# ifpen/wfcrl-env

Hardware: AMD Instinct MI355X
Metric: farm_steps_per_sec (higher is better)
Workload: dtype f32

## Files before the change

### include/wfstep.h

```cpp
#ifndef WFSTEP_H
#define WFSTEP_H

#ifdef __cplusplus
extern "C" {
#endif

#define WF_ABI_VERSION 7

#define WF_OK 0
#define WF_E_INVALID -1
#define WF_E_UNSUPPORTED -2
#define WF_E_NODEVICE -3
#define WF_E_HIP -4
#define WF_E_NOMEM -5

#define WF_MAX_TURBINES 256
#define WF_MAX_TABLE 64
#define WF_MAX_TURBINE_TYPES 4

typedef struct wf_handle wf_handle;

typedef struct wf_model_params {
  double air_density, ambient_ti, shear, veer;
  double rotor_diameter, hub_height, tsr, pP, pT, gen_eff, ref_density;
// ... 42 lines not shown
int wf_set_wind(wf_handle* h, const double* ws, const double* wd, int count, int on_device);

int wf_set_wind_counts(wf_handle* h, const double* ws, int n_ws, const double* wd, int n_wd, int on_device);

int wf_step(wf_handle* h, const float* yaw, float* power, float* wind_speed, float* wind_dir, float* load,
            int on_device);

int wf_sync(wf_handle* h);

#define WF_RISK_OVERLAP 1
#define WF_RISK_POWER_KNEE 2
#define WF_RISK_THRUST_RAMP 4
#define WF_RISK_THRUST_UNITY 8
#define WF_RISK_NEGATIVE_SPEED 16
int wf_set_risk_guard(wf_handle* h, double rel_band);
int wf_get_risk_flags(wf_handle* h, int* flags, int on_device);

int wf_set_risk_resolve(wf_handle* h, int mode);
int wf_get_risk_resolve(wf_handle* h, int* mode);
int wf_get_resolve_stats(wf_handle* h, int* n_resolved, int* raw_flags, int on_device);

typedef struct wf_env_params {
  float yaw_lo, yaw_hi, yaw_step;
  float actuator_rate;
  float dt;
  float budget;
  float load_coef;
  int discrete;
} wf_env_params;

int wf_env_config(wf_handle* h, const wf_env_params* p);

int wf_env_set_power_unit(wf_handle* h, int megawatts);

int wf_env_reset(wf_handle* h);

int wf_env_step(wf_handle* h, const float* action, float* reward, float* yaw, float* power, float* wind_speed,
                float* wind_dir, float* load, int on_device);

int wf_env_set_prev_wind(wf_handle* h, const double* wind_speed , int on_device);

int wf_env_state(wf_handle* h, float* yaw, float* acc, int* moves, int set, int on_device);

typedef struct wf_wind_dist {
  double ws_scale, ws_shape, ws_lo, ws_hi, wd_mean, wd_std, wd_lo, wd_hi;
} wf_wind_dist;
int wf_wind_sample(wf_handle* h, unsigned long long seed, const wf_wind_dist* dist);

int wf_wind_sample_binned(wf_handle* h, unsigned long long seed, const wf_wind_dist* dist, double step_deg);

int wf_wind_series(wf_handle* h, int T, const double* ws, const double* wd, const int* start, unsigned long long seed);
int wf_wind_series_step(wf_handle* h);

int wf_get_wind(wf_handle* h, double* ws, double* wd, int on_device);

int wf_timing_begin(wf_handle* h);
int wf_timing_end(wf_handle* h, float* elapsed_ms);

typedef struct wf_kernel_info {
  int lanes_per_env, slots_per_lane, envs_per_block, threads_per_block, grid_blocks;
  int vgprs, lds_bytes, scratch_bytes;
  int pair_table;
  int direction_groups;
  int mixed_main_farms;
  int one_block_kernel;
} wf_kernel_info;
int wf_get_kernel_info(wf_handle* h, wf_kernel_info* info);

typedef struct wf_kernel_choice {
  int slot_G, slot_S;
  int one_block;
  int ll_G, ll_S;
  int pair_table;
  int fly_one_block;
  int far_skip;
  int calibrate;
  int mixed;
} wf_kernel_choice;
int wf_set_kernel_choice(wf_handle* h, const wf_kernel_choice* c);
int wf_get_calibration(wf_handle* h, int* code, float* family_ms);
int wf_get_fly_calibration(wf_handle* h, int* choice, float* ms);
int wf_get_mixed_launch(wf_handle* h, int* main_farms, float* mixed_ms);
int wf_get_kernel_choice(wf_handle* h, wf_kernel_choice* c);
int wf_calibrate(wf_handle* h);
int wf_set_calibration(wf_handle* h, int code, int fly_choice);

const char* wf_last_error(wf_handle* h);

#ifdef __cplusplus
}
#endif
#endif
```

### wfcrl-env_amd/_lib.py

```python
from __future__ import annotations

import ctypes as C
import os
import subprocess
from pathlib import Path

PKG_DIR = Path(__file__).resolve().parent
LIB_PATH = PKG_DIR / "libwfstep.so"

WF_OK = 0
WF_RISK_OVERLAP = 1
WF_RISK_POWER_KNEE = 2
WF_RISK_THRUST_RAMP = 4
WF_RISK_THRUST_UNITY = 8
WF_RISK_NEGATIVE_SPEED = 16
WF_E = {-1: "WF_E_INVALID", -2: "WF_E_UNSUPPORTED", -3: "WF_E_NODEVICE", -4: "WF_E_HIP", -5: "WF_E_NOMEM"}

_MODEL_DOUBLES = (
    "air_density", "ambient_ti", "shear", "veer",
    "rotor_diameter", "hub_height", "tsr", "pP", "pT", "gen_eff", "ref_density",
    "alpha", "beta", "ka", "kb", "ad", "bd", "dm",
    "ch_initial", "ch_constant", "ch_ai", "ch_downstream",
    "eps_gain", "num_eps", "kappa", "gch_gain", "overlap_thresh", "near_wake_c",
    "defl_alpha", "defl_beta", "defl_ka", "defl_kb",
# ... 1 lines not shown
_MODEL_SWITCHES = ("enable_secondary_steering", "enable_yaw_added_recovery", "enable_transverse_velocities")


class ModelParams(C.Structure):

    _fields_ = [(n, C.c_double) for n in _MODEL_DOUBLES] + [
        ("n_table", C.c_int),
        ("table_ws", C.POINTER(C.c_double)),
        ("table_ct", C.POINTER(C.c_double)),
        ("table_cp", C.POINTER(C.c_double)),
    ] + [(n, C.c_int) for n in _MODEL_SWITCHES]


class TurbineDef(C.Structure):

    _fields_ = [("n_table", C.c_int), ("table_ws", C.POINTER(C.c_double)), ("table_ct", C.POINTER(C.c_double)),
                ("table_cp", C.POINTER(C.c_double))] + [(n, C.c_double) for n in ("tsr", "pP", "gen_eff", "ref_density")]


class EnvParams(C.Structure):

    _fields_ = [(n, C.c_float) for n in ("yaw_lo", "yaw_hi", "yaw_step", "actuator_rate", "dt", "budget", "load_coef")] + [
        ("discrete", C.c_int)]


class WindDist(C.Structure):

    _fields_ = [(n, C.c_double) for n in ("ws_scale", "ws_shape", "ws_lo", "ws_hi", "wd_mean", "wd_std", "wd_lo", "wd_hi")]


class KernelInfo(C.Structure):
    _fields_ = [(n, C.c_int) for n in (
        "lanes_per_env", "slots_per_lane", "envs_per_block", "threads_per_block", "grid_blocks",
        "vgprs", "lds_bytes", "scratch_bytes", "pair_table", "direction_groups", "mixed_main_farms", "one_block_kernel")]


class KernelChoice(C.Structure):

    _fields_ = [(n, C.c_int) for n in ("slot_G", "slot_S", "one_block", "ll_G", "ll_S", "pair_table", "fly_one_block", "far_skip", "calibrate", "mixed")]


_P = C.c_void_p
ABI = {
    "wf_version": (C.c_int, []),
    "wf_default_model": (C.c_int, [C.POINTER(ModelParams)]),
    "wf_turbine_table": (C.c_int, [C.c_char_p, C.POINTER(C.c_int), C.POINTER(C.POINTER(C.c_double)),
                                   C.POINTER(C.POINTER(C.c_double)), C.POINTER(C.POINTER(C.c_double))]),
    "wf_create": (C.c_int, [C.c_int, C.POINTER(_P)]),
    "wf_destroy": (C.c_int, [_P]),
    "wf_set_stream": (C.c_int, [_P, _P, C.c_int]),
    "wf_get_stream": (_P, [_P]),
    "wf_set_model": (C.c_int, [_P, C.POINTER(ModelParams)]),
    "wf_set_turbine_types": (C.c_int, [_P, C.c_int, C.POINTER(TurbineDef), C.POINTER(C.c_int)]),
    "wf_get_turbine_types": (C.c_int, [_P, C.POINTER(C.c_int)]),
    "wf_set_layout": (C.c_int, [_P, C.c_int, _P, _P]),
    "wf_set_batch": (C.c_int, [_P, C.c_int]),
    "wf_set_layouts": (C.c_int, [_P, C.c_int, _P, _P, _P]),
    "wf_set_layouts_counts": (C.c_int, [_P, C.c_int, _P, _P, _P, _P]),
    "wf_set_wind": (C.c_int, [_P, _P, _P, C.c_int, C.c_int]),
    "wf_set_wind_counts": (C.c_int, [_P, _P, C.c_int, _P, C.c_int, C.c_int]),
    "wf_wind_sample_binned": (C.c_int, [_P, C.c_ulonglong, C.POINTER(WindDist), C.c_double]),
    "wf_step": (C.c_int, [_P, _P, _P, _P, _P, _P, C.c_int]),
    "wf_sync": (C.c_int, [_P]),
    "wf_set_risk_guard": (C.c_int, [_P, C.c_double]),
    "wf_get_risk_flags": (C.c_int, [_P, _P, C.c_int]),
    "wf_set_risk_resolve": (C.c_int, [_P, C.c_int]),
    "wf_get_risk_resolve": (C.c_int, [_P, C.POINTER(C.c_int)]),
    "wf_get_resolve_stats": (C.c_int, [_P, C.POINTER(C.c_int), _P, C.c_int]),
    "wf_wind_sample": (C.c_int, [_P, C.c_ulonglong, C.POINTER(WindDist)]),
    "wf_wind_series": (C.c_int, [_P, C.c_int, _P, _P, _P, C.c_ulonglong]),
    "wf_wind_series_step": (C.c_int, [_P]),
    "wf_get_wind": (C.c_int, [_P, _P, _P, C.c_int]),
    "wf_env_config": (C.c_int, [_P, C.POINTER(EnvParams)]),
    "wf_env_set_power_unit": (C.c_int, [_P, C.c_int]),
    "wf_env_reset": (C.c_int, [_P]),
    "wf_env_state": (C.c_int, [_P, _P, _P, _P, C.c_int, C.c_int]),
    "wf_env_set_prev_wind": (C.c_int, [_P, _P, C.c_int]),
    "wf_env_step": (C.c_int, [_P, _P, _P, _P, _P, _P, _P, _P, C.c_int]),
    "wf_timing_begin": (C.c_int, [_P]),
    "wf_timing_end": (C.c_int, [_P, C.POINTER(C.c_float)]),
    "wf_get_kernel_info": (C.c_int, [_P, C.POINTER(KernelInfo)]),
    "wf_set_kernel_choice": (C.c_int, [_P, C.POINTER(KernelChoice)]),
    "wf_get_kernel_choice": (C.c_int, [_P, C.POINTER(KernelChoice)]),
    "wf_get_calibration": (C.c_int, [_P, C.POINTER(C.c_int), C.POINTER(C.c_float)]),
    "wf_get_fly_calibration": (C.c_int, [_P, C.POINTER(C.c_int), C.POINTER(C.c_float)]),
    "wf_get_mixed_launch": (C.c_int, [_P, C.POINTER(C.c_int), C.POINTER(C.c_float)]),
    "wf_calibrate": (C.c_int, [_P]),
    "wf_set_calibration": (C.c_int, [_P, C.c_int, C.c_int]),
    "wf_last_error": (C.c_char_p, [_P]),
}

PROBE_ABI = {
    "wf_probe_create": (C.c_int, [_P, C.POINTER(_P)]),
    "wf_probe_destroy": (C.c_int, [_P]),
    "wf_probe_set_points": (C.c_int, [_P, C.c_int, _P, C.c_int, C.c_int]),
    "wf_probe_sample": (C.c_int, [_P, _P, C.c_int, _P, _P, C.c_int]),
    "wf_probe_last_timing": (C.c_int, [_P, C.POINTER(C.c_float), C.POINTER(C.c_float)]),
    "wf_probe_kernel_info": (C.c_int, [_P, C.POINTER(C.c_int)]),
    "wf_probe_last_error": (C.c_char_p, [_P]),
}

YAWOPT_ABI = {
    "wf_yawopt_create": (C.c_int, [_P, C.POINTER(_P)]),
    "wf_yawopt_destroy": (C.c_int, [_P]),
    "wf_yawopt_config": (C.c_int, [_P, C.c_double, C.c_double, C.c_int, C.POINTER(C.c_int), C.c_int, C.c_int]),
    "wf_yawopt_run": (C.c_int, [_P, _P, C.c_int, _P, _P, _P, _P, C.c_int]),
    "wf_yawopt_set_timing": (C.c_int, [_P, C.c_int]),
    "wf_yawopt_last_timing": (C.c_int, [_P, C.POINTER(C.c_float), C.POINTER(C.c_float), C.POINTER(C.c_float)]),
    "wf_yawopt_evaluator": (_P, [_P]),
    "wf_yawopt_last_error": (C.c_char_p, [_P]),
}

ROSE_ABI = {
    "wf_rose_create": (C.c_int, [_P, C.POINTER(_P)]),
    "wf_rose_destroy": (C.c_int, [_P]),
    "wf_rose_set_table": (C.c_int, [_P, C.c_int, C.c_int, _P, C.c_int, _P, _P, C.c_int, C.c_int]),
    "wf_rose_set_rose": (C.c_int, [_P, C.c_int, _P, C.c_int, _P, _P, C.c_double, C.c_double]),
    "wf_rose_config": (C.c_int, [_P, C.c_int, C.c_int]),
    "wf_rose_evaluate": (C.c_int, [_P, C.c_int, _P, _P, _P, _P, _P, _P, C.c_int]),
    "wf_rose_policy": (C.c_int, [_P, C.c_int, _P, _P, C.c_int]),
    "wf_rose_last_timing": (C.c_int, [_P, C.POINTER(C.c_float), C.POINTER(C.c_float), C.POINTER(C.c_float)]),
    "wf_rose_kernel_info": (C.c_int, [_P, C.POINTER(C.c_int)]),
    "wf_rose_last_error": (C.c_char_p, [_P]),
}

ROBUST_ABI = {
    "wf_robust_create": (C.c_int, [_P, C.POINTER(_P)]),
    "wf_robust_destroy": (C.c_int, [_P]),
    "wf_robust_set_members": (C.c_int, [_P, C.c_int, _P, _P, C.c_int]),
    "wf_robust_config": (C.c_int, [_P, C.c_double, C.c_double, C.c_int, C.POINTER(C.c_int), C.c_int, C.c_int]),
    "wf_robust_evaluate": (C.c_int, [_P, _P, C.c_int, _P, _P, _P, _P, C.c_int]),
    "wf_robust_optimize": (C.c_int, [_P, _P, C.c_int, _P, _P, _P, _P, C.c_int]),
    "wf_robust_set_timing": (C.c_int, [_P, C.c_int]),
    "wf_robust_last_timing": (C.c_int, [_P, C.POINTER(C.c_float), C.POINTER(C.c_float), C.POINTER(C.c_float)]),
    "wf_robust_evaluator": (_P, [_P]),
    "wf_robust_kernel_info": (C.c_int, [_P, C.POINTER(C.c_int)]),
    "wf_robust_last_error": (C.c_char_p, [_P]),
}

GRAD_ABI = {
    "wf_grad_create": (C.c_int, [_P, C.POINTER(_P)]),
    "wf_grad_destroy": (C.c_int, [_P]),
    "wf_grad_config": (C.c_int, [_P, C.c_double, C.c_double, C.c_double, C.c_int, C.c_int]),
    "wf_grad_run": (C.c_int, [_P, _P, _P, C.c_int, _P, _P, _P, _P, C.c_int]),
    "wf_grad_set_timing": (C.c_int, [_P, C.c_int]),
    "wf_grad_last_timing": (C.c_int, [_P, C.POINTER(C.c_float), C.POINTER(C.c_float), C.POINTER(C.c_float)]),
    "wf_grad_evaluator": (_P, [_P]),
    "wf_grad_kernel_info": (C.c_int, [_P, C.POINTER(C.c_int)]),
    "wf_grad_last_error": (C.c_char_p, [_P]),
}

_lib = None


def build(force: bool = False) -> Path:
    srcs = []
    for d in ("", "ext", "probe", "yawopt", "rose", "robust", "grad"):
        srcs += sorted((PKG_DIR / "csrc" / d).glob("*.hip")) + sorted((PKG_DIR / "csrc" / d).glob("*.h"))
    srcs += [PKG_DIR.parent / "include" / h for h in ("wfstep.h", "wfprobe.h", "wfyawopt.h", "wfrose.h", "wfrobust.h", "wfgrad.h")]
    stale = (not LIB_PATH.exists()) or any(s.stat().st_mtime > LIB_PATH.stat().st_mtime for s in srcs)
    if force or stale:
        subprocess.run(["make", "-j4", "-C", str(PKG_DIR / "csrc")] + (["-B"] if force else []), check=True)
    return LIB_PATH


def _share_hip_runtime_with_torch():
# ... 62 lines not shown
```

### wfcrl-env_amd/backend.py

```python
from __future__ import annotations

import ctypes as C

import numpy as np

from . import _lib
from ._lib import EnvParams, KernelChoice, KernelInfo, ModelParams, WindDist, check


def _is_torch(a) -> bool:
    return type(a).__module__.startswith("torch")


def default_model() -> dict:
    p = ModelParams()
    check(_lib.load().wf_default_model(C.byref(p)))
    d = {n: getattr(p, n) for n in _lib._MODEL_DOUBLES}
    d.update({n: bool(getattr(p, n)) for n in _lib._MODEL_SWITCHES})
    n = p.n_table
    d["table_ws"] = [p.table_ws[i] for i in range(n)]
    d["table_ct"] = [p.table_ct[i] for i in range(n)]
    d["table_cp"] = [p.table_cp[i] for i in range(n)]
    return d

# ... 447 lines not shown

    def env_set_state(self, state: dict):
        B, N = self.env_batch, self.num_turbines
        yaw = np.ascontiguousarray(state["yaw"], np.float32).reshape(B, N)
        acc = np.ascontiguousarray(state["acc"], np.float32).reshape(B, N)
        moves = np.ascontiguousarray(state["moves"], np.int32).reshape(B)
        check(self._lib.wf_env_state(self._h, yaw.ctypes.data, acc.ctypes.data, moves.ctypes.data, 1, 0), self._h)

    def env_step(self, action=None, want=("reward", "yaw", "power", "wind_speed", "wind_direction", "load"), out=None):
        B, N = self.env_batch, self.num_turbines
        shapes = {"reward": (B,), "yaw": (B, N), "power": (B, N), "wind_speed": (B, N), "wind_direction": (B, N),
                  "load": (B, N, 4)}
        order = ("reward", "yaw", "power", "wind_speed", "wind_direction", "load")
        use_torch = _is_torch(action) or (action is None and out is not None and any(_is_torch(v) for v in out.values()))
        if use_torch:
            import torch

            dev = action.device if action is not None else next(iter(out.values())).device
            self._follow_torch_stream()
            if action is not None:
                assert action.is_cuda and action.dtype == torch.float32 and action.numel() == B * N
                action = action.contiguous()
            out = dict(out or {})
            for k in want:
                if k not in out:
                    out[k] = torch.empty(shapes[k], device=dev, dtype=torch.float32)
            ptrs = [out[k].data_ptr() if k in want else None for k in order]
            check(self._lib.wf_env_step(self._h, action.data_ptr() if action is not None else None, *ptrs, 1), self._h)
            return {k: out[k] for k in want}
        if action is not None:
            action = np.ascontiguousarray(action, dtype=np.float32).reshape(B, N)
        out = dict(out or {})
        for k in want:
            if k not in out:
                out[k] = np.empty(shapes[k], np.float32)
        ptrs = [out[k].ctypes.data if k in want else None for k in order]
        check(self._lib.wf_env_step(self._h, action.ctypes.data if action is not None else None, *ptrs, 0), self._h)
        return {k: out[k] for k in want}

    def sync(self):
        check(self._lib.wf_sync(self._h), self._h)

    def set_risk_guard(self, rel_band: float):
        check(self._lib.wf_set_risk_guard(self._h, float(rel_band)), self._h)

    def set_risk_resolve(self, mode: int | bool = 1):
        check(self._lib.wf_set_risk_resolve(self._h, int(mode)), self._h)

    def risk_resolve(self) -> int:
        m = C.c_int(0)
        check(self._lib.wf_get_risk_resolve(self._h, C.byref(m)), self._h)
        return int(m.value)

    def resolve_stats(self) -> dict:
        if not self.risk_resolve():
            raise RuntimeError("resolve_stats() needs the float64 re-solve on (set_risk_resolve(1), the default); with it off "
                               "the flags of the last step are risk_flags()")
        n = C.c_int(0)
        raw = np.empty(self.env_batch, np.int32)
        check(self._lib.wf_get_resolve_stats(self._h, C.byref(n), raw.ctypes.data, 0), self._h)
        return {"n_resolved": int(n.value), "raw_flags": raw}

    def risk_flags(self, as_torch: bool = False):
        B = self.env_batch
        if as_torch:
            import torch

            self._follow_torch_stream()
            f = torch.empty(B, dtype=torch.int32, device=f"cuda:{self.device_id}")
            check(self._lib.wf_get_risk_flags(self._h, f.data_ptr(), 1), self._h)
            return f
        f = np.empty(B, np.int32)
        check(self._lib.wf_get_risk_flags(self._h, f.ctypes.data, 0), self._h)
        return f

    def timing_begin(self):
        check(self._lib.wf_timing_begin(self._h), self._h)

    def timing_end(self) -> float:
        ms = C.c_float()
        check(self._lib.wf_timing_end(self._h, C.byref(ms)), self._h)
        return float(ms.value)

    def set_kernel_choice(self, slot=None, one_block=None, pair_table=None, fly_one_block=None, far_skip=None, calibrate=None, mixed=None):
        def gs(v, default_s=1):
            if isinstance(v, bool):
                raise ValueError("a kernel shape is (G, S), 'GxS' or G — not a bool (one_block=False disables the one-block "
                                 "kernel, None leaves the choice to the rounds model)")
            if isinstance(v, str):
                parts = v.lower().split("x")
                return int(parts[0]), (int(parts[1]) if len(parts) > 1 else default_s)
            if isinstance(v, int):
                return v, default_s
            return int(v[0]), int(v[1])

        c = KernelChoice(0, 0, -1, 0, 0, -1, -1, -1, -1, -1)
        if slot:
            c.slot_G, c.slot_S = gs(slot)
        if one_block is not None:
            if one_block is False or (not isinstance(one_block, bool) and one_block == 0):
                c.one_block = 0
            else:
                c.one_block = 1
                c.ll_G, c.ll_S = gs(one_block)
        if pair_table is not None:
            c.pair_table = int(bool(pair_table)) if pair_table is False else -1
        if fly_one_block is not None:
            c.fly_one_block = 0 if fly_one_block is False else -1
        if far_skip is not None:
            c.far_skip = 0 if far_skip is False or far_skip == 0 else -1
        if calibrate is not None:
            c.calibrate = 0 if calibrate is False or calibrate == 0 else -1
        if mixed is not None:
            c.mixed = 0 if mixed is False or mixed == 0 else -1
        check(self._lib.wf_set_kernel_choice(self._h, C.byref(c)), self._h)

    def kernel_choice(self) -> dict:
        c = KernelChoice()
        check(self._lib.wf_get_kernel_choice(self._h, C.byref(c)), self._h)
        return {n: getattr(c, n) for n, _ in KernelChoice._fields_}

    def calibration(self) -> dict:
        code = C.c_int(-1)
        ms = (C.c_float * 6)()
        check(self._lib.wf_get_calibration(self._h, C.byref(code), ms), self._h)
        names = ("slot", "8x1", "4x2", "4x1", "2x2", "16x1")
        shape = None if code.value < 0 else ("slot" if code.value == 0 else f"{code.value >> 4}x{code.value & 15}")
        fly, fms = C.c_int(0), (C.c_float * 2)()
        check(self._lib.wf_get_fly_calibration(self._h, C.byref(fly), fms), self._h)
        mixn, mixms = C.c_int(0), C.c_float(0.0)
        check(self._lib.wf_get_mixed_launch(self._h, C.byref(mixn), C.byref(mixms)), self._h)
        return {"shape": shape, "family_ms": {n: float(m) for n, m in zip(names, ms) if m > 0.0},
                "on_the_fly": (None, "one_block", "slot")[fly.value], "on_the_fly_ms": {n: float(m) for n, m in zip(("one_block", "slot"), fms) if m > 0.0},
                "mixed_main_farms": int(mixn.value), "mixed_ms": float(mixms.value)}

    def calibrate(self):
        check(self._lib.wf_calibrate(self._h), self._h)

    _FAMILY_CODES = {"slot": 0, "8x1": (8 << 4) | 1, "4x2": (4 << 4) | 2, "4x1": (4 << 4) | 1, "2x2": (2 << 4) | 2, "16x1": (16 << 4) | 1}

    def set_calibration(self, shape=None, on_the_fly=None):
        code = -1 if shape is None else self._FAMILY_CODES[shape]
        fly = {None: 0, "one_block": 1, "slot": 2}[on_the_fly]
        check(self._lib.wf_set_calibration(self._h, code, fly), self._h)

    def kernel_info(self) -> dict:
        k = KernelInfo()
        check(self._lib.wf_get_kernel_info(self._h, C.byref(k)), self._h)
        return {n: getattr(k, n) for n, _ in KernelInfo._fields_}

    def close(self):
        if getattr(self, "_h", None) is not None and self._h.value:
            for name in ("_probe_points", "_probe_plane", "_yawopt_obj", "_rose_obj", "_robust_obj", "_grad_obj"):
                ext = getattr(self, name, None)
                if ext is not None:
                    ext.close()
                    setattr(self, name, None)
            self._lib.wf_destroy(self._h)
            self._h = C.c_void_p()

    def __del__(self):
        try:
            self.close()
        except Exception:
            pass


class _Ext:

    NAME = ""
    KERNELS = ()

    def __init__(self, owner: WfStep):
        self._w, self._lib = owner, owner._lib
        self._r = C.c_void_p()
        check(self._fn("create")(owner._h, C.byref(self._r)), owner._h)

    def _fn(self, name):
        return getattr(self._lib, f"wf_{self.NAME}_{name}")

    def _call(self, name, *args):
        _lib.check_ext(self._fn(name)(self._r, *args), self._r, f"wf_{self.NAME}_last_error")

    def timing(self, detail=None):
        if detail is not None:
            self._call("set_timing", int(bool(detail)))
            return None
        t = [C.c_float(), C.c_float(), C.c_float()]
        self._call("last_timing", *[C.byref(v) for v in t])
        return {"total_ms": float(t[0].value), "step_ms": float(t[1].value), "glue_ms": float(t[2].value)}

    def kernel_info(self) -> dict:
        v = (C.c_int * (3 * len(self.KERNELS)))()
        self._call("kernel_info", v)
        keys = ("vgprs", "lds_bytes", "scratch_bytes")
        return {n: dict(zip(keys, v[3 * i:3 * i + 3])) for i, n in enumerate(self.KERNELS)}

    def evaluator(self):
# ... 319 lines not shown
```

### wfcrl-env_amd/csrc/ext/wf_ext.h

```cpp
#pragma once
#include <functional>

#include "../wf_handle.h"
#include "wf_ext_kernels.h"

namespace wfi {

struct ext_base {
  wf_handle* h = nullptr;
  std::string err;
  int detail = 0;
  std::vector<hipEvent_t> ev_pool;
  size_t n_ev = 0, per_chunk = 0;
  bool timed = false;
  ~ext_base();
};

inline int ext_fail(ext_base* x, int code, const std::string& msg) {
  if (x) x->err = msg;
  return code;
}
#define WFX_HIP(x, call)                                                                             \
  do {                                                                                               \
    hipError_t e_ = (call);                                                                          \
    if (e_ != hipSuccess) return ext_fail(x, WF_E_HIP, std::string(#call) + ": " + hipGetErrorString(e_)); \
  } while (0)
#define WFX_EV(x, evh, call)                                                     \
  do {                                                                           \
    int rc_ = (call);                                                            \
    if (rc_ != WF_OK) return ext_fail(x, rc_, std::string("evaluator: ") + wf_last_error(evh)); \
  } while (0)
#define WFX_ON_DEVICE(x)                 \
  DeviceGuard guard_((x)->h->device);    \
  if (guard_.err != hipSuccess) return ext_fail(x, WF_E_HIP, std::string("hipSetDevice: ") + hipGetErrorString(guard_.err))

template <class T>
struct dev_buf {
  T* p = nullptr;
  size_t cap = 0;
  dev_buf() = default;
  dev_buf(const dev_buf&) = delete;
  dev_buf& operator=(const dev_buf&) = delete;
  ~dev_buf() { hipFree(p); }
  operator T*() const { return p; }
};

template <class T>
int reserve(ext_base* x, dev_buf<T>& buf, size_t n) {
  if (n <= buf.cap) return WF_OK;
  WFX_HIP(x, hipStreamSynchronize(x->h->stream));
  hipFree(buf.p);
  buf.p = nullptr; buf.cap = 0;
  WFX_HIP(x, hipMalloc(&buf.p, sizeof(T) * n));
  buf.cap = n;
  return WF_OK;
}

struct evaluator {
  wf_handle* ev = nullptr;
  int E = 0, mode = -1;
  wf_model_params model{};
  std::vector<double> tws, tct, tcp, lx, ly;
  wf_kernel_choice choice{};
  double guard = 0.0;
  hipStream_t stream = nullptr;
  evaluator() = default;
  evaluator(const evaluator&) = delete;
  evaluator& operator=(const evaluator&) = delete;
  ~evaluator() { if (ev) wf_destroy(ev); }
};
int ensure_evaluator(ext_base* x, evaluator& s, int E, int mode);

struct farm_list {
  dev_buf<int> d;
  std::vector<int> host;
};

int check_parent(ext_base* x, const char* what, const char* call);
int check_wind(ext_base* x, const char* call);
int check_farms(ext_base* x, int* n_farms, const int* farms);
int upload_farms(ext_base* x, farm_list& fl, const int* farms, int n_farms);

inline WfSlots chunk_slots(const farm_list& fl, const int* farms, int base, int n_farms, int C) {
  return WfSlots{farms ? fl.d.p : nullptr, base, n_farms - base < C ? n_farms - base : C, C};
}

template <class T>
int stage_in(ext_base* x, const dev_buf<T>& buf, const T* src, size_t n, int on_device, const T** d) {
  *d = src;
  if (!src || on_device) return WF_OK;
  WFX_HIP(x, hipMemcpyAsync(buf.p, src, sizeof(T) * n, hipMemcpyHostToDevice, x->h->stream));
  *d = buf.p;
  return WF_OK;
}
template <class T>
T* out_ptr(T* user, const dev_buf<T>& staging, size_t offset, int on_device) {
  return user ? (on_device ? user : staging.p + offset) : nullptr;
}

int record(ext_base* x);
int last_timing(ext_base* x, const char* not_run, float* total_ms, float* step_ms, float* glue_ms);
int kernel_info(ext_base* x, int n, hipError_t (*attributes)(int, hipFuncAttributes*), int* info);

struct search_config {
  double lo = -25.0, hi = 25.0;
  int P = 2, K[WF_SEARCH_MAX_PASSES] = {5, 4, 0, 0};
  int strict = 0, max_eval = 65536;
};
int set_search_config(ext_base* x, search_config& c, double lo, double hi, int n_passes, const int* K, int strict, int max_eval_farms,
                      int rows_per_candidate, const char* rows_msg);
int k_max(int P, const int* K);
void pass_grids(double lo, double hi, int P, const int* K, WfGrid* grid);

struct yaw_search {
  search_config cfg;
  dev_buf<float> d_yaw, d_pow, d_best;
  dev_buf<int> d_order;
  farm_list farms;
  dev_buf<float> d_in, d_out;
};

struct search_policy {
  const char *what, *name;
  int rows_per_candidate;
  std::string no_rows;
  const char* rows_msg;
  std::function<int(int E)> reserve;
  std::function<int(const WfSlots&, int R, int E)> begin_chunk;
  std::function<int(const WfAdvanceArgs&, int v)> visit;
};
int run_search(ext_base* x, yaw_search& s, evaluator& es, const search_policy& k, const float* yaw0, int n_farms, const int* farms,
               float* yaw_opt, float* power_opt, float* power_init, int on_device);

template <class T>
int ext_create(wf_handle* h, T** out) {
  if (!h || !out) return WF_E_INVALID;
  *out = nullptr;
  T* x = new (std::nothrow) T();
  if (!x) return fail(h, WF_E_NOMEM, "out of host memory");
  x->h = h;
  *out = x;
  return WF_OK;
}

template <class T>
int ext_destroy(T* x) {
// ... 9 lines not shown
```

### wfcrl-env_amd/csrc/ext/wf_ext.hip

```cpp
#include "wf_ext.h"

namespace wfi {

ext_base::~ext_base() {
  for (hipEvent_t e : ev_pool) hipEventDestroy(e);
}

namespace {

bool same_model(const wf_model_params& a, const wf_model_params& b) {
  return std::memcmp(&a, &b, offsetof(wf_model_params, n_table)) == 0 && a.n_table == b.n_table &&
         a.enable_secondary_steering == b.enable_secondary_steering && a.enable_yaw_added_recovery == b.enable_yaw_added_recovery &&
         a.enable_transverse_velocities == b.enable_transverse_velocities;
}

}

int ensure_evaluator(ext_base* x, evaluator& s, int E, int mode) {
  wf_handle* h = x->h;
  const size_t n = (size_t)h->N;
  const bool same = s.ev && s.E == E && same_model(s.model, h->model) && s.tws == h->tws && s.tct == h->tct && s.tcp == h->tcp &&
                    s.lx.size() == n && std::equal(s.lx.begin(), s.lx.end(), h->lx.begin()) &&
                    std::equal(s.ly.begin(), s.ly.end(), h->ly.begin()) &&
                    std::memcmp(&s.choice, &h->choice, sizeof(wf_kernel_choice)) == 0 && s.guard == h->guard_rel;
  if (same) {
    if (s.stream != h->stream) {
      WFX_EV(x, s.ev, wf_set_stream(s.ev, (void*)h->stream, 1));
      s.stream = h->stream;
    }
    if (s.mode != mode) {
      WFX_EV(x, s.ev, wf_set_risk_resolve(s.ev, mode));
      s.mode = mode;
    }
    return WF_OK;
  }
  WFX_HIP(x, hipStreamSynchronize(h->stream));
  if (s.ev) wf_destroy(s.ev);
  s.ev = nullptr;
  wf_handle* ev = nullptr;
  if (wf_create(h->device, &ev) != WF_OK) return ext_fail(x, WF_E_HIP, std::string("evaluator: ") + wf_last_error(nullptr));
  s.ev = ev;
  wf_model_params m = h->model;
  m.table_ws = h->tws.data(); m.table_ct = h->tct.data(); m.table_cp = h->tcp.data();
  WFX_EV(x, ev, wf_set_stream(ev, (void*)h->stream, 1));
  WFX_EV(x, ev, wf_set_model(ev, &m));
  WFX_EV(x, ev, wf_set_kernel_choice(ev, &h->choice));
  if (h->guard_user) WFX_EV(x, ev, wf_set_risk_guard(ev, h->guard_rel));
  WFX_EV(x, ev, wf_set_layout(ev, h->N, h->lx.data(), h->ly.data()));
  WFX_EV(x, ev, wf_set_batch(ev, E));
  WFX_EV(x, ev, wf_set_risk_resolve(ev, mode));
  s.E = E; s.mode = mode; s.stream = h->stream;
  s.model = h->model; s.tws = h->tws; s.tct = h->tct; s.tcp = h->tcp;
  s.lx.assign(h->lx.begin(), h->lx.begin() + n); s.ly.assign(h->ly.begin(), h->ly.begin() + n);
  s.choice = h->choice; s.guard = h->guard_rel;
  return WF_OK;
}

int check_wind(ext_base* x, const char* call) {
  if (x->h->wind_count == 0)
    return ext_fail(x, WF_E_INVALID, std::string("no wind has been set: wf_set_wind (or wf_wind_*) must be called before ") + call);
  return WF_OK;
}

int check_parent(ext_base* x, const char* what, const char* call) {
  wf_handle* h = x->h;
  if (h->N <= 0 || h->B <= 0) return ext_fail(x, WF_E_INVALID, "no layout / batch: wf_set_layout and wf_set_batch come first");
  if (h->n_layouts > 1 || !h->layout_n.empty())
    return ext_fail(x, WF_E_UNSUPPORTED, std::string(what) + " a handle with ONE layout: this one holds several layouts (wf_set_layouts / wf_set_layouts_counts)");
  if (!h->types.empty())
    return ext_fail(x, WF_E_UNSUPPORTED, std::string(what) + " one turbine definition: this handle holds several turbine definitions (wf_set_turbine_types)");
  return call ? check_wind(x, call) : WF_OK;
}

int check_farms(ext_base* x, int* n_farms, const int* farms) {
  if (!farms) {
    *n_farms = x->h->B;
    return WF_OK;
  }
  if (*n_farms < 1) return ext_fail(x, WF_E_INVALID, "n_farms must be >= 1");
  for (int k = 0; k < *n_farms; ++k)
    if (farms[k] < 0 || farms[k] >= x->h->B) return ext_fail(x, WF_E_INVALID, "farm index out of range (0 .. env_batch - 1)");
  return WF_OK;
}

int upload_farms(ext_base* x, farm_list& fl, const int* farms, int n_farms) {
  WFX_HIP(x, hipStreamSynchronize(x->h->stream));
  fl.host.assign(farms, farms + n_farms);
  WFX_HIP(x, hipMemcpyAsync(fl.d, fl.host.data(), sizeof(int) * n_farms, hipMemcpyHostToDevice, x->h->stream));
  return WF_OK;
}

int record(ext_base* x) {
  if (x->n_ev == x->ev_pool.size()) {
    hipEvent_t e = nullptr;
    WFX_HIP(x, hipEventCreate(&e));
    x->ev_pool.push_back(e);
  }
  WFX_HIP(x, hipEventRecord(x->ev_pool[x->n_ev++], x->h->stream));
  return WF_OK;
}

int last_timing(ext_base* x, const char* not_run, float* total_ms, float* step_ms, float* glue_ms) {
  if (!x->timed || x->n_ev < 2) return ext_fail(x, WF_E_INVALID, not_run);
  WFX_ON_DEVICE(x);
  WFX_HIP(x, hipEventSynchronize(x->ev_pool[x->n_ev - 1]));
  float total = 0.0f, step = 0.0f, glue = 0.0f;
  WFX_HIP(x, hipEventElapsedTime(&total, x->ev_pool[0], x->ev_pool[x->n_ev - 1]));
  for (size_t k = 1; x->per_chunk && k < x->n_ev; ++k) {
    float ms = 0.0f;
    WFX_HIP(x, hipEventElapsedTime(&ms, x->ev_pool[k - 1], x->ev_pool[k]));
    const size_t q = k % x->per_chunk;
    if (q != 0 && q % 2 == 0) step += ms;
    else glue += ms;
  }
  if (total_ms) *total_ms = total;
  if (step_ms) *step_ms = step;
  if (glue_ms) *glue_ms = glue;
  return WF_OK;
}

int kernel_info(ext_base* x, int n, hipError_t (*attributes)(int, hipFuncAttributes*), int* info) {
  WFX_ON_DEVICE(x);
  for (int k = 0; k < n; ++k) {
    hipFuncAttributes a{};
    WFX_HIP(x, attributes(k, &a));
    info[3 * k] = a.numRegs; info[3 * k + 1] = (int)a.sharedSizeBytes; info[3 * k + 2] = (int)a.localSizeBytes;
  }
  return WF_OK;
}

int set_search_config(ext_base* x, search_config& c, double lo, double hi, int n_passes, const int* K, int strict, int max_eval_farms,
                      int rows_per_candidate, const char* rows_msg) {
  if (!std::isfinite(lo) || !std::isfinite(hi) || !(lo < hi)) return ext_fail(x, WF_E_INVALID, "yaw bounds must be finite with lo < hi");
  if (n_passes < 1 || n_passes > WF_SEARCH_MAX_PASSES) return ext_fail(x, WF_E_INVALID, "the number of passes must be in 1..4");
  if (K[0] < 2 || K[0] > WF_SEARCH_MAX_K0) return ext_fail(x, WF_E_INVALID, "the first pass needs 2..31 candidates (K_0)");
  for (int p = 1; p < n_passes; ++p)
    if (K[p] < 1 || K[p] > WF_SEARCH_MAX_K) return ext_fail(x, WF_E_INVALID, "a refining pass needs 1..15 candidates (K_p)");
// ... 98 lines not shown
```

### wfcrl-env_amd/csrc/wf_abi.hip

```cpp
#include "wf_handle.h"

namespace wfi {

thread_local std::string g_create_error;

void free_batch(wf_handle* h) {
  hipFree(h->d_ws); hipFree(h->d_wd); hipFree(h->d_gx); hipFree(h->d_gy); hipFree(h->d_gidx); hipFree(h->d_flags);
  hipFree(h->d_farm_tie);
  hipFree(h->d_dir_perm); hipFree(h->d_sort_keys); hipFree(h->d_sort_vals); hipFree(h->d_sort_tmp);
  h->d_dir_perm = h->d_sort_vals = nullptr; h->d_sort_keys = nullptr; h->d_sort_tmp = nullptr;
  h->sort_tmp_bytes = h->dir_perm_cap = 0; h->dir_slots = 0;
  hipFree(h->d_res_list); hipFree(h->d_res_count); hipFree(h->d_flags_raw);
  h->d_res_list = h->d_res_count = h->d_flags_raw = nullptr;
  if (h->h_res_seen) (void)hipHostFree(h->h_res_seen);
  h->h_res_seen = nullptr;
  h->d_flags = h->d_farm_tie = nullptr;
  hipFree(h->d_yaw); hipFree(h->d_out);
  hipFree(h->d_env_yaw); hipFree(h->d_env_acc); hipFree(h->d_env_act); hipFree(h->d_env_out); hipFree(h->d_env_moves);
  if (h->h_env_act) hipHostFree(h->h_env_act);
  if (h->h_env_out) hipHostFree(h->h_env_out);
  h->d_env_yaw = h->d_env_acc = h->d_env_act = h->d_env_out = h->h_env_act = h->h_env_out = nullptr;
  h->d_env_moves = nullptr;
  hipFree(h->d_series_ws); hipFree(h->d_series_wd); hipFree(h->d_series_start); hipFree(h->d_ws_prev);
  hipFree(h->d_pair_tab); hipFree(h->d_pair_first); h->d_pair_tab = nullptr; h->d_pair_first = nullptr; h->pair_dirty = true;
  hipFree(h->d_ll_tab); hipFree(h->d_ll_flag); hipFree(h->d_src_log);
  h->d_ll_tab = h->d_src_log = nullptr; h->d_ll_flag = nullptr; h->ll_groups_cap = h->log_records_cap = 0;
  hipFree(h->d_perm); hipFree(h->d_blk_group); hipFree(h->d_group_wd); hipFree(h->d_bins);
  h->d_perm = h->d_blk_group = h->d_bins = nullptr; h->d_group_wd = nullptr;
  h->perm_cap = h->blk_cap = h->pair_groups_cap = 0; h->n_groups = 0; h->grid_step = 0.0;
  h->d_series_ws = h->d_series_wd = h->d_ws_prev = nullptr; h->d_series_start = nullptr; h->series_T = 0;
  if (h->h_yaw) hipHostFree(h->h_yaw);
  if (h->h_out) hipHostFree(h->h_out);
  h->d_ws = h->d_wd = h->d_gx = h->d_gy = nullptr; h->d_gidx = nullptr;
  h->d_yaw = h->d_out = h->h_yaw = h->h_out = nullptr;
  h->cap_env = h->cap_bn = 0;
}

}

using namespace wfi;

extern "C" {

int wf_version(void) { return WF_ABI_VERSION; }
int wf_create(int device_id, wf_handle** out) {
  if (!out) return fail(nullptr, WF_E_INVALID, "out == NULL");
  *out = nullptr;
  int ndev = 0;
  hipError_t e = hipGetDeviceCount(&ndev);
  if (e != hipSuccess || ndev <= 0)
    return fail(nullptr, WF_E_NODEVICE, std::string("no HIP device visible (") + hipGetErrorString(e) +
                                            "); libwfstep has no CPU fallback");
  if (device_id < 0 || device_id >= ndev) return fail(nullptr, WF_E_NODEVICE, "device id out of range");
  wf_handle* h = new (std::nothrow) wf_handle();
  if (!h) return fail(nullptr, WF_E_NOMEM, "out of host memory");
  h->device = device_id;
  {
    wf_kernel_choice& c = h->choice;
    if (getenv("WF_NO_PAIR_TABLE")) c.pair_table = 0;
    const char* f = getenv("WF_LL_FLY");
    if (f && f[0] == '0') c.fly_one_block = 0;
    const char* gs = getenv("WF_KERNEL_GS");
    int og = 0, os = 0;
    if (gs && sscanf(gs, "%dx%d", &og, &os) == 2 && og > 0 && os > 0) { c.slot_G = og; c.slot_S = os; }
    const char* off = getenv("WF_LL");
    if (off && off[0] == '0') c.one_block = 0;
    const char* fs = getenv("WF_LL_FAR_SKIP");
    if (fs && fs[0] == '0') c.far_skip = 0;
    const char* rr = getenv("WF_RISK_RESOLVE");
    if (rr && rr[0] >= '0' && rr[0] <= '2' && rr[1] == 0) h->resolve_mode = rr[0] - '0';
    const char* cal = getenv("WF_CALIBRATE");
    if (cal && cal[0] == '0') c.calibrate = 0;
    const char* force = getenv("WF_LL_G");
    if (force && c.one_block != 0) {
      int g = 0, sl = 1;
      if (sscanf(force, "%dx%d", &g, &sl) >= 1) { c.one_block = 1; c.ll_G = g; c.ll_S = sl; }
      else c.one_block = 0;
    }
  }
  DeviceGuard guard(device_id);
  if ((e = guard.err) != hipSuccess || (e = hipStreamCreateWithFlags(&h->own_stream, hipStreamNonBlocking)) != hipSuccess ||
      (e = hipEventCreate(&h->ev0)) != hipSuccess || (e = hipEventCreate(&h->ev1)) != hipSuccess ||
      (e = hipMalloc(&h->d_tab, sizeof(WfTables))) != hipSuccess) {
    std::string msg = std::string("wf_create: ") + hipGetErrorString(e);
    delete h;
    return fail(nullptr, WF_E_HIP, msg);
  }
  h->stream = h->own_stream;
  {
    hipDeviceProp_t prop;
    if (hipGetDeviceProperties(&prop, device_id) == hipSuccess && prop.multiProcessorCount > 0) h->n_cu = prop.multiProcessorCount;
  }
  wf_model_params p;
  wf_default_model(&p);
  h->model = p;
  h->tws.assign(p.table_ws, p.table_ws + p.n_table);
  h->tct.assign(p.table_ct, p.table_ct + p.n_table);
  h->tcp.assign(p.table_cp, p.table_cp + p.n_table);
  *out = h;
  return WF_OK;
}

int wf_destroy(wf_handle* h) {
  if (!h) return WF_OK;
  DeviceGuard guard(h->device);
  hipStreamSynchronize(h->stream);
  free_batch(h);
  hipFree(h->d_tab64_mt); hipFree(h->d_type_consts); hipFree(h->d_type_of);
  hipFree(h->d_tab); hipFree(h->d_tab64); hipFree(h->d_lx); hipFree(h->d_ly); hipFree(h->d_centre); hipFree(h->d_layout_of);
  hipEventDestroy(h->ev0); hipEventDestroy(h->ev1);
  hipStreamDestroy(h->own_stream);
  delete h;
  return WF_OK;
}

int wf_set_stream(wf_handle* h, void* s, int external) {
  if (!h) return WF_E_INVALID;
  WF_ON_DEVICE(h);
  hipStream_t next = external ? (hipStream_t)s : h->own_stream;
  if (next != h->stream) {
    WF_HIP(h, hipStreamSynchronize(h->stream));
    h->stream = next;
  }
  return WF_OK;
}
void* wf_get_stream(wf_handle* h) { return h ? (void*)h->stream : nullptr; }

static int upload_layouts(wf_handle* h, int n, int K, const double* x, const double* y, const int* layout_of, const int* counts = nullptr) {
  std::vector<double> centre(2 * (size_t)K);
  for (int l = 0; l < K; ++l) {
    const double *xl = x + (size_t)l * n, *yl = y + (size_t)l * n;
    double xmin = xl[0], xmax = xl[0], ymin = yl[0], ymax = yl[0];
    const int n_l = counts ? counts[l] : n;
    for (int i = 0; i < n_l; ++i) {
      if (!std::isfinite(xl[i]) || !std::isfinite(yl[i])) return fail(h, WF_E_INVALID, "turbine coordinates must be finite");
      xmin = std::fmin(xmin, xl[i]); xmax = std::fmax(xmax, xl[i]);
      ymin = std::fmin(ymin, yl[i]); ymax = std::fmax(ymax, yl[i]);
    }
    centre[2 * l] = (xmin + xmax) / 2.0; centre[2 * l + 1] = (ymin + ymax) / 2.0;
  }
  WF_HIP(h, hipStreamSynchronize(h->stream));
  hipFree(h->d_lx); hipFree(h->d_ly); hipFree(h->d_centre); hipFree(h->d_layout_of); hipFree(h->d_layout_n); hipFree(h->d_nreal);
  h->d_lx = h->d_ly = h->d_centre = nullptr; h->d_layout_of = h->d_layout_n = h->d_nreal = nullptr;
  h->layout_n.clear();
  const size_t kn = (size_t)K * n;
  WF_HIP(h, hipMalloc(&h->d_lx, sizeof(double) * kn));
  WF_HIP(h, hipMalloc(&h->d_ly, sizeof(double) * kn));
  WF_HIP(h, hipMalloc(&h->d_centre, sizeof(double) * 2 * K));
  WF_HIP(h, hipMemcpy(h->d_lx, x, sizeof(double) * kn, hipMemcpyHostToDevice));
  WF_HIP(h, hipMemcpy(h->d_ly, y, sizeof(double) * kn, hipMemcpyHostToDevice));
  WF_HIP(h, hipMemcpy(h->d_centre, centre.data(), sizeof(double) * 2 * K, hipMemcpyHostToDevice));
// ... 212 lines not shown
```

### wfcrl-env_amd/csrc/wf_dispatch.hip

```cpp
#include "wf_handle.h"

#include <cstdlib>
#include <cstddef>
#include <map>
#include <tuple>

namespace wfi {

int find_variant(int G, int S) {
  for (int i = 0; i < wfk_num_variants(); ++i) {
    int g, s; const void* fn;
    wfk_variant(i, &g, &s, &fn);
    if (g == G && s == S) return i;
  }
  return -1;
}

int pick_variant(const wf_handle* h, int N, int B) {
  if (h->choice.slot_G > 0 && h->choice.slot_G * h->choice.slot_S >= N) {
    const int v = find_variant(h->choice.slot_G, h->choice.slot_S);
    if (v >= 0) return v;
  }
  static const int pref[][3] = {
      {4, 4, 1}, {8, 4, 2}, {12, 4, 3}, {16, 4, 4}, {24, 8, 3}, {32, 8, 4}, {48, 16, 3}, {64, 16, 4},
// ... 89 lines not shown
  const long per_round = (long)h->n_cu * per_cu * fpb;
  return (main_farms / per_round) * round_ms(fi, N, per_cu) + 0.9 * ll_estimate(h, 0, N, B - main_farms);
}

double family_estimate(const wf_handle* h, int fi, int N, long B, int* mix) {
  double t = ll_estimate(h, fi, N, B);
  *mix = 0;
  const int m = mix_candidate(h, fi, N, B);
  if (m) {
    const double tm = mix_estimate(h, fi, N, B, m);
    if (tm < 0.93 * t) { t = tm; *mix = m; }
  }
  return t;
}

int pick_ll(const wf_handle* h, int N, int B) {
  if (h->choice.one_block == 0) return 0;
  const bool veer = h->model.veer != 0.0;
  if (N > WF_PAIR_MAX_N) return 0;
  if (h->choice.one_block == 1) {
    const int g = h->choice.ll_G, sl = h->choice.ll_S > 0 ? h->choice.ll_S : 1;
    const bool ok = ((g == 4 || g == 8 || g == 16) && sl == 1) || ((g == 4 || g == 2) && sl == 2);
    return (ok && N > g * sl && (!veer || wfk_ll_has_veer(g, sl, 1))) ? ((g << 4) | sl) : 0;
  }
  if (N <= 16) return 0;
  {
    int fpb, per_cu;
    family_shape(h, 0, N, &fpb, &per_cu);
    if ((long)B <= (long)h->n_cu * fpb) return 0;
  }
  int best = 0;
  double t_best = 1e300;
  for (int fi = 0; fi < kNumFamilies; ++fi) {
    const LlFamily& f = kLlFamilies[fi];
    if (f.code && N <= (f.code >> 4) * (f.code & 15)) continue;
    if (f.code == ((8 << 4) | 1) && N <= 32) continue;
    if (veer && f.code && !wfk_ll_has_veer(f.code >> 4, f.code & 15, 1)) continue;
    int mix_unused;
    double t = family_estimate(h, fi, N, B, &mix_unused);
    if (f.code == ((16 << 4) | 1) && (long)B <= 2l * h->n_cu * f.farms_per_block) t *= 1.04;
    if (t < t_best) { t_best = t; best = f.code; }
  }
  return best;
}

int repick_ll_slots(const wf_handle* h, int N, int ll_G, int ll_S, long farm_slots) {
  if (ll_G != 4 || h->choice.one_block == 1 || N <= 8) return ll_S;
  return ll_estimate(h, 3, N, farm_slots) < ll_estimate(h, 2, N, farm_slots) ? 1 : 2;
}

void reset_calibration(wf_handle* h) {
  h->calib_done = false; h->calib_code = -1; h->tab_slot = false; h->mix_main = 0;
  for (float& m : h->calib_ms) m = 0.0f;
  h->fly_calib = 0; h->fly_calib_ms[0] = h->fly_calib_ms[1] = 0.0f;
}

int model_mix(const wf_handle* h, int code, int N, int B) {
  if (!code || h->choice.one_block == 0) return 0;
  for (int fi = 0; fi < kNumFamilies; ++fi)
    if (kLlFamilies[fi].code == code) {
      int m = 0;
      family_estimate(h, fi, N, B, &m);
      return m;
    }
  return 0;
}

void apply_kernel_pick(wf_handle* h, int N, int B, bool* variant_changed) {
  reset_calibration(h);
  const int v = pick_variant(h, N, B);
  const int llg = pick_ll(h, N, B);
  set_ll_shape(h, llg >> 4, llg ? (llg & 15) : 1);
  h->mix_main = model_mix(h, llg, N, B);
  if (variant_changed) *variant_changed = v != h->variant;
  if (v != h->variant) {
    hipFree(h->d_pair_tab); hipFree(h->d_pair_first);
    h->d_pair_tab = nullptr; h->d_pair_first = nullptr; h->pair_dirty = true; h->pair_groups_cap = 0;
    h->variant = v;
  }
}

void set_ll_shape(wf_handle* h, int G, int S) {
  if (G == h->ll_G && S == h->ll_S) return;
  hipFree(h->d_ll_tab); hipFree(h->d_ll_flag); hipFree(h->d_src_log);
  h->d_ll_tab = h->d_src_log = nullptr; h->d_ll_flag = nullptr; h->ll_groups_cap = h->log_records_cap = 0;
  h->ll_G = G; h->ll_S = S; h->pair_dirty = true;
}
int pair_table(wf_handle* h, const float** out) {
  *out = nullptr;
  if ((h->wind_count != 1 && !h->shared_dir && h->n_groups == 0) || h->N > WF_PAIR_MAX_N || !wfk_variant_has_table(h->variant) || h->choice.pair_table == 0)
    return WF_OK;
  int vG, vS; const void* vfn;
  wfk_variant(h->variant, &vG, &vS, &vfn);
  const int NP = vG * vS;
  const size_t ng = h->n_groups > 0 ? (size_t)h->n_groups : 1;
  if (!h->d_pair_tab || h->pair_groups_cap < ng) {
    hipFree(h->d_pair_tab); hipFree(h->d_pair_first);
    h->d_pair_tab = nullptr; h->d_pair_first = nullptr; h->pair_groups_cap = 0;
    WF_HIP(h, hipMalloc(&h->d_pair_tab, sizeof(float) * ng * h->N * WF_PAIR_ROW_FLOATS(NP)));
    WF_HIP(h, hipMalloc(&h->d_pair_first, sizeof(int) * ng * h->N));
    h->pair_groups_cap = ng;
    h->pair_dirty = true;
  }
  if (h->pair_dirty) {
    const wf_model_params& m = h->model;
    WfPairConsts pc{};
    const double D = m.rotor_diameter, HH = m.hub_height, eps = m.eps_gain * D;
    pc.N = h->N; pc.NP = NP; pc.D = D; pc.HH = HH; pc.eps2 = eps * eps; pc.num_eps = m.num_eps; pc.ch_down = m.ch_downstream;
    const double off[3] = {-D / 4, 0.0, D / 4};
    double uinf = 0;
    for (int k = 0; k < 3; ++k) uinf += std::pow((HH + off[k]) / HH, m.shear) / 3.0;
    pc.fifteenD = 15.0 * D;
    pc.twoD = 2.0 * D;
    pc.gam_top = (1.0 / 16.0) * D * std::pow((HH + D / 2) / HH, m.shear) * uinf;
    pc.gam_bot = (1.0 / 16.0) * D * std::pow((HH - D / 2) / HH, m.shear) * uinf;
    for (int k = 0; k < 3; ++k) {
      pc.off[k] = off[k];
      const double z = HH + off[k];
      const double dudz = m.shear * std::pow(1.0 / HH, m.shear) * std::pow(z, m.shear - 1.0);
      const double lm = m.kappa * z / (1.0 + m.kappa * z / (D / 8.0));
      pc.decay_a[k] = 4.0 * lm * lm * std::fabs(dudz) / uinf / pc.eps2;
    }
    WF_HIP(h, wfk_launch_pair_table(&pc, (int)ng, h->d_gx, h->d_gy, h->d_pair_tab, h->d_pair_first, h->stream));
    if (h->ll_G) {
      if (!h->d_ll_tab || h->ll_groups_cap < ng) {
        hipFree(h->d_ll_tab); hipFree(h->d_ll_flag);
        h->d_ll_tab = nullptr; h->d_ll_flag = nullptr; h->ll_groups_cap = 0;
        WF_HIP(h, hipMalloc(&h->d_ll_tab, sizeof(float) * ng * wfk_ll_table_floats(h->N, h->ll_G * h->ll_S)));
        WF_HIP(h, hipMalloc(&h->d_ll_flag, sizeof(int) * ng));
        h->ll_groups_cap = ng;
      }
      WF_HIP(h, wfk_launch_pair_table_ll(&pc, h->ll_G * h->ll_S, (int)ng, h->d_gx, h->d_gy, h->d_ll_tab, h->d_ll_flag, h->stream));
      h->ll_ties = 2;
      if (h->wind_sync) {
        std::vector<int> f(ng);
        WF_HIP(h, hipMemcpyAsync(f.data(), h->d_ll_flag, sizeof(int) * ng, hipMemcpyDeviceToHost, h->stream));
        WF_HIP(h, hipStreamSynchronize(h->stream));
        size_t tied = 0;
        for (int v : f) tied += v != 0;
        h->ll_ties = tied == 0 ? 0 : (tied == ng ? 1 : 2);
      }
    }
    h->pair_dirty = false;
  }
  *out = h->d_pair_tab;
  return WF_OK;
}

int ll_fly_S(const wf_handle* h);
int ll_fly_G(const wf_handle* h);
int run_geometry(wf_handle* h, int n_env, const double* d_wd, bool sync_ok) {
  const bool per_farm = n_env == h->B && h->B > 1 && h->ll_G && wfk_ll_has_fly(ll_fly_G(h), ll_fly_S(h));
  WF_HIP(h, wfk_launch_geometry(n_env, h->N, h->d_lx, h->d_ly, h->d_centre, h->n_layouts == 1 ? 0 : (h->d_layout_of ? 2 : 1),
                                h->d_layout_of, h->d_layout_n, d_wd, 1, h->d_gx, h->d_gy, h->d_gidx,
                                per_farm ? ll_fly_G(h) * ll_fly_S(h) : 0, h->d_farm_tie, h->d_farm_tie ? h->d_farm_tie + h->B : nullptr,
                                h->stream));
  h->farm_ties = 2;
  h->dir_slots = 0;
  h->geo_tie_block = per_farm ? ll_fly_G(h) * ll_fly_S(h) : 0;
  if (per_farm && h->n_layouts == 1 && h->choice.fly_one_block != 0 && h->choice.far_skip != 0) {
    const int fpb = wfk_ll_farms_per_block(ll_fly_G(h));
    const size_t slots = (size_t)((h->B + fpb - 1) / fpb) * fpb;
    if (slots > h->dir_perm_cap) {
      WF_HIP(h, hipStreamSynchronize(h->stream));
      hipFree(h->d_dir_perm); hipFree(h->d_sort_keys); hipFree(h->d_sort_vals); hipFree(h->d_sort_tmp);
      h->d_dir_perm = h->d_sort_vals = nullptr; h->d_sort_keys = nullptr; h->d_sort_tmp = nullptr; h->dir_perm_cap = 0;
      WF_HIP(h, wfk_sort_tmp_bytes(h->B, &h->sort_tmp_bytes));
      WF_HIP(h, hipMalloc(&h->d_dir_perm, sizeof(int) * slots));
      WF_HIP(h, hipMalloc(&h->d_sort_keys, sizeof(float) * 2 * (size_t)h->B));
      WF_HIP(h, hipMalloc(&h->d_sort_vals, sizeof(int) * (size_t)h->B));
      WF_HIP(h, hipMalloc(&h->d_sort_tmp, h->sort_tmp_bytes > 0 ? h->sort_tmp_bytes : 16));
      h->dir_perm_cap = slots;
    }
    WF_HIP(h, wfk_sort_by_direction(h->B, (int)slots, d_wd, h->d_sort_keys, h->d_sort_vals, h->d_sort_tmp, h->sort_tmp_bytes,
                                    h->d_dir_perm, h->stream));
    h->dir_slots = (int)slots;
  }
  if (per_farm && sync_ok) {
    int any = 0;
    WF_HIP(h, hipMemcpyAsync(&any, h->d_farm_tie + h->B, sizeof(int), hipMemcpyDeviceToHost, h->stream));
    WF_HIP(h, hipStreamSynchronize(h->stream));
    h->farm_ties = any ? 1 : 0;
  }
  return WF_OK;
}

int ll_fly_S(const wf_handle* h) { return h->ll_G <= 4 ? 2 : h->ll_S; }
int ll_fly_G(const wf_handle* h) {
  if (h->ll_G == 2) return h->model.veer != 0.0 ? 4 : 2;
  return h->ll_G == 16 ? 8 : h->ll_G;
}

size_t ll_npad(const wf_handle* h) {
  const int a = h->ll_G * h->ll_S, b = ll_fly_G(h) * ll_fly_S(h), gs = a > b ? a : b;
  return (size_t)((h->N + gs - 1) / gs) * gs;
}

int ll_log_fpb(const wf_handle* h) {
  const int a = wfk_ll_farms_per_block(h->ll_G), b = wfk_ll_farms_per_block(ll_fly_G(h));
  return a > b ? a : b;
}
static int ensure_log(wf_handle* h, size_t slots, size_t* records) {
  *records = slots * ll_npad(h);
  if (*records > h->log_records_cap) {
    WF_HIP(h, hipStreamSynchronize(h->stream));
    hipFree(h->d_src_log); h->d_src_log = nullptr; h->log_records_cap = 0;
    WF_HIP(h, hipMalloc(&h->d_src_log, sizeof(float) * *records * (WF_LOG_FLOATS + WF_LOG_SIDE_FLOATS)));
    h->log_records_cap = *records;
  }
  return WF_OK;
}
int launch_step_f32(wf_handle* h, const float* yaw, float* power, float* wspd, float* wdir, float* load, const WfEnvArgs* ea) {
  const int gstride = (h->wind_count == 1 || h->shared_dir) ? 0 : h->N;
  const int wstride = (h->wind_count == 1) ? 0 : 1;
  const float* ptab = nullptr;
  int rc = pair_table(h, &ptab);
  if (rc != WF_OK) return rc;
  WfGroupArgs ga{};
  ga.mod = 1;
  ga.risk_flags = h->d_flags;
  ga.n_real = h->d_nreal;
  if (h->res_mask) {
    ga.res_list = h->d_res_list; ga.flags_raw = h->d_flags_raw; ga.res_mask = h->res_mask;
    ga.res_count = h->d_res_count + h->res_parity; ga.res_zero = h->d_res_count + (h->res_parity ^ 1);
  }
  ga.blk_unit = 1;
  if (h->n_groups > 0) {
    ga.perm = h->d_perm; ga.blk_group = h->d_blk_group; ga.n_blocks = h->n_blocks;
    ga.shift = h->group_shift; ga.mod = h->n_groups;
    ga.blk_unit = group_unit(h); ga.n_slots = h->n_slots;
  }
  if (ptab && h->ll_G && !(h->tab_slot && h->n_groups == 0)) {
    const int fpb = ll_log_fpb(h);
    const size_t slots = h->n_groups > 0 ? (size_t)h->n_slots : (size_t)((h->B + fpb - 1) / fpb) * fpb;
    size_t log_records = 0;
    if ((rc = ensure_log(h, slots, &log_records)) != WF_OK) return rc;
    const int M = (h->choice.mixed != 0 && h->mix_main > 0 && h->mix_main < h->B && h->n_groups == 0) ? h->mix_main : 0;
    if (M) { ga.env_base = 0; ga.env_end = M; }
    if (h->ll_ties != 1)
      WF_HIP(h, wfk_launch_step_ll(h->ll_G, h->ll_S, &h->consts, h->d_tab, h->d_gidx, h->d_ws, h->d_wd, wstride, yaw, power, wspd, wdir,
                                   load, h->B, ea, h->d_ll_tab, h->d_ll_flag, h->d_src_log,
                                   log_records, &ga, h->stream));
    if (M) {
      if (h->ll_ties != 0) {
        WfGroupArgs gp = ga;
        gp.pred = h->d_ll_flag;
        WF_HIP(h, wfk_launch_step(h->variant, &h->consts, h->d_tab, h->d_gx, h->d_gy, h->d_gidx, gstride, h->d_ws, h->d_wd,
                                  wstride, yaw, power, wspd, wdir, load, h->B, ea, ptab, h->d_pair_first, &gp, h->stream, &h->grid));
      }
      ga.env_base = M; ga.env_end = h->B;
      WF_HIP(h, wfk_launch_step(h->variant, &h->consts, h->d_tab, h->d_gx, h->d_gy, h->d_gidx, gstride, h->d_ws, h->d_wd,
                                wstride, yaw, power, wspd, wdir, load, h->B, ea, ptab, h->d_pair_first, &ga, h->stream, &h->grid));
      return WF_OK;
    }
    if (h->ll_ties == 0) return WF_OK;
    ga.pred = h->d_ll_flag;
  }
  if (!ptab && gstride != 0 && h->B > 1 && h->ll_G && wfk_ll_has_fly(ll_fly_G(h), ll_fly_S(h)) && h->choice.fly_one_block != 0 &&
      h->fly_calib != 2) {
    const int fpb = ll_log_fpb(h);
    const size_t slots = (size_t)((h->B + fpb - 1) / fpb) * fpb;
    size_t log_records = 0;
    if ((rc = ensure_log(h, slots, &log_records)) != WF_OK) return rc;
    if (h->geo_tie_block != ll_fly_G(h) * ll_fly_S(h)) {
      if ((rc = run_geometry(h, h->B, h->d_wd, false)) != WF_OK) return rc;
    }
    WfGroupArgs gf = ga;
    if (h->dir_slots > 0 && h->n_groups == 0) gf.perm = h->d_dir_perm;
    WF_HIP(h, wfk_launch_step_ll_fly(ll_fly_G(h), ll_fly_S(h), &h->consts, h->d_tab, h->d_gidx, h->d_gx, h->d_gy, h->d_ws, h->d_wd, yaw,
                                     power, wspd, wdir, load, h->B, ea, h->d_farm_tie, h->d_src_log,
                                     log_records, &gf, h->stream));
    if (h->farm_ties == 0) return WF_OK;
    ga.farm_pred = h->d_farm_tie;
  }
  WF_HIP(h, wfk_launch_step(h->variant, &h->consts, h->d_tab, h->d_gx, h->d_gy, h->d_gidx, gstride, h->d_ws, h->d_wd,
                            wstride, yaw, power, wspd, wdir, load, h->B, ea, ptab, h->d_pair_first, &ga, h->stream, &h->grid));
  return WF_OK;
}

static bool calibration_due(const wf_handle* h) {
  if (h->calib_done || h->choice.calibrate == 0 || h->choice.one_block != -1 || h->choice.pair_table == 0) return false;
  if (h->N <= 16 || h->N > WF_PAIR_MAX_N || h->n_groups > 0 || h->n_layouts != 1) return false;
  if (!(h->wind_count == 1 || h->shared_dir) || !wfk_variant_has_table(h->variant)) return false;
  int fpb, per_cu;
  family_shape(h, 0, h->N, &fpb, &per_cu);
  return (long)h->B > (long)h->n_cu * fpb;
}

struct CalibKey {
  int device, N, B, n_cu, far_skip;
  int mixed, slot_G, slot_S;
  unsigned long long layout_hash, model_hash;
  bool operator<(const CalibKey& o) const {
    return std::tie(device, N, B, n_cu, far_skip, mixed, slot_G, slot_S, layout_hash, model_hash) <
           std::tie(o.device, o.N, o.B, o.n_cu, o.far_skip, o.mixed, o.slot_G, o.slot_S, o.layout_hash, o.model_hash);
  }
};
struct CalibVal {
  bool have_tab = false, have_fly = false;
  int code = -1, fly = 0, mix_main = 0;
  float ms[8] = {}, fly_ms[2] = {};
};
static std::mutex g_calib_mu;
static std::map<CalibKey, CalibVal> g_calib;

static unsigned long long fnv(const void* p, size_t n, unsigned long long hsh = 1469598103934665603ull) {
  const unsigned char* b = static_cast<const unsigned char*>(p);
  for (size_t i = 0; i < n; ++i) hsh = (hsh ^ b[i]) * 1099511628211ull;
  return hsh;
}
static CalibKey calib_key(const wf_handle* h) {
  CalibKey k{};
  k.device = h->device; k.N = h->N; k.B = h->B; k.n_cu = h->n_cu; k.far_skip = h->choice.far_skip;
  k.mixed = h->choice.mixed != 0; k.slot_G = h->choice.slot_G; k.slot_S = h->choice.slot_S;
  k.layout_hash = fnv(h->ly.data(), sizeof(double) * h->ly.size(), fnv(h->lx.data(), sizeof(double) * h->lx.size()));
  const wf_model_params& m = h->model;
  unsigned long long mh = fnv(&m, offsetof(wf_model_params, n_table));
  const int sw[3] = {m.enable_secondary_steering, m.enable_yaw_added_recovery, m.enable_transverse_velocities};
  mh = fnv(sw, sizeof(sw), mh);
  mh = fnv(h->tws.data(), sizeof(double) * h->tws.size(), mh);
  mh = fnv(h->tct.data(), sizeof(double) * h->tct.size(), mh);
  k.model_hash = fnv(h->tcp.data(), sizeof(double) * h->tcp.size(), mh);
  return k;
}

static void apply_family(wf_handle* h, int code, int guess_code) {
  if (code == 0) {
    set_ll_shape(h, guess_code >> 4, guess_code ? (guess_code & 15) : 1);
    h->tab_slot = guess_code != 0;
  } else {
    set_ll_shape(h, code >> 4, code & 15);
    h->tab_slot = false;
  }
}

static bool family_valid(const wf_handle* h, int fi) {
  const LlFamily& f = kLlFamilies[fi];
  const bool veer = h->model.veer != 0.0;
  if (f.code && h->N <= (f.code >> 4) * (f.code & 15)) return false;
  if (f.code == ((8 << 4) | 1) && h->N <= 32) return false;
  if (veer && f.code && !wfk_ll_has_veer(f.code >> 4, f.code & 15, 1)) return false;
  return true;
}

static int calibrate_families(wf_handle* h, const float* yaw, float* power, float* wspd, float* wdir, float* load, const WfEnvArgs* ea) {
  const int N = h->N, B = h->B;
  double est[kNumFamilies], best_est = 1e300;
  int mix_f[kNumFamilies];
  for (int fi = 0; fi < kNumFamilies; ++fi) {
    est[fi] = 1e300;
    mix_f[fi] = 0;
    if (!family_valid(h, fi)) continue;
    est[fi] = family_estimate(h, fi, N, B, &mix_f[fi]);
    if (est[fi] < best_est) best_est = est[fi];
  }
  hipEvent_t e0 = nullptr, e1 = nullptr;
  WF_HIP(h, hipEventCreate(&e0));
  WF_HIP(h, hipEventCreate(&e1));
  int best = -1, guess = -1;
  float best_ms = 1e30f;
  int rc = WF_OK;
  const int code0 = h->ll_G ? ((h->ll_G << 4) | h->ll_S) : 0;
  for (int fi = 0; fi < kNumFamilies && rc == WF_OK; ++fi) {
    if (kLlFamilies[fi].code == code0 && est[fi] < 1e300) guess = fi;
    if (!(est[fi] <= 1.6 * best_est) && fi != guess) continue;
    hipStreamSynchronize(h->stream);
    apply_family(h, kLlFamilies[fi].code, code0);
    h->mix_main = mix_f[fi];
    if ((rc = launch_step_f32(h, yaw, power, wspd, wdir, load, ea)) != WF_OK) break;
    float fam_ms = 1e30f;
    for (int r = 0; r < 3 && rc == WF_OK; ++r) {
      hipError_t e = hipEventRecord(e0, h->stream);
      rc = launch_step_f32(h, yaw, power, wspd, wdir, load, ea);
      if (e == hipSuccess) e = hipEventRecord(e1, h->stream);
      if (e == hipSuccess) e = hipEventSynchronize(e1);
      float ms = 0.0f;
      if (e == hipSuccess) e = hipEventElapsedTime(&ms, e0, e1);
      if (e != hipSuccess) { rc = fail(h, WF_E_HIP, std::string("calibration: ") + hipGetErrorString(e)); break; }
      if (ms < fam_ms) fam_ms = ms;
    }
    if (rc != WF_OK) break;
    h->calib_ms[fi] = fam_ms;
    if (fam_ms < best_ms) { best_ms = fam_ms; best = fi; }
  }
  hipStreamSynchronize(h->stream);
  if (rc != WF_OK) {
    hipEventDestroy(e0);
    hipEventDestroy(e1);
    apply_family(h, code0, code0);
    h->mix_main = guess >= 0 ? mix_f[guess] : 0;
    return rc;
  }
  if (guess >= 0 && h->calib_ms[guess] > 0.0f && h->calib_ms[guess] <= 1.04f * best_ms) best = guess;
  const int code = best >= 0 ? kLlFamilies[best].code : code0;
  apply_family(h, code, code0);
  h->calib_code = code;
// ... 173 lines not shown
  if (ea) {
    ra.yaw_state = ea->yaw_state; ra.reward = ea->reward; ra.ws_prev = ea->ws_prev; ra.load_coef = ea->load_coef;
    ra.power_mw = ea->power_mw;
  }
  h->rconsts.N = h->N;
  if (!h->types.empty()) {
    ra.tab64 = h->d_tab64_mt; ra.n_types = (int)h->types.size(); ra.type_of = h->d_type_of; ra.type_consts = h->d_type_consts;
    WF_HIP(h, wfk_launch_resolve_mt(&h->rconsts, &ra, h->B, 1, h->d_flags_raw, h->n_cu, h->stream));
    return WF_OK;
  }
  WF_HIP(h, wfk_launch_resolve(&h->rconsts, &ra, h->B, mode == 2 ? 1 : 0, h->d_flags_raw, h->n_cu, h->stream));
  return WF_OK;
}

}

using namespace wfi;

extern "C" {

int wf_get_kernel_info(wf_handle* h, wf_kernel_info* info) {
  if (!h || !info) return WF_E_INVALID;
  if (h->variant < 0) return fail(h, WF_E_INVALID, "wf_set_layout must be called first");
  int G, S; const void* fn;
  wfk_variant(h->variant, &G, &S, &fn);
  if (h->model_dirty && h->N > 0) { int rc = build_consts(h); if (rc != WF_OK) return rc; }
  const bool tab = (h->wind_count == 1 || h->shared_dir || h->n_groups > 0) && h->N <= WF_PAIR_MAX_N && wfk_variant_has_table(h->variant) && h->choice.pair_table != 0;
  const bool veer = h->model.veer != 0.0;
  fn = wfk_variant_fn(h->variant, tab ? (h->wind_count == 1 ? (veer ? 5 : 2) : (veer ? 6 : 3)) : (veer ? 4 : (h->consts.mirror_core_n <= 1 ? 0 : 1)));
  info->pair_table = tab ? 1 : 0;
  info->direction_groups = h->n_groups;
  hipFuncAttributes a;
  WF_ON_DEVICE(h);
  WF_HIP(h, hipFuncGetAttributes(&a, fn));
  info->lanes_per_env = G; info->slots_per_lane = S;
  const int wpb = tab ? wfk_tab_waves() : 4;
  info->envs_per_block = wpb * (64 / G); info->threads_per_block = 64 * wpb;
  info->grid_blocks = h->n_groups > 0 ? (h->n_slots + info->envs_per_block - 1) / info->envs_per_block
                                      : (h->B > 0 ? (h->B + info->envs_per_block - 1) / info->envs_per_block : 0);
  const bool ll_fly = !tab && h->wind_count == h->B && h->B > 1 && h->n_groups == 0 && h->ll_G && wfk_ll_has_fly(ll_fly_G(h), ll_fly_S(h)) && h->choice.fly_one_block != 0 &&
                      h->fly_calib != 2;
  info->one_block_kernel = ((tab && h->ll_G && !(h->tab_slot && h->n_groups == 0)) || ll_fly) ? 1 : 0;
  info->mixed_main_farms = (tab && info->one_block_kernel && !ll_fly && h->n_groups == 0 && h->choice.mixed != 0 && h->mix_main > 0 && h->mix_main < h->B) ? h->mix_main : 0;
  if (info->one_block_kernel) {
    const int ll_s = tab ? h->ll_S : ll_fly_S(h), ll_g = tab ? h->ll_G : ll_fly_G(h);
    info->lanes_per_env = ll_g; info->slots_per_lane = ll_s;
    info->envs_per_block = wfk_ll_farms_per_block(ll_g); info->threads_per_block = 256;
    info->grid_blocks = (int)(((h->n_groups > 0 ? (size_t)h->n_slots : (size_t)h->B) + info->envs_per_block - 1) / info->envs_per_block);
    const int ll_blocks = info->mixed_main_farms ? info->mixed_main_farms / info->envs_per_block : info->grid_blocks;
    WF_HIP(h, wfk_ll_func_attributes(ll_g, ll_s, h->wind_count == 1 ? 1 : 0, tab ? 1 : 0, veer ? 1 : 0,
                                     (ll_s == 1 && ll_blocks <= 2 * h->n_cu) ? 1 : 0, &a));
  }
  info->vgprs = a.numRegs;
  info->lds_bytes = (int)a.sharedSizeBytes; info->scratch_bytes = (int)a.localSizeBytes;
  return WF_OK;
}


int wf_set_kernel_choice(wf_handle* h, const wf_kernel_choice* c) {
  if (!h || !c) return WF_E_INVALID;
  if ((c->slot_G > 0) != (c->slot_S > 0) || (c->slot_G > 0 && find_variant(c->slot_G, c->slot_S) < 0))
    return fail(h, WF_E_INVALID, "no wf_step_kernel variant with these lanes per farm x slots per lane");
  if (c->one_block < -1 || c->one_block > 1 || c->pair_table < -1 || c->pair_table > 1 || c->fly_one_block < -1 || c->fly_one_block > 1 ||
      c->far_skip < -1 || c->far_skip > 1 || c->calibrate < -1 || c->calibrate > 1 || c->mixed < -1 || c->mixed > 1)
    return fail(h, WF_E_INVALID, "kernel choice switches must be -1 (automatic), 0 or 1");
  if (c->one_block == 1) {
    const int g = c->ll_G, sl = c->ll_S > 0 ? c->ll_S : 1;
    if (!(((g == 4 || g == 8 || g == 16) && sl == 1) || ((g == 4 || g == 2) && sl == 2)))
      return fail(h, WF_E_INVALID, "wf_step_ll_kernel is instantiated for G x S in {4x1, 8x1, 16x1, 4x2, 2x2}");
  }
  WF_ON_DEVICE(h);
  WF_HIP(h, hipStreamSynchronize(h->stream));
  if (c->far_skip != h->choice.far_skip) h->model_dirty = true;
  h->choice = *c;
  if (h->N > 0) {
    const int v = pick_variant(h, h->N, h->B);
    if (v < 0) return fail(h, WF_E_UNSUPPORTED, "no kernel variant for this turbine count");
    apply_kernel_pick(h, h->N, h->B, nullptr);
  }
  h->wind_count = 0; h->shared_dir = false; h->n_groups = 0; h->grid_step = 0.0; h->series_T = 0; h->pair_dirty = true;
  return WF_OK;
}

int wf_calibrate(wf_handle* h) {
  if (!h) return WF_E_INVALID;
  if (h->wind_count == 0) return fail(h, WF_E_INVALID, "wf_set_wind must be called before wf_calibrate");
  WF_ON_DEVICE(h);
  if (h->model_dirty) {
    int rc = build_consts(h);
    if (rc != WF_OK) return rc;
  }
  WF_HIP(h, hipStreamSynchronize(h->stream));
  apply_kernel_pick(h, h->N, h->B, nullptr);
  if (h->variant < 0) return fail(h, WF_E_UNSUPPORTED, "no kernel variant for this turbine count");
  const size_t bn = (size_t)h->B * h->N;
  float* d = nullptr;
  WF_HIP(h, hipMalloc(&d, sizeof(float) * bn * 8));
  hipError_t e = hipMemsetAsync(d, 0, sizeof(float) * bn, h->stream);
  int rc = e == hipSuccess ? calibrate_now(h, d, d + bn, d + 2 * bn, d + 3 * bn, d + 4 * bn, nullptr, false)
                           : fail(h, WF_E_HIP, std::string("wf_calibrate: ") + hipGetErrorString(e));
  hipStreamSynchronize(h->stream);
  hipFree(d);
  return rc;
}

int wf_set_calibration(wf_handle* h, int code, int fly_choice) {
  if (!h) return WF_E_INVALID;
  if (h->N <= 0 || h->B <= 0) return fail(h, WF_E_INVALID, "wf_set_layout and wf_set_batch must be called before wf_set_calibration");
  if (code < -1 || fly_choice < 0 || fly_choice > 2) return fail(h, WF_E_INVALID, "wf_set_calibration: code is -1 or a family code, fly_choice 0, 1 or 2");
  WF_ON_DEVICE(h);
  return apply_saved_calibration(h, code, fly_choice);
}

int wf_get_calibration(wf_handle* h, int* code, float* family_ms) {
  if (!h) return WF_E_INVALID;
  if (code) *code = h->calib_done ? h->calib_code : -1;
  if (family_ms)
    for (int fi = 0; fi < 6; ++fi) family_ms[fi] = fi < kNumFamilies ? h->calib_ms[fi] : 0.0f;
  return WF_OK;
}

int wf_get_mixed_launch(wf_handle* h, int* main_farms, float* mixed_ms) {
  if (!h) return WF_E_INVALID;
  if (main_farms) *main_farms = (h->choice.mixed != 0 && h->mix_main > 0 && h->mix_main < h->B) ? h->mix_main : 0;
  if (mixed_ms) *mixed_ms = h->calib_ms[6];
  return WF_OK;
}

int wf_get_fly_calibration(wf_handle* h, int* choice, float* ms) {
  if (!h) return WF_E_INVALID;
  if (choice) *choice = h->fly_calib;
  if (ms) { ms[0] = h->fly_calib_ms[0]; ms[1] = h->fly_calib_ms[1]; }
  return WF_OK;
}

int wf_get_kernel_choice(wf_handle* h, wf_kernel_choice* c) {
  if (!h || !c) return WF_E_INVALID;
  *c = h->choice;
  return WF_OK;
}

}
```

### wfcrl-env_amd/csrc/wf_handle.h

```cpp
#pragma once
#include <hip/hip_runtime.h>

#include <cmath>
#include <cstdio>
#include <cstdlib>
#include <cstring>
#include <mutex>
#include <new>
#include <string>
#include <vector>

#include "../../include/wfstep.h"
#include "wf_device.h"
#include "wf_resolve.h"

extern "C" hipError_t wfk_launch_resolve(const WfResolveConsts* c, const WfResolveArgs* a, int B, int all, int* raw_flags,
                                         int n_cu, hipStream_t s);
extern "C" int wfk_num_variants();
extern "C" void wfk_variant(int i, int* G, int* S, const void** fn);
extern "C" int wfk_variant_has_table(int i);
extern "C" int wfk_tab_waves();
extern "C" const void* wfk_variant_fn(int i, int kind);
extern "C" hipError_t wfk_launch_geometry(int n_env, int N, const double* lx, const double* ly, const double* centre,
                                          int layout_mode, const int* layout_of, const int* layout_n, const double* wd, int wd_stride, double* gx,
                                          double* gy, int* gidx, int tie_block, int* farm_tie, int* any_tie, hipStream_t s);
extern "C" int wfk_ll_has_fly(int G, int S);
extern "C" int wfk_ll_has_veer(int G, int S, int table);
extern "C" hipError_t wfk_launch_step_ll_fly(int G, int S, const WfConsts* c, const WfTables* tab, const int* gidx, const double* gx,
                                             const double* gy, const double* ws, const double* wd, const float* yaw,
                                             float* power, float* o_ws, float* o_wd, float* load, int B, const WfEnvArgs* env,
                                             const int* farm_tie, float* src_log, size_t log_records,
                                             const WfGroupArgs* grp, hipStream_t s);
extern "C" hipError_t wfk_launch_step(int variant, const WfConsts* c, const WfTables* tab, const double* gx,
                                      const double* gy, const int* gidx, int geom_stride, const double* ws,
                                      const double* wd, int wind_stride, const float* yaw, float* power, float* o_ws,
                                      float* o_wd, float* load, int B, const WfEnvArgs* env, const float* pair_tab,
                                      const int* pair_first, const WfGroupArgs* grp, hipStream_t s, int* grid_out);
extern "C" hipError_t wfk_launch_pair_table(const WfPairConsts* pc, int n_groups, const double* gx, const double* gy,
                                            float* tab, int* first_active, hipStream_t s);

extern "C" hipError_t wfk_launch_wind_sample(int B, unsigned long long seed, const double* dist, double* ws, double* wd,
                                             hipStream_t s);
extern "C" size_t wfk_ll_table_floats(int N, int G);
extern "C" int wfk_ll_farms_per_block(int G);
extern "C" hipError_t wfk_launch_pair_table_ll(const WfPairConsts* pc, int G, int n_groups, const double* gx, const double* gy,
                                               float* tab, int* cross_tie, hipStream_t s);
extern "C" hipError_t wfk_launch_step_ll(int G, int S, const WfConsts* c, const WfTables* tab, const int* gidx, const double* ws,
                                         const double* wd, int wind_stride, const float* yaw, float* power, float* o_ws,
                                         float* o_wd, float* load, int B, const WfEnvArgs* env, const float* ll_tab,
                                         const int* cross_tie, float* src_log, size_t log_records,
                                         const WfGroupArgs* grp, hipStream_t s);
extern "C" hipError_t wfk_ll_func_attributes(int G, int S, int shared_speed, int table, int veer, int occ2, hipFuncAttributes* a);
extern "C" hipError_t wfk_launch_fill(int n, double* a, hipStream_t s);
extern "C" hipError_t wfk_sort_tmp_bytes(int B, size_t* bytes);
extern "C" hipError_t wfk_sort_by_direction(int B, int n_slots, const double* wd, float* keys, int* vals, void* tmp, size_t tmp_bytes,
                                            int* perm, hipStream_t s);
extern "C" hipError_t wfk_launch_wind_sample_binned(int B, unsigned long long seed, const double* dist, double step, double* ws,
                                                    double* wd, int* bin, hipStream_t s);
extern "C" hipError_t wfk_launch_bin_centres(int K, double step, double* wd, hipStream_t s);
extern "C" hipError_t wfk_launch_series_start(int B, int T, unsigned long long seed, int* start, hipStream_t s);
extern "C" hipError_t wfk_launch_series_gather(int B, int T, int t, const int* start, const double* s_ws,
                                               const double* s_wd, double* ws, double* wd, hipStream_t s);

struct wf_handle {
  int device = 0;
  hipStream_t own_stream = nullptr;
  hipStream_t stream = nullptr;
  hipEvent_t ev0 = nullptr, ev1 = nullptr;
  std::string err;

  wf_model_params model{};
  std::vector<double> tws, tct, tcp;
  bool model_dirty = true;

  int N = 0;
  std::vector<double> lx, ly;
  double xc = 0, yc = 0;
  int n_layouts = 1;
  std::vector<int> layout_of;
  int* d_layout_of = nullptr;
  double* d_centre = nullptr;
  std::vector<int> layout_n;
  int* d_layout_n = nullptr;
  int* d_nreal = nullptr;
  int B = 0;
  int wind_count = 0;
  int variant = -1;
  int grid = 0;

  WfConsts consts{};
  WfTables* d_tab = nullptr;
  double *d_lx = nullptr, *d_ly = nullptr;
  double *d_ws = nullptr, *d_wd = nullptr;
  double* d_gx = nullptr;
  double* d_gy = nullptr;
  int* d_gidx = nullptr;
  int* d_flags = nullptr;
  double guard_rel = 1.0e-5;
  bool guard_user = false;
  float *d_yaw = nullptr, *d_out = nullptr;
  float *h_yaw = nullptr, *h_out = nullptr;
  size_t cap_env = 0, cap_bn = 0;
  wf_env_params env{-40.f, 40.f, 5.f, 0.3f, 60.f, 0.1f, 0.1f, 0};
  int env_power_mw = 0;
  float *d_env_yaw = nullptr, *d_env_acc = nullptr, *d_env_act = nullptr, *d_env_out = nullptr;
  int* d_env_moves = nullptr;
  float *h_env_act = nullptr, *h_env_out = nullptr;
  int series_T = 0, series_t = 0;
  double *d_series_ws = nullptr, *d_series_wd = nullptr;
  int* d_series_start = nullptr;
  double* d_ws_prev = nullptr;
  float* d_pair_tab = nullptr;
  int* d_pair_first = nullptr;
  bool pair_dirty = true;
  bool ws_prev_valid = false;
  bool shared_dir = false;
  int n_groups = 0;
  int group_shift = 0;
  int n_blocks = 0;
  int n_slots = 0;
  int *d_perm = nullptr, *d_blk_group = nullptr;
  size_t perm_cap = 0, blk_cap = 0;
  size_t pair_groups_cap = 0;
  double* d_group_wd = nullptr;
  double grid_step = 0.0;
  int* d_bins = nullptr;
  int ll_G = 0, ll_S = 1;
  float* d_ll_tab = nullptr;
  int* d_ll_flag = nullptr;
  float* d_src_log = nullptr;
  size_t ll_groups_cap = 0, log_records_cap = 0;
  int* d_farm_tie = nullptr;
  int* d_dir_perm = nullptr;
  float* d_sort_keys = nullptr;
  int* d_sort_vals = nullptr;
  void* d_sort_tmp = nullptr;
  size_t sort_tmp_bytes = 0, dir_perm_cap = 0;
  int dir_slots = 0;
  int geo_tie_block = 0;
  int farm_ties = 2;
  bool wind_sync = true;
  int ll_ties = 2;
  wf_kernel_choice choice{0, 0, -1, 0, 0, -1, -1, -1, -1, -1};
  int n_cu = 256;
  bool calib_done = false;
  int calib_code = -1;
  int mix_main = 0;
  bool tab_slot = false;
  float calib_ms[8] = {};
  int fly_calib = 0;
  float fly_calib_ms[2] = {};
  int resolve_mode = 1;
  WfResolveConsts rconsts{};
  double* d_tab64 = nullptr;
  int *d_res_list = nullptr, *d_res_count = nullptr, *d_flags_raw = nullptr;
  int* h_res_seen = nullptr;
  int res_parity = 0;
  bool res_last = false;
  int res_mask = 0;
  struct TurbineType {
    std::vector<double> ws, ct, cp;
    double tsr, pP, gen_eff, ref_density;
  };
  std::vector<TurbineType> types;
  std::vector<int> type_of;
  double* d_tab64_mt = nullptr;
  double* d_type_consts = nullptr;
  int* d_type_of = nullptr;
};

namespace wfi {

extern thread_local std::string g_create_error;

struct DeviceGuard {
  int prev = -1;
  bool switched = false;
  hipError_t err = hipSuccess;
  explicit DeviceGuard(int device) {
    err = hipGetDevice(&prev);
    if (err == hipSuccess && prev != device) {
      err = hipSetDevice(device);
      switched = err == hipSuccess;
    }
  }
  ~DeviceGuard() {
    if (switched) hipSetDevice(prev);
  }
};
#define WF_ON_DEVICE(h) \
  DeviceGuard guard_((h)->device); \
  if (guard_.err != hipSuccess) return fail(h, WF_E_HIP, std::string("hipSetDevice: ") + hipGetErrorString(guard_.err))
inline int fail(wf_handle* h, int code, const std::string& msg) {
  if (h) h->err = msg; else g_create_error = msg;
  return code;
}
#define WF_HIP(h, call)                                                                       \
  do {                                                                                        \
    hipError_t e_ = (call);                                                                   \
    if (e_ != hipSuccess) return fail(h, WF_E_HIP, std::string(#call) + ": " + hipGetErrorString(e_)); \
  } while (0)

void free_batch(wf_handle* h);
void init_default_table();
int build_consts(wf_handle* h);
int pick_variant(const wf_handle* h, int N, int B);
int pick_ll(const wf_handle* h, int N, int B);
int model_mix(const wf_handle* h, int code, int N, int B);
int repick_ll_slots(const wf_handle* h, int N, int ll_G, int ll_S, long farm_slots);
void set_ll_shape(wf_handle* h, int G, int S);
void apply_kernel_pick(wf_handle* h, int N, int B, bool* variant_changed);
int pair_table(wf_handle* h, const float** out);
int run_geometry(wf_handle* h, int n_env, const double* d_wd, bool sync_ok);
int ll_fly_S(const wf_handle* h);
int ll_fly_G(const wf_handle* h);
size_t ll_npad(const wf_handle* h);
int ll_log_fpb(const wf_handle* h);
int launch_step(wf_handle* h, const float* yaw, float* power, float* wspd, float* wdir, float* load, const WfEnvArgs* ea);
void reset_calibration(wf_handle* h);
int calibrate_now(wf_handle* h, const float* yaw, float* power, float* wspd, float* wdir, float* load, const WfEnvArgs* probe, bool use_cache);
int apply_saved_calibration(wf_handle* h, int code, int fly_choice);
void ungroup(wf_handle* h);
int farms_per_block(const wf_handle* h);
int group_pad(const wf_handle* h);
int group_unit(const wf_handle* h);
bool groups_pay_off(const wf_handle* h, int K);
// ... 6 lines not shown
```

### wfcrl-env_amd/csrc/wf_kernels_ll.hip

```cpp
#include <hip/hip_runtime.h>

#include <cstring>
#include <type_traits>
#include <utility>

#include "wf_kernel_common.h"

namespace {

template <class F, int... I>
__device__ __forceinline__ void static_for_impl(F&& f, std::integer_sequence<int, I...>) {
  (f(std::integral_constant<int, I>{}), ...);
}
template <int N, class F>
__device__ __forceinline__ void static_for(F&& f) {
  static_for_impl(f, std::make_integer_sequence<int, N>{});
}

__device__ __forceinline__ void sincos_yaw(float x, float& s, float& c) {
  const float x2 = x * x;
  s = x * fmaf(x2, fmaf(x2, fmaf(x2, fmaf(x2, 2.7557319e-6f, -1.9841270e-4f), 8.3333333e-3f), -1.6666667e-1f), 1.0f);
  c = fmaf(x2, fmaf(x2, fmaf(x2, fmaf(x2, fmaf(x2, -2.7557319e-7f, 2.4801587e-5f), -1.3888889e-3f), 4.1666667e-2f), -0.5f), 1.0f);
  if (__any(fabsf(x) > 0.8f)) {
    float s2, c2;
    sincosf(x, &s2, &c2);
    s = (fabsf(x) > 0.8f) ? s2 : s;
    c = (fabsf(x) > 0.8f) ? c2 : c;
  }
}

template <int G>
__device__ __forceinline__ float wave_max(float v) {
  auto dpp = [](float x, auto ctrl, auto rows) {
    return __int_as_float(__builtin_amdgcn_update_dpp(__float_as_int(x), __float_as_int(x), decltype(ctrl)::value, decltype(rows)::value, 0xf, false));
  };
  using I = std::integral_constant<int, 0>;
  (void)sizeof(I);
  if constexpr (G < 2) v = fmaxf(v, dpp(v, std::integral_constant<int, 0xB1>{}, std::integral_constant<int, 0xf>{}));
  if constexpr (G < 4) v = fmaxf(v, dpp(v, std::integral_constant<int, 0x4E>{}, std::integral_constant<int, 0xf>{}));
  if constexpr (G < 8) v = fmaxf(v, dpp(v, std::integral_constant<int, 0x141>{}, std::integral_constant<int, 0xf>{}));
  if constexpr (G < 16) v = fmaxf(v, dpp(v, std::integral_constant<int, 0x140>{}, std::integral_constant<int, 0xf>{}));
  v = fmaxf(v, dpp(v, std::integral_constant<int, 0x142>{}, std::integral_constant<int, 0xa>{}));
  v = fmaxf(v, dpp(v, std::integral_constant<int, 0x143>{}, std::integral_constant<int, 0xc>{}));
  return __int_as_float(__builtin_amdgcn_readlane(__float_as_int(v), 63));
}

struct SrcLog {
  float Gy, Gwt, sy0d, sz0d;
  float sM, tan_th0, sy0v, snw;
  float kdef, x0d, kyd, pj;
  float x0v, kyv, ch_pref, ix0v;
  float inv_s0d, d0;
};
struct ColdRec { float4 a, b, c; };
static_assert(WF_LOG_HOT_FLOATS == 2 && WF_LOG_COLD_FLOATS == 12, "source log record");
struct WfLogSide { float TI0, TI1, TI2, dTI; };

}

__global__ void wf_pair_table_ll_kernel(const WfPairConsts pc, int G, const double* __restrict__ gx,
                                        const double* __restrict__ gy, float* __restrict__ tab, size_t group_floats,
                                        int* __restrict__ cross_tie) {
  const int i = blockIdx.x, t = threadIdx.x, grp = blockIdx.y;
  const int nblk = (pc.N + G - 1) / G;
  if (t >= nblk * G) return;
  gx += (size_t)grp * pc.N;
  gy += (size_t)grp * pc.N;
  const int J = t / G;
  if (i >= (J + 1) * G) {
    if (t < pc.N && gx[t] - gx[i] >= 0.0) atomicOr(&cross_tie[grp], 1);
    return;
  }
  float* o = tab + (size_t)grp * group_floats + wf_ll_block_offset(J, pc.N, G) + ((size_t)i * G + (t - J * G)) * WF_PAIR_STRIDE;
  wf_pair_record(pc, gx, gy, i, t, o);
}

extern "C" size_t wfk_ll_table_floats(int N, int G) { return wf_ll_block_offset((N + G - 1) / G, N, G); }

extern "C" hipError_t wfk_launch_pair_table_ll(const WfPairConsts* pc, int G, int n_groups, const double* gx, const double* gy,
                                               float* tab, int* cross_tie, hipStream_t s) {
  const int nblk = (pc->N + G - 1) / G;
  const int threads = ((nblk * G + 63) / 64) * 64;
  hipError_t e = hipMemsetAsync(cross_tie, 0, sizeof(int) * (size_t)n_groups, s);
  if (e != hipSuccess) return e;
  hipLaunchKernelGGL(wf_pair_table_ll_kernel, dim3(pc->N, n_groups), dim3(threads), 0, s, *pc, G, gx, gy, tab,
                     wfk_ll_table_floats(pc->N, G), cross_tie);
  return hipGetLastError();
}

#ifdef WF_LL_STAMP
__device__ unsigned long long wf_ll_stamp[16];
#define WF_T(v) const unsigned long long v = __builtin_readcyclecounter()
#define WF_ACC(k, a, b) st_acc[k] += (b) - (a)
#else
#define WF_T(v)
#define WF_ACC(k, a, b)
#endif
template <int G, int S, bool UWS, bool TAB, bool MC1, int WPB, bool VEER = false, bool OCC2 = false>
__global__ __launch_bounds__(64 * WPB, ((S == 1 && !OCC2) ? 3 : 2) * 4 / WPB) void wf_step_ll_kernel(
    const WfConsts c, const WfTables* __restrict__ tab, const int* __restrict__ gidx, const double* __restrict__ ws_in,
    const double* __restrict__ wd_in, int wind_stride, const float* __restrict__ yaw_in, float* __restrict__ o_power,
    float* __restrict__ o_ws, float* __restrict__ o_wd, float* __restrict__ o_load, int B, const WfEnvArgs ea,
    const float* __restrict__ ll_tab, size_t group_floats, const int* __restrict__ cross_tie, float* __restrict__ src_log,
    size_t log_cold_offset, size_t log_side_offset, int n_pad, const WfGroupArgs ga, const double* __restrict__ gx,
    const double* __restrict__ gy) {
  constexpr int EPW = 64 / G;
  constexpr int GS = G * S;
  constexpr int CH = 64 / GS;
  constexpr int CHUNK_FLOATS = TAB ? 64 * WF_PAIR_STRIDE : 4;
  __shared__ TableLds T;
  __shared__ __attribute__((aligned(16))) float prow[2][CHUNK_FLOATS];
  __shared__ unsigned risk_lds[WPB][EPW];
  __shared__ int env_lds[WPB][EPW];
  extern __shared__ __attribute__((aligned(16))) float yaw_lds[];

  if (ga.res_zero && blockIdx.x == 0 && threadIdx.x == 0) *ga.res_zero = 0;
  int grp = 0;
  if (ga.blk_group) {
    grp = ga.blk_group[(blockIdx.x * (WPB * EPW)) / ga.blk_unit];
    if (grp < 0) return;
    grp = (grp + ga.shift) % ga.mod;
  }
  if constexpr (TAB) {
    if (cross_tie[grp]) return;
    ll_tab += (size_t)grp * group_floats;
  }

  auto stage_chunk = [&](int q) {
    const char* g0 = reinterpret_cast<const char*>(ll_tab) + (size_t)q * (CHUNK_FLOATS * 4);
    char* l0 = reinterpret_cast<char*>(&prow[q & 1][0]);
    for (int ch = (int)(threadIdx.x >> 6); ch < CHUNK_FLOATS * 4 / 1024; ch += WPB)
      lds_dma16(g0 + ch * 1024 + (threadIdx.x & 63) * 16, l0 + ch * 1024, false);
  };
  if constexpr (TAB) stage_chunk(0);
  for (int k = threadIdx.x; k < WF_TABLE_PAD; k += blockDim.x) {
    T.knot[k] = tab->knot[k];
    T.ct[k] = tab->ct[k];
    T.cts[k] = tab->ct_slope[k];
    T.pw[k] = tab->pw[k];
    T.pws[k] = tab->pw_slope[k];
  }
  for (int k = threadIdx.x; k < WF_BUCKETS; k += blockDim.x) T.bucket[k] = tab->bucket[k];

  const int lane = threadIdx.x & 63;
  const int wave = threadIdx.x >> 6;
  const int sub = lane & (G - 1);
  const int gbase = lane & ~(G - 1);
  const int eiw = lane / G;
  const int slot = (blockIdx.x * WPB + wave) * EPW + eiw;
  int env_raw = slot + ga.env_base;
  if (ga.perm) env_raw = ga.perm[env_raw];
  bool env_ok = env_raw >= 0 && env_raw < (ga.env_end ? ga.env_end : B);
  const int env = env_ok ? env_raw : (B - 1);
  if constexpr (!TAB) env_ok = env_ok && !cross_tie[env];
  if (sub == 0) risk_lds[wave][eiw] = 0u;
  const int N = c.N;
  const int nblk = (N + GS - 1) / GS;

  auto uni = [](float v) { return UWS ? __int_as_float(__builtin_amdgcn_readfirstlane(__float_as_int(v))) : v; };
  const float ws = uni((float)ws_in[(size_t)env * wind_stride]);
  const double wd_d = fmod(wd_in[(size_t)env * wind_stride], 360.0);
  const float wd = uni((float)(wd_d < 0.0 ? wd_d + 360.0 : wd_d));
  const float Ui[3] = {uni(ws * c.shearf[0]), uni(ws * c.shearf[1]), uni(ws * c.shearf[2])};
  const float offk = c.off[2] * kGs;
  const float U02c = uni(Ui[0] * Ui[0] * Ui[0] + Ui[2] * Ui[2] * Ui[2]), U1c = uni(Ui[1] * Ui[1] * Ui[1]);
  auto cube_sum = [&](const float* e) {
    if constexpr (VEER) {
      float m = 0.0f;
#pragma unroll
      for (int j = 0; j < 3; ++j)
#pragma unroll
        for (int k = 0; k < 3; ++k) {
          const float u = Ui[k] * (1.0f - fsqrt(e[3 * j + k]));
          m = fmaf(u * u, u, m);
        }
      return m;
    } else {
      float fe = 0.0f, fc = 0.0f;
#pragma unroll
      for (int j = 0; j < 3; ++j) {
        const float ue = 1.0f - fsqrt(e[2 * j]), uc = 1.0f - fsqrt(e[2 * j + 1]);
        fe = fmaf(ue * ue, ue, fe);
        fc = fmaf(uc * uc, uc, fc);
      }
      return fmaf(U02c, fe, U1c * fc);
    }
  };
  const float ovh = 0.5f * c.guard_inv;
  const float ovs[3] = {uni(ovh * Ui[0] * c.inv_overlap_thr), uni(ovh * Ui[1] * c.inv_overlap_thr), uni(ovh * Ui[2] * c.inv_overlap_thr)};
  const float ovc = 0.5f - ovh;

// ... 203 lines not shown
      const float s_c = fsqrt(fmaxf(1.0f - R.sM * R.sM, 0.0f));
      const float om_sc = R.sM * R.sM * frcp(1.0f + s_c);
      const float b2om = c.beta2 * om_sc, b2om_d = c.beta2_d * om_sc;
      const float x0num_d = R.x0d * fmaf(c.alpha4_d, X.TI0, b2om_d);
      const float x0num_v = R.x0v * fmaf(c.alpha4, X.TI0 + X.dTI, b2om);
      const float pfac = R.pj * R.kyd;
      const float tis[3] = {X.TI0, X.TI1, X.TI2};
      auto col_consts = [&](int j) {
        ColConsts k;
        if (j == 0 || !mine) {
          k.x0d = R.x0d; k.kyd = R.kyd; k.d0 = d0; k.pj = R.pj; k.x0v = R.x0v; k.ix0v = ix0v; k.kyv = R.kyv;
        } else {
          k.x0d = x0num_d * frcp(fmaf(c.alpha4_d, tis[j], b2om_d));
          k.kyd = fmaf(c.ka_d, tis[j], c.kb_d);
          k.d0 = sc.tan_th0 * k.x0d;
          k.pj = pfac * frcp(k.kyd);
          k.x0v = x0num_v * frcp(fmaf(c.alpha4, tis[j] + X.dTI, b2om));
          k.ix0v = frcp(k.x0v);
          k.kyv = fmaf(c.ka, tis[j] + X.dTI, c.kb);
        }
        return k;
      };
      const bool need1 = __any(mine && X.TI1 != X.TI0), need2 = __any(mine && X.TI2 != X.TI0);
      const bool same12 = !__any(mine && X.TI2 != X.TI1);
      const ColWake w0 = column_wake(c, sc, col_consts(0), dx, lin, amp_on);
      ColWake w1 = w0, w2 = w0;
      if (need1) w1 = column_wake(c, sc, col_consts(1), dx, lin, amp_on);
      if (need2) {
        if (need1 && same12) w2 = w1;
        else w2 = column_wake(c, sc, col_consts(2), dx, lin, amp_on);
      }
      column_rows(w0, dy + c.off[0], e1[0], e0[0]);
      column_rows(w1, dy + c.off[1], e1[1], e0[1]);
      column_rows(w2, dy + c.off[2], e1[2], e0[2]);
    }
#pragma unroll
    for (int j = 0; j < 3; ++j) {
      if constexpr (VEER) {
        esq[p][3 * j] = fmaf(e0[j], e0[j], esq[p][3 * j]);
        esq[p][3 * j + 1] = fmaf(e1[j], e1[j], esq[p][3 * j + 1]);
        esq[p][3 * j + 2] = fmaf(e2[j], e2[j], esq[p][3 * j + 2]);
      } else {
        esq[p][2 * j] = fmaf(e0[j], e0[j], esq[p][2 * j]);
        esq[p][2 * j + 1] = fmaf(e1[j], e1[j], esq[p][2 * j + 1]);
      }
    }
    float tipow = ex.z;
    if constexpr (TAB) {
      if (!__any(in15 && (bits & 7))) return;
    } else {
      if (!__any(in15 && (fabsf(dy) < c.twoD + c.off[2] + 1.0f))) return;
      const double twoD_d = 8.0 * c.q_d;
      bits |= (fabs(yi_d - (yt_d - c.q_d)) < twoD_d) ? 1 : 0;
      bits |= (fabs(yi_d - yt_d) < twoD_d) ? 2 : 0;
      bits |= (fabs(yi_d - (yt_d + c.q_d)) < twoD_d) ? 4 : 0;
      const float dxp = (bits & 8) ? dx : dx + 1.0f;
      tipow = fexp2(c.ch_down * flog2(dxp * c.invD));
    }
    float cnt = 0.0f;
    unsigned fbits = 0u;
#pragma unroll
    for (int j = 0; j < 3; ++j) {
      const float f0 = __builtin_amdgcn_fmed3f(fmaf(e0[j], ovs[0], ovc), 0.0f, 1.0f);
      const float f1 = __builtin_amdgcn_fmed3f(fmaf(e1[j], ovs[1], ovc), 0.0f, 1.0f);
      const float f2 = __builtin_amdgcn_fmed3f(fmaf((VEER ? e2[VEER ? j : 0] : e0[j]), ovs[2], ovc), 0.0f, 1.0f);
      cnt += (f0 + f1) + f2;
      fbits |= __float_as_uint(f0) | __float_as_uint(f1) | __float_as_uint(f2);
    }
    cnt = rintf(cnt);
    if ((fbits & 0xc07fffffu) && in15 && (bits & 7)) atomicOr(&risk_lds[wave][eiw], (unsigned)WF_RISK_OVERLAP);
    const float ti = fabsf(R.ch_pref) * tipow;
    const float tia = in15 ? ti * (cnt * (1.0f / 9.0f)) : 0.0f;
    const float cand = fsqrt(fmaf(tia, tia, c.amb2));
#pragma unroll
    for (int j = 0; j < 3; ++j) {
      const float cm = (bits & (1 << j)) ? cand : 0.0f;
      TI[p][j] = __uint_as_float(max(__float_as_uint(TI[p][j]), __float_as_uint(cm)));
    }
  };

  float psum = 0.0f, lsum = 0.0f;
  const int n_real = ga.n_real ? ga.n_real[env] : N;
#ifdef WF_LL_STAMP
  unsigned long long st_acc[12] = {0, 0, 0, 0, 0, 0, 0, 0, 0, 0, 0, 0};
  WF_T(st_begin);
#endif
  int q = 0;
  const size_t wave_rec0 = (size_t)(slot - eiw) * n_pad;
  float2* const log_hot = reinterpret_cast<float2*>(src_log + wave_rec0 * WF_LOG_HOT_FLOATS);
  float4* const log_cold = reinterpret_cast<float4*>(src_log + log_cold_offset + wave_rec0 * WF_LOG_COLD_FLOATS) + eiw;
  float4* const bndL = reinterpret_cast<float4*>(yaw_lds) + (size_t)wave * n_pad;
  constexpr int HOT_INSTR = (CH / 2) * EPW * 16 >= 1024 ? (CH / 2) * EPW * 16 / 1024 : 1;
  constexpr int HOT_F4 = HOT_INSTR * 64;
  float4* const hotL = reinterpret_cast<float4*>(yaw_lds) + (size_t)WPB * n_pad + (size_t)wave * (2 * HOT_F4);
  auto stage_hot = [&](int qq, int i_first) {
    const char* g0 = reinterpret_cast<const char*>(reinterpret_cast<const float4*>(log_hot) + (size_t)(i_first >> 1) * EPW);
    char* l0 = reinterpret_cast<char*>(hotL + (qq & 1) * HOT_F4);
#pragma unroll
    for (int ch = 0; ch < HOT_INSTR; ++ch) lds_dma16(g0 + ch * 1024 + lane * 16, l0 + ch * 1024, true);
  };
  auto hot_index = [&](int i) { return 2 * ((size_t)(i >> 1) * EPW + eiw) + (i & 1); };
  auto load_hot = [&](int i) { return log_hot[hot_index(i)]; };
  auto load_cold = [&](int i) {
    const float4* lp = log_cold + (size_t)i * (3 * EPW);
    ColdRec r;
    r.a = lp[0]; r.b = lp[EPW]; r.c = lp[2 * EPW];
    return r;
  };
  const float snw_f = c.near_c * 0.70710678118f;
  auto unpack = [&](const float2 h, const ColdRec& r) {
    SrcLog R;
    R.Gy = h.x * h.y; R.Gwt = h.y;
    R.sy0d = r.a.x; R.sz0d = r.a.y; R.sM = r.a.z; R.tan_th0 = r.a.w;
    R.sy0v = r.b.x; R.x0d = r.b.y; R.kyd = r.b.z; R.pj = r.b.w;
    R.x0v = r.c.x; R.kyv = r.c.y; R.ch_pref = r.c.z; R.ix0v = r.c.w;
    R.snw = snw_f * R.sM;
    R.kdef = (R.sM * R.sM) * (R.sy0v * c.kdef_sy0v);
    R.inv_s0d = frcp(R.sy0d * R.sz0d);
    R.d0 = R.tan_th0 * R.x0d;
    return R;
  };
  float* const logx = src_log + log_side_offset + (size_t)slot * n_pad * WF_LOG_SIDE_FLOATS;
  int oidx[S], oidx_nx[S], oidx_n2[S];
  float yaw_nx[S];
#pragma unroll
  for (int p = 0; p < S; ++p) {
    oidx_nx[p] = gidx[gofs + min(p * G + sub, N - 1)];
    oidx_n2[p] = gidx[gofs + min(GS + p * G + sub, N - 1)];
  }
#pragma unroll
  for (int p = 0; p < S; ++p) yaw_nx[p] = load_yaw(oidx_nx[p]);
  for (int J = 0; J < nblk; ++J) {
    int tt[S];
    bool tvalid[S];
    float yaw_t[S], sg_t[S], cg_t[S];
    double xt_d[TAB ? 1 : S] = {}, yt_d[TAB ? 1 : S] = {};
#pragma unroll
    for (int p = 0; p < S; ++p) {
      tt[p] = J * GS + p * G + sub;
      tvalid[p] = tt[p] < N;
      if constexpr (!TAB) {
        xt_d[p] = tvalid[p] ? gx[gofs + tt[p]] : -1.0e300;
        yt_d[p] = gy[gofs + (tvalid[p] ? tt[p] : 0)];
      }
#pragma unroll
      for (int k = 0; k < 9; ++k) { V[p][k] = 0.0f; W[p][k] = 0.0f; }
#pragma unroll
      for (int k = 0; k < NE; ++k) esq[p][k] = 0.0f;
#pragma unroll
      for (int j = 0; j < 3; ++j) TI[p][j] = amb0;
      oidx[p] = oidx_nx[p];
      yaw_t[p] = yaw_nx[p];
      oidx_nx[p] = oidx_n2[p];
      oidx_n2[p] = gidx[gofs + min(tt[p] + 2 * GS, N - 1)];
      yaw_nx[p] = load_yaw(oidx_nx[p]);
      sincos_yaw(yaw_t[p] * kDeg2Rad, sg_t[p], cg_t[p]);
    }

    const int first_own = J * GS;
    const int n_src = min(N, first_own + GS);
    const int n_chunks = (n_src + CH - 1) / CH;
    float2 hot_nx = make_float2(0.0f, 0.0f);
    ColdRec cold_nx = {};
    double xs_nx = 0.0, ys_nx = 0.0;
    if (first_own > 0) {
      if constexpr (!TAB) {
        hot_nx = load_hot(0);
        cold_nx = load_cold(0);
        xs_nx = gx[gofs];
        ys_nx = gy[gofs];
      }
    }

    auto fly_record = [&](auto PP, double xi, double yi) {
      constexpr int p = decltype(PP)::value;
      constexpr int q = TAB ? 0 : p;
      float4 r;
      r.x = (float)(xt_d[q] - xi);
      r.y = (float)(yt_d[q] - yi);
      r.z = (xt_d[q] <= xi + c.fifteenD_d) ? 1.0f : 0.0f;
      r.w = __int_as_float((xt_d[q] > xi + 0.1) ? 8 : 0);
      return r;
    };

    auto own_source = [&](auto PS, int i, const float* recs) {
      constexpr int ps = decltype(PS)::value;
      const int src = gbase + ((i - first_own) - ps * G);
      __builtin_amdgcn_s_setprio(3);
      WF_T(so_0);
      float vsum = 0.0f;
#pragma unroll
      for (int k2 = 0; k2 < 9; ++k2) vsum += V[ps][k2];
      const float m3 = __shfl(cube_sum(esq[ps]), src);
      const float Vmean = __shfl(vsum, src) * (1.0f / 9.0f);
      float TIs[3];
#pragma unroll
      for (int j = 0; j < 3; ++j) TIs[j] = __shfl(TI[ps][j], src);
      const float yaw_i = __shfl(yaw_t[ps], src);
      const float cg = __shfl(cg_t[ps], src), sg = __shfl(sg_t[ps], src);
      WF_T(so_1);
      WF_ACC(6, so_0, so_1);
      SrcLog Sc;
      const float ubar = fcbrt_pos(m3 * (1.0f / 9.0f));
      unsigned trisk;
      const float ct = table_ct(c, T, ubar, trisk) * cg;
      if (trisk) atomicOr(&risk_lds[wave][eiw], trisk);
      const float sq1 = fsqrt(1.0f - ct * cg);
      const float a = 0.5f * ct * frcp(1.0f + sq1);
      const float Gwr = c.gam_wr * (a - a * a) * ubar;
      const float gt = c.gam_top * ws * ct, gb = c.gam_bot * ws * ct;
      const float scg = sg * cg * c.sw_tv;
      Sc.Gy = scg * ct * ws;
      Sc.Gwt = Gwr * c.sw_tv;
      WF_T(so_2);
      WF_ACC(7, so_1, so_2);
      float4 ex[S];
      double xi_d = 0.0, yi_d = 0.0;
      if constexpr (!TAB) {
        xi_d = gx[gofs + i];
        yi_d = gy[gofs + i];
      }
      auto pass1_slot = [&](auto PP) {
        constexpr int p = decltype(PP)::value;
        if constexpr (TAB) {
          const float* rec = recs + (p * G + sub) * WF_PAIR_STRIDE;
          ex[p] = *reinterpret_cast<const float4*>(rec + WF_PAIR_DX);
          const bool act1 = (p > ps) ? tvalid[p] : (ex[p].x >= 0.0f);
          if (p >= ps || __any(act1)) {
            if (act1) apply_tab(PP, reinterpret_cast<const float4*>(rec), Sc.Gy, Sc.Gwt);
          }
        } else {
          ex[p] = fly_record(PP, xi_d, yi_d);
          const bool act1 = (p > ps) ? tvalid[p] : (ex[p].x >= 0.0f);
          if (p >= ps || __any(act1)) {
            if (act1) apply_fly(PP, ex[p].x, ex[p].y, Sc.Gy, Sc.Gwt);
          }
        }
      };
      static_for<S>(pass1_slot);
      WF_T(so_3);
      WF_ACC(8, so_2, so_3);
      float vbar = 0.0f, wbar = 0.0f;
#pragma unroll
      for (int k2 = 0; k2 < 9; ++k2) { vbar += V[ps][k2]; wbar += W[ps][k2]; }
      vbar = __shfl(vbar, src) * (1.0f / 9.0f);
      wbar = __shfl(wbar, src) * (1.0f / 9.0f);
      float val = c.sw_steer * (Vmean - Gwr * c.ks_core) * frcp(gt * c.ks_top - gb * c.ks_bot);
      val = fminf(fmaxf(val, -1.0f), 1.0f);
      const float asv = __any(fabsf(val) > 0.3f) ? asinf(val) : asin_small(val);
      const float gd = -(yaw_i * kDeg2Rad + 0.5f * asv);
      const float c2h = fsqrt(fmaxf(fmaf(-val, val, 1.0f), 0.0f));
      const float chh = fsqrt(0.5f * (1.0f + c2h));
      const float shh = 0.5f * val * frcp(chh);
      const float cgd = fmaf(cg, chh, -sg * shh);
      const float s_cc = fsqrt(1.0f - ct * cgd), s_c = fsqrt(1.0f - ct);
      const float om_scc = ct * cgd * frcp(1.0f + s_cc);
      const float om_sc = ct * frcp(1.0f + s_c);
      Sc.sM = fsqrt(ct);
      const float E0 = fmaf(om_sc, om_sc, fmaf(-c.e0c1, om_sc, c.e0c2));
      Sc.sz0d = 0.5f * c.D * fsqrt((1.0f + s_cc) * frcp(2.0f * (1.0f + s_c)));
      Sc.sy0d = Sc.sz0d * cgd;
      if constexpr (VEER) Sc.sy0d *= c.cos_veer;
      const float th0 = c.dm03 * gd * frcp(cgd) * om_scc;
      {
        const float t2 = th0 * th0;
        const float poly = th0 * fmaf(t2, fmaf(t2, fmaf(t2, fmaf(t2, fmaf(t2, 0.0088632355f, 0.0218694885f), 0.0539682540f),
                                                          0.1333333333f), 0.3333333333f), 1.0f);
        Sc.tan_th0 = poly;
        if (__any(fabsf(th0) > 0.35f)) {
          const float rev = th0 * 0.15915494309189535f;
          const float hw = __builtin_amdgcn_sinf(rev) * frcp(__builtin_amdgcn_cosf(rev));
          Sc.tan_th0 = (fabsf(th0) > 0.35f) ? hw : poly;
        }
      }
      const float pfac = th0 * E0 * (1.0f / 5.2f) * fsqrt(Sc.sy0d * Sc.sz0d * frcp(ct)) * kLn2;
      const float x0num_d = c.D * cgd * (1.0f + s_cc) * (1.0f / 1.41421356237f);
      const float I0 = TIs[0];
      const float uI = ubar * I0;
      const float mix2 = (vbar * vbar + wbar * wbar) * (1.0f / 3.0f);
      const float inv_ubar = frcp(ubar);
      const float Itot = fsqrt(fmaf(uI, uI, mix2)) * inv_ubar;
      const float Imix = mix2 * inv_ubar * inv_ubar * frcp(Itot + I0);
      WfLogSide X;
      X.dTI = c.gch_gain * Imix;
      if (lane == src) {
#pragma unroll
        for (int j = 0; j < 3; ++j) TI[ps][j] = fmaxf(TI[ps][j] + X.dTI, amb0);
      }
      Sc.sy0v = c.sz0v * cg;
      if constexpr (VEER) Sc.sy0v *= c.cos_veer;
      Sc.snw = c.near_c * fsqrt(0.5f * ct);
      Sc.kdef = ct * cg * c.kdef;
      Sc.ch_pref = c.ch_c * fexp2(c.ch_ai * flog2(a));
      const float x0num_v = c.D * cg * (1.0f + s_c) * (1.0f / 1.41421356237f);
      const float b2om = c.beta2 * om_sc, b2om_d = c.beta2_d * om_sc;
      Sc.x0d = x0num_d * frcp(fmaf(c.alpha4_d, TIs[0], b2om_d));
      Sc.kyd = fmaf(c.ka_d, TIs[0], c.kb_d);
      Sc.pj = pfac * frcp(Sc.kyd);
      Sc.x0v = x0num_v * frcp(fmaf(c.alpha4, TIs[0] + X.dTI, b2om));
      Sc.kyv = fmaf(c.ka, TIs[0] + X.dTI, c.kb);
      X.TI0 = TIs[0]; X.TI1 = TIs[1]; X.TI2 = TIs[2];
      const bool split = !((TIs[0] == TIs[1]) && (TIs[1] == TIs[2]));
      Sc.ch_pref = split ? -Sc.ch_pref : Sc.ch_pref;
      Sc.ix0v = frcp(Sc.x0v);
      Sc.inv_s0d = frcp(Sc.sy0d * Sc.sz0d);
      Sc.d0 = Sc.tan_th0 * Sc.x0d;
      if (J + 1 < nblk) {
        if (sub == 0) {
          log_hot[hot_index(i)] = make_float2(Sc.Gwt != 0.0f ? Sc.Gy * frcp(Sc.Gwt) : 0.0f, Sc.Gwt);
          float4* lp = log_cold + (size_t)i * (3 * EPW);
          lp[0] = make_float4(Sc.sy0d, Sc.sz0d, Sc.sM, Sc.tan_th0);
          lp[EPW] = make_float4(Sc.sy0v, Sc.x0d, Sc.kyd, Sc.pj);
          lp[2 * EPW] = make_float4(Sc.x0v, Sc.kyv, Sc.ch_pref, Sc.ix0v);
          if (split) *reinterpret_cast<float4*>(logx + (size_t)i * WF_LOG_SIDE_FLOATS) = make_float4(X.TI0, X.TI1, X.TI2, X.dTI);
        }
        const float s0 = VEER ? c.sz0v : Sc.sy0v;
        float kyv_m = Sc.kyv, bb = fmaf(-Sc.kyv, Sc.x0v, s0);
        float db = fabsf(Sc.tan_th0 * Sc.x0d) + 2.2f * fabsf(Sc.pj);
        if (__any(split)) {
          const float TImax = fmaxf(TIs[0], fmaxf(TIs[1], TIs[2])), TImin = fminf(TIs[0], fminf(TIs[1], TIs[2]));
          const float x0d_m = x0num_d * frcp(fmaf(c.alpha4_d, TImin, b2om_d));
          const float pj_m = pfac * frcp(fmaf(c.ka_d, TImin, c.kb_d));
          kyv_m = fmaf(c.ka, TImax + X.dTI, c.kb);
          bb = split ? s0 : bb;
          db = fabsf(Sc.tan_th0 * x0d_m) + 2.2f * fabsf(pj_m);
        }
        const float dbo = db + c.off[2];
        float k6 = c.far_k * kyv_m, b6 = fmaf(c.far_k, bb, dbo), n6 = fmaf(c.far_k, fmaxf(Sc.snw, s0), dbo);
        k6 = wave_max<G>(k6);
        b6 = wave_max<G>(b6);
        n6 = wave_max<G>(n6);
        if (!c.far_on) { k6 = 0.0f; b6 = 0.0f; n6 = 3.0e38f; }
        if (lane == 0) bndL[i] = make_float4(k6, b6, n6, 0.0f);
      }
      WF_T(so_4);
      WF_ACC(9, so_3, so_4);
      const float xs_[4] = {X.TI0, X.TI1, X.TI2, X.dTI};
      static_for<S>([&](auto PP) {
        constexpr int p = decltype(PP)::value;
        if constexpr (p == ps) pass2(PP, Sc, xs_, false, ex[p], ex[p].x > 0.0f, yt_d[TAB ? 0 : p], yi_d);
        else if constexpr (p > ps) pass2(PP, Sc, xs_, false, ex[p], tvalid[p], yt_d[TAB ? 0 : p], yi_d);
      });
      WF_T(so_5);
      WF_ACC(10, so_4, so_5);
      __builtin_amdgcn_s_setprio(0);
    };

    for (int cq = 0; cq < n_chunks; ++cq, ++q) {
      if constexpr (TAB) {
        if (cq == 0 && first_own > 0) wf_dma_wait();
        if (cq + 1 < n_chunks || J + 1 < nblk) stage_chunk(q + 1);
        if (cq + 1 < n_chunks && (cq + 1) * CH < first_own) stage_hot(q + 1, (cq + 1) * CH);
      }
      const float* buf = &prow[q & 1][0];
      const int i0 = cq * CH;
      const int k_log = min(max(first_own - i0, 0), CH);
      const int k_end = min(n_src - i0, CH);
      WF_T(st_a);
      auto within_bound = [&](const float4 bnd, float dx, float dy) {
        return fabsf(dy) < fmaxf(fmaf(bnd.x, dx, bnd.y), bnd.z) + fabsf(fmaf(c.bd, dx, c.ad));
      };
      if constexpr (TAB) {
        if (k_log > 0) {
          unsigned long long near_bits, pair_bits;
          {
            const int kk = lane / GS, rr = lane % GS;
            const float2 e = *reinterpret_cast<const float2*>(buf + (kk * GS + rr) * WF_PAIR_STRIDE + WF_PAIR_DX);
            const float4 bnd = bndL[min(i0 + kk, n_pad - 1)];
            pair_bits = __ballot(kk < k_log && (J * GS + rr) < N && within_bound(bnd, e.x, e.y));
            near_bits = pair_bits;
#pragma unroll
            for (int sh = 1; sh < GS; sh <<= 1) near_bits |= near_bits >> sh;
            unsigned long long rep = 0ull;
#pragma unroll
            for (int kq = 0; kq < CH; ++kq) rep |= 1ull << (kq * GS);
            near_bits &= rep;
          }
          ColdRec cold_nx = {};
          if (near_bits) cold_nx = load_cold(i0 + (__builtin_ctzll(near_bits) / GS));
          static_assert(GS % 2 == 0 && CH % 2 == 0, "logged sources come in pairs");
#pragma unroll 1
          for (int k = 0; k < k_log; k += 2) {
            const float4 hot2 = hotL[(q & 1) * HOT_F4 + (k >> 1) * EPW + eiw];
            float4 cf[S][9];
#pragma unroll
            for (int p = 0; p < S; ++p)
#pragma unroll
              for (int qq = 0; qq < 9; ++qq)
                cf[p][qq] = *reinterpret_cast<const float4*>(buf + (k * GS + p * G + sub) * WF_PAIR_STRIDE + 4 * qq);
            static_for<S>([&](auto PP) { apply_tab_ratio(PP, cf[decltype(PP)::value], hot2.x, hot2.y); });
#pragma unroll
            for (int p = 0; p < S; ++p)
#pragma unroll
              for (int qq = 0; qq < 9; ++qq)
                cf[p][qq] = *reinterpret_cast<const float4*>(buf + ((k + 1) * GS + p * G + sub) * WF_PAIR_STRIDE + 4 * qq);
            static_for<S>([&](auto PP) { apply_tab_ratio(PP, cf[decltype(PP)::value], hot2.z, hot2.w); });
          }
          WF_T(st_ab);
          WF_ACC(11, st_a, st_ab);
          auto near_step = [&](int k, const ColdRec& cold, ColdRec& nxt) {
            const int i = i0 + k;
            float4 exs[S];
#pragma unroll
            for (int p = 0; p < S; ++p)
              exs[p] = *reinterpret_cast<const float4*>(buf + (k * GS + p * G + sub) * WF_PAIR_STRIDE + WF_PAIR_DX);
            asm volatile("" ::: "memory");
#ifdef WF_EXP_NOCOLD
            nxt = cold;
#else
            nxt = load_cold(near_bits ? i0 + (__builtin_ctzll(near_bits) / GS) : i);
#endif
            const SrcLog Sl = unpack(make_float2(0.0f, 0.0f), cold);
            const float* side = logx + (size_t)i * WF_LOG_SIDE_FLOATS;
            static_for<S>([&](auto PP) {
              constexpr int p = decltype(PP)::value;
              if ((pair_bits >> (k * GS + p * G)) & ((1ull << G) - 1ull)) pass2(PP, Sl, side, true, exs[p], tvalid[p]);
            });
          };
          ColdRec cold_b = {};
          __builtin_amdgcn_s_setprio(1);
#pragma unroll 1
          while (near_bits) {
            const int k0 = __builtin_ctzll(near_bits) / GS;
            near_bits &= near_bits - 1ull;
            near_step(k0, cold_nx, cold_b);
            if (!near_bits) break;
            const int k1 = __builtin_ctzll(near_bits) / GS;
            near_bits &= near_bits - 1ull;
            near_step(k1, cold_b, cold_nx);
          }
          __builtin_amdgcn_s_setprio(0);
        }
      } else {
#pragma unroll 1
        for (int k = 0; k < k_log; ++k) {
          const int i = i0 + k;
          const float2 hot = hot_nx;
          const ColdRec cold = cold_nx;
          const int inx = min(i + 1, first_own - 1);
          const float* side = logx + (size_t)i * WF_LOG_SIDE_FLOATS;
          const double xs_d = xs_nx, ys_d = ys_nx;
          hot_nx = load_hot(inx);
          cold_nx = load_cold(inx);
          xs_nx = gx[gofs + inx];
          ys_nx = gy[gofs + inx];
          const float4 bnd = bndL[i];
          float4 exr[S];
          int nr = 0;
          static_for<S>([&](auto PP) {
            constexpr int p = decltype(PP)::value;
            exr[p] = fly_record(PP, xs_d, ys_d);
            nr |= (int)tvalid[p] & (int)within_bound(bnd, exr[p].x, exr[p].y);
          });
          const bool near = __any(nr != 0);
          const SrcLog Sl = unpack(hot, cold);
          static_for<S>([&](auto PP) {
            constexpr int p = decltype(PP)::value;
            if (tvalid[p]) apply_fly(PP, exr[p].x, exr[p].y, hot.x * hot.y, hot.y);
            if (near) pass2(PP, Sl, side, true, exr[p], tvalid[p], yt_d[TAB ? 0 : p], ys_d);
          });
        }
      }
      WF_T(st_b);
      WF_ACC(0, st_a, st_b);
#pragma unroll 1
      for (int k = k_log; k < k_end; ++k) {
        const int i = i0 + k;
        const float* recs = buf + (k * GS) * WF_PAIR_STRIDE;
        const int slot_of_source = (i - first_own) / G;
        static_for<S>([&](auto PS) {
          if (slot_of_source == decltype(PS)::value) own_source(PS, i, recs);
        });
      }
      WF_T(st_c);
      WF_ACC(1, st_b, st_c);
      if constexpr (TAB) {
        wf_dma_wait();
        __syncthreads();
      }
      WF_T(st_d);
      WF_ACC(2, st_c, st_d);
    }
    if constexpr (TAB) {
      if (J + 1 < nblk) stage_hot(q, 0);
    }
    WF_T(st_e);

#pragma unroll
    for (int p = 0; p < S; ++p) {
      if (!tvalid[p]) continue;
      const int o = oidx[p];
      float U[9], m3 = 0.0f, mu = 0.0f, mv = 0.0f, mw = 0.0f, adir = 0.0f;
#pragma unroll
      for (int j = 0; j < 3; ++j) {
        if constexpr (VEER) {
#pragma unroll
          for (int k = 0; k < 3; ++k) U[3 * j + k] = Ui[k] * (1.0f - fsqrt(esq[p][3 * j + k]));
        } else {
          const float ue = 1.0f - fsqrt(esq[p][2 * j]), uc = 1.0f - fsqrt(esq[p][2 * j + 1]);
          U[3 * j] = Ui[0] * ue; U[3 * j + 1] = Ui[1] * uc; U[3 * j + 2] = Ui[2] * ue;
        }
      }
#pragma unroll
      for (int k = 0; k < 9; ++k) {
        m3 = fmaf(U[k] * U[k], U[k], m3);
        mu += U[k]; mv += V[p][k]; mw += W[p][k];
      }
      if (o_wd) {
        bool small = true;
        float rr[9];
#pragma unroll
        for (int k = 0; k < 9; ++k) {
          rr[k] = V[p][k] * frcp(U[k]);
          small = small && (U[k] > 0.0f) && (fabsf(rr[k]) <= 0.25f);
        }
        if (__all(small)) {
#pragma unroll
          for (int k = 0; k < 9; ++k) adir += atan_small(rr[k]);
        } else {
#pragma unroll
          for (int k = 0; k < 9; ++k) adir += atan2f(V[p][k], U[k]);
        }
      }
      mu *= (1.0f / 9.0f); mv *= (1.0f / 9.0f); mw *= (1.0f / 9.0f);
      float su = 0.0f, sv = 0.0f, sw = 0.0f;
#pragma unroll
      for (int k = 0; k < 9; ++k) {
        const float du = U[k] - mu, dv = V[p][k] - mv, dw = W[p][k] - mw;
        su = fmaf(du, du, su); sv = fmaf(dv, dv, sv); sw = fmaf(dw, dw, sw);
      }
      const float wsp = fcbrt_pos(m3 * (1.0f / 9.0f));
      {
        float umin = U[0];
#pragma unroll
        for (int k = 1; k < 9; ++k) umin = fminf(umin, U[k]);
        if (!(umin > 0.0f)) atomicOr(&risk_lds[wave][eiw], (unsigned)WF_RISK_NEGATIVE_SPEED);
      }
      const float veff = c.dens_f * wsp * fexp2(c.pw * flog2(cg_t[p]));
      float pslope;
      const float pwr = c.rho * table_pw(c, T, veff, pslope);
      if (c.rho * fabsf(pslope) * veff > c.knee_kappa * fmaxf(pwr, 1.0e3f))
        atomicOr(&risk_lds[wave][eiw], (unsigned)WF_RISK_POWER_KNEE);
      float4 l;
      l.x = (TI[p][0] + TI[p][1] + TI[p][2]) * (1.0f / 3.0f);
      l.y = fsqrt(su * (1.0f / 9.0f));
      l.z = fsqrt(sv * (1.0f / 9.0f));
      l.w = fsqrt(sw * (1.0f / 9.0f));
      const bool real = o < n_real;
      psum += real ? pwr : 0.0f;
      lsum += real ? (l.x + l.y) + (l.z + l.w) : 0.0f;
      if (env_ok) {
        const size_t oo = yofs + o;
        if (o_power) o_power[oo] = real ? (ea.power_mw ? pwr * 1.0e-6f : pwr) : 0.0f;
        if (o_ws) o_ws[oo] = real ? wsp : 0.0f;
        if (o_wd) o_wd[oo] = real ? wd - adir * (kRad2Deg / 9.0f) : 0.0f;
        if (o_load) reinterpret_cast<float4*>(o_load)[oo] = real ? l : make_float4(0.0f, 0.0f, 0.0f, 0.0f);
      }
    }
    WF_T(st_f);
    WF_ACC(3, st_e, st_f);
  }
#ifdef WF_LL_STAMP
  if (lane == 0) {
    st_acc[4] = __builtin_readcyclecounter() - st_begin;
    for (int k = 0; k < 5; ++k) atomicAdd(&wf_ll_stamp[k], st_acc[k]);
    atomicAdd(&wf_ll_stamp[5], 1ull);
    for (int k = 6; k < 12; ++k) atomicAdd(&wf_ll_stamp[k], st_acc[k]);
  }
#endif

  if (ga.risk_flags && sub == 0 && env_ok) {
    const int rf = (int)risk_lds[wave][eiw];
    ga.risk_flags[env] = rf;
    if (ga.res_list) {
      ga.flags_raw[env] = rf;
      if (rf & ga.res_mask) ga.res_list[atomicAdd(ga.res_count, 1)] = env;
    }
  }
  if (ea.reward) {
#pragma unroll
    for (int w = G / 2; w >= 1; w >>= 1) {
      psum += __shfl_xor(psum, w);
      lsum += __shfl_xor(lsum, w);
    }
    if (sub == 0 && env_ok) {
      const float invN = __fdiv_rn(1.0f, (float)n_real);
      const float wr = ea.ws_prev ? (float)ea.ws_prev[env] : ws;
      const float r = psum * invN * 1.0e-3f * frcp(wr * wr * wr) - ea.load_coef * lsum * invN * 0.25f;
      ea.reward[env] = r;
    }
  }
}

constexpr int kLLWaves = 4;

template <int G, int S, bool TAB, bool MC1, bool VEER = false>
static hipError_t launch_ll(const WfConsts* c, const WfTables* tab, const int* gidx, const double* ws, const double* wd,
                            int wind_stride, const float* yaw, float* power, float* o_ws, float* o_wd, float* load, int B,
                            const WfEnvArgs* env, const float* ll_tab, const int* cross_tie, float* src_log, size_t log_records,
                            const WfGroupArgs* grp, const double* gx, const double* gy, hipStream_t s) {
  constexpr int fpb = kLLWaves * (64 / G);
  WfGroupArgs ga = *grp;
  const int n_farms = ga.env_end ? ga.env_end - ga.env_base : B;
  const int grid = ga.blk_group ? (ga.n_slots + fpb - 1) / fpb : (n_farms + fpb - 1) / fpb;
  WfConsts cc = *c;
  WfEnvArgs ea;
  if (env) ea = *env; else memset(&ea, 0, sizeof(ea));
  size_t group_floats = wfk_ll_table_floats(cc.N, G * S);
  int n_pad = ((cc.N + G * S - 1) / (G * S)) * (G * S);
  constexpr int hot_bytes = 32768 / (G * G * S) >= 1024 ? 32768 / (G * G * S) : 1024;
  const size_t dyn_lds = sizeof(float4) * (size_t)kLLWaves * n_pad + (TAB ? (size_t)kLLWaves * 2 * hot_bytes : 0);
  size_t log_cold_offset = log_records * WF_LOG_HOT_FLOATS, log_side_offset = log_records * WF_LOG_FLOATS;
  void* args[] = {&cc, &tab, &gidx, &ws, &wd, &wind_stride, &yaw, &power, &o_ws, &o_wd, &load, &B, &ea, &ll_tab,
                  &group_floats, &cross_tie, &src_log, &log_cold_offset, &log_side_offset, &n_pad, &ga, &gx, &gy};
  const void* fn = (const void*)&wf_step_ll_kernel<G, S, false, TAB, MC1, kLLWaves, VEER>;
  if constexpr (TAB) {
    if (wind_stride == 0) fn = (const void*)&wf_step_ll_kernel<G, S, true, TAB, MC1, kLLWaves, VEER>;
  }
  if constexpr (S == 1 && (MC1 || !TAB) && !VEER) {
    static int n_cu_of[64] = {};
    int dev = 0, n_cu = 0;
    if (hipGetDevice(&dev) == hipSuccess && dev >= 0 && dev < 64) {
      n_cu = n_cu_of[dev];
      if (n_cu == 0 && hipDeviceGetAttribute(&n_cu, hipDeviceAttributeMultiprocessorCount, dev) == hipSuccess) n_cu_of[dev] = n_cu;
    }
    if (n_cu > 0 && grid <= 2 * n_cu)
      fn = wind_stride == 0 ? (const void*)&wf_step_ll_kernel<G, S, true, TAB, MC1, kLLWaves, VEER, true>
                            : (const void*)&wf_step_ll_kernel<G, S, false, TAB, MC1, kLLWaves, VEER, true>;
  }
  return hipLaunchKernel(fn, dim3(grid), dim3(64 * kLLWaves), args, dyn_lds, s);
}

extern "C" int wfk_ll_farms_per_block(int G) { return kLLWaves * (64 / G); }
#ifdef WF_LL_STAMP
extern "C" int wfk_ll_stamps(unsigned long long* out, int reset) {
  hipError_t e = hipMemcpyFromSymbol(out, HIP_SYMBOL(wf_ll_stamp), sizeof(wf_ll_stamp));
  if (e == hipSuccess && reset) {
    unsigned long long z[16] = {};
    e = hipMemcpyToSymbol(HIP_SYMBOL(wf_ll_stamp), z, sizeof(z));
  }
  return (int)e;
}
#endif

#define WF_LL_DISPATCH(G_, S_, CALL) \
  if (G == G_ && S == S_) return CALL(G_, S_)
extern "C" hipError_t wfk_launch_step_ll(int G, int S, const WfConsts* c, const WfTables* tab, const int* gidx, const double* ws,
                                         const double* wd, int wind_stride, const float* yaw, float* power, float* o_ws,
                                         float* o_wd, float* load, int B, const WfEnvArgs* env, const float* ll_tab,
                                         const int* cross_tie, float* src_log, size_t log_records,
                                         const WfGroupArgs* grp, hipStream_t s) {
#define WF_LL_LAUNCH(G_, S_) launch_ll<G_, S_, true, true>(c, tab, gidx, ws, wd, wind_stride, yaw, power, o_ws, o_wd, load, B, env, ll_tab, cross_tie, src_log, log_records, grp, nullptr, nullptr, s)
#define WF_LL_LAUNCH_VEER(G_, S_) launch_ll<G_, S_, true, true, true>(c, tab, gidx, ws, wd, wind_stride, yaw, power, o_ws, o_wd, load, B, env, ll_tab, cross_tie, src_log, log_records, grp, nullptr, nullptr, s)
  if (c->veer_on) {
    WF_LL_DISPATCH(4, 1, WF_LL_LAUNCH_VEER);
    WF_LL_DISPATCH(4, 2, WF_LL_LAUNCH_VEER);
    WF_LL_DISPATCH(2, 2, WF_LL_LAUNCH_VEER);
    return hipErrorInvalidValue;
  }
  WF_LL_DISPATCH(4, 1, WF_LL_LAUNCH);
  WF_LL_DISPATCH(8, 1, WF_LL_LAUNCH);
  WF_LL_DISPATCH(16, 1, WF_LL_LAUNCH);
  WF_LL_DISPATCH(4, 2, WF_LL_LAUNCH);
  WF_LL_DISPATCH(2, 2, WF_LL_LAUNCH);
  return hipErrorInvalidValue;
}

extern "C" int wfk_ll_has_veer(int G, int S, int table) { return table ? ((G == 4 && S <= 2) || (G == 2 && S == 2)) : (G == 4 && S == 2); }

extern "C" int wfk_ll_has_fly(int G, int S) { return (G == 4 && S <= 2) || (G == 8 && S == 1) || (G == 2 && S == 2); }

extern "C" hipError_t wfk_launch_step_ll_fly(int G, int S, const WfConsts* c, const WfTables* tab, const int* gidx, const double* gx,
                                             const double* gy, const double* ws, const double* wd, const float* yaw,
                                             float* power, float* o_ws, float* o_wd, float* load, int B, const WfEnvArgs* env,
                                             const int* farm_tie, float* src_log, size_t log_records,
                                             const WfGroupArgs* grp, hipStream_t s) {
#define WF_LL_LAUNCH_FLY(G_, S_)                                                                                              \
  (c->mirror_core_n <= 1                                                                                                      \
       ? launch_ll<G_, S_, false, true>(c, tab, gidx, ws, wd, 1, yaw, power, o_ws, o_wd, load, B, env, nullptr, farm_tie, src_log, \
                                        log_records, grp, gx, gy, s)                                                       \
       : launch_ll<G_, S_, false, false>(c, tab, gidx, ws, wd, 1, yaw, power, o_ws, o_wd, load, B, env, nullptr, farm_tie,      \
                                         src_log, log_records, grp, gx, gy, s))
  if (c->veer_on) {
    if (G == 4 && S == 2)
      return launch_ll<4, 2, false, false, true>(c, tab, gidx, ws, wd, 1, yaw, power, o_ws, o_wd, load, B, env, nullptr, farm_tie, src_log,
                                                 log_records, grp, gx, gy, s);
    return hipErrorInvalidValue;
  }
  WF_LL_DISPATCH(4, 2, WF_LL_LAUNCH_FLY);
  WF_LL_DISPATCH(2, 2, WF_LL_LAUNCH_FLY);
  WF_LL_DISPATCH(4, 1, WF_LL_LAUNCH_FLY);
  WF_LL_DISPATCH(8, 1, WF_LL_LAUNCH_FLY);
  return hipErrorInvalidValue;
}

extern "C" hipError_t wfk_ll_func_attributes(int G, int S, int shared_speed, int table, int veer, int occ2, hipFuncAttributes* a) {
#define WF_LL_ATTR_VEER(G_, S_) hipFuncGetAttributes(a, shared_speed ? (const void*)&wf_step_ll_kernel<G_, S_, true, true, true, kLLWaves, true> : (const void*)&wf_step_ll_kernel<G_, S_, false, true, true, kLLWaves, true>)
  if (veer) {
    if (!table) return (G == 4 && S == 2) ? hipFuncGetAttributes(a, (const void*)&wf_step_ll_kernel<4, 2, false, false, true, kLLWaves, true>) : hipErrorInvalidValue;
    WF_LL_DISPATCH(4, 1, WF_LL_ATTR_VEER);
    WF_LL_DISPATCH(4, 2, WF_LL_ATTR_VEER);
    WF_LL_DISPATCH(2, 2, WF_LL_ATTR_VEER);
    return hipErrorInvalidValue;
  }
#define WF_LL_ATTR(G_, S_) hipFuncGetAttributes(a, shared_speed ? (const void*)&wf_step_ll_kernel<G_, S_, true, true, true, kLLWaves> : (const void*)&wf_step_ll_kernel<G_, S_, false, true, true, kLLWaves>)
#define WF_LL_ATTR_FLY(G_, S_) hipFuncGetAttributes(a, (const void*)&wf_step_ll_kernel<G_, S_, false, false, true, kLLWaves>)
#define WF_LL_ATTR_FLY_OCC2(G_, S_) hipFuncGetAttributes(a, (const void*)&wf_step_ll_kernel<G_, S_, false, false, true, kLLWaves, false, true>)
  if (!table) {
    if (occ2) {
      WF_LL_DISPATCH(4, 1, WF_LL_ATTR_FLY_OCC2);
      WF_LL_DISPATCH(8, 1, WF_LL_ATTR_FLY_OCC2);
    }
    WF_LL_DISPATCH(4, 2, WF_LL_ATTR_FLY);
    WF_LL_DISPATCH(2, 2, WF_LL_ATTR_FLY);
    WF_LL_DISPATCH(4, 1, WF_LL_ATTR_FLY);
    WF_LL_DISPATCH(8, 1, WF_LL_ATTR_FLY);
    return hipErrorInvalidValue;
  }
#define WF_LL_ATTR_OCC2(G_, S_) hipFuncGetAttributes(a, shared_speed ? (const void*)&wf_step_ll_kernel<G_, S_, true, true, true, kLLWaves, false, true> : (const void*)&wf_step_ll_kernel<G_, S_, false, true, true, kLLWaves, false, true>)
  if (occ2) {
    WF_LL_DISPATCH(4, 1, WF_LL_ATTR_OCC2);
    WF_LL_DISPATCH(8, 1, WF_LL_ATTR_OCC2);
    WF_LL_DISPATCH(16, 1, WF_LL_ATTR_OCC2);
  }
  WF_LL_DISPATCH(4, 1, WF_LL_ATTR);
  WF_LL_DISPATCH(8, 1, WF_LL_ATTR);
  WF_LL_DISPATCH(16, 1, WF_LL_ATTR);
  WF_LL_DISPATCH(4, 2, WF_LL_ATTR);
  WF_LL_DISPATCH(2, 2, WF_LL_ATTR);
  return hipErrorInvalidValue;
}
```

Before: 82.66 million.

## Add speculative own-stage pass for LL step kernel using precomputed per-block reach test

Extends the LL pair-table kernel to precompute, per direction group and turbine block, whether the block's wakes can be resolved in an own stage, using a wake reach bound built from rotor diameter and expansion constants. The step kernel takes this flag table and, where allowed, runs a speculative own stage that saves state to extra dynamic LDS and uses DPP sub-group reductions and broadcasts, aiming to skip cross-block serial work. The source is also split into separately compiled parts (WF_LL_PART) for the S=2 shapes. It adds a new API and env knob, extra LDS and a device buffer, and may lower occupancy or add speculation overhead when the pre-test fails.

```diff
diff --git a/include/wfstep.h b/include/wfstep.h
--- a/include/wfstep.h
+++ b/include/wfstep.h
@@ -148,6 +148,8 @@
 int wf_get_fly_calibration(wf_handle* h, int* choice, float* ms);
 int wf_get_mixed_launch(wf_handle* h, int* main_farms, float* mixed_ms);
 int wf_get_kernel_choice(wf_handle* h, wf_kernel_choice* c);
+int wf_set_own_stage(wf_handle* h, int mode);
+int wf_get_own_stage(wf_handle* h, int* mode, int* spec_blocks, int* blocks);
 int wf_calibrate(wf_handle* h);
 int wf_set_calibration(wf_handle* h, int code, int fly_choice);
 
diff --git a/wfcrl-env_amd/_lib.py b/wfcrl-env_amd/_lib.py
--- a/wfcrl-env_amd/_lib.py
+++ b/wfcrl-env_amd/_lib.py
@@ -107,6 +107,8 @@
     "wf_get_kernel_info": (C.c_int, [_P, C.POINTER(KernelInfo)]),
     "wf_set_kernel_choice": (C.c_int, [_P, C.POINTER(KernelChoice)]),
     "wf_get_kernel_choice": (C.c_int, [_P, C.POINTER(KernelChoice)]),
+    "wf_set_own_stage": (C.c_int, [_P, C.c_int]),
+    "wf_get_own_stage": (C.c_int, [_P, C.POINTER(C.c_int), C.POINTER(C.c_int), C.POINTER(C.c_int)]),
     "wf_get_calibration": (C.c_int, [_P, C.POINTER(C.c_int), C.POINTER(C.c_float)]),
     "wf_get_fly_calibration": (C.c_int, [_P, C.POINTER(C.c_int), C.POINTER(C.c_float)]),
     "wf_get_mixed_launch": (C.c_int, [_P, C.POINTER(C.c_int), C.POINTER(C.c_float)]),
diff --git a/wfcrl-env_amd/backend.py b/wfcrl-env_amd/backend.py
--- a/wfcrl-env_amd/backend.py
+++ b/wfcrl-env_amd/backend.py
@@ -553,7 +553,8 @@
         check(self._lib.wf_timing_end(self._h, C.byref(ms)), self._h)
         return float(ms.value)
 
-    def set_kernel_choice(self, slot=None, one_block=None, pair_table=None, fly_one_block=None, far_skip=None, calibrate=None, mixed=None):
+    def set_kernel_choice(self, slot=None, one_block=None, pair_table=None, fly_one_block=None, far_skip=None, calibrate=None, mixed=None,
+                          own_stage=None):
         def gs(v, default_s=1):
             if isinstance(v, bool):
                 raise ValueError("a kernel shape is (G, S), 'GxS' or G — not a bool (one_block=False disables the one-block "
@@ -585,6 +586,17 @@
         if mixed is not None:
             c.mixed = 0 if mixed is False or mixed == 0 else -1
         check(self._lib.wf_set_kernel_choice(self._h, C.byref(c)), self._h)
+        if own_stage is not None:
+            self.set_own_stage(own_stage)
+
+    def set_own_stage(self, mode):
+        m = {None: -1, True: 1, False: 0, "always": 2}.get(mode, mode)
+        check(self._lib.wf_set_own_stage(self._h, int(m)), self._h)
+
+    def own_stage(self) -> dict:
+        m, n, t = C.c_int(0), C.c_int(0), C.c_int(0)
+        check(self._lib.wf_get_own_stage(self._h, C.byref(m), C.byref(n), C.byref(t)), self._h)
+        return {"mode": int(m.value), "spec_blocks": int(n.value), "blocks": int(t.value)}
 
     def kernel_choice(self) -> dict:
         c = KernelChoice()
diff --git a/wfcrl-env_amd/csrc/ext/wf_ext.h b/wfcrl-env_amd/csrc/ext/wf_ext.h
--- a/wfcrl-env_amd/csrc/ext/wf_ext.h
+++ b/wfcrl-env_amd/csrc/ext/wf_ext.h
@@ -62,6 +62,7 @@
   wf_model_params model{};
   std::vector<double> tws, tct, tcp, lx, ly;
   wf_kernel_choice choice{};
+  int own_stage = -1;
   double guard = 0.0;
   hipStream_t stream = nullptr;
   evaluator() = default;
diff --git a/wfcrl-env_amd/csrc/ext/wf_ext.hip b/wfcrl-env_amd/csrc/ext/wf_ext.hip
--- a/wfcrl-env_amd/csrc/ext/wf_ext.hip
+++ b/wfcrl-env_amd/csrc/ext/wf_ext.hip
@@ -22,7 +22,7 @@
   const bool same = s.ev && s.E == E && same_model(s.model, h->model) && s.tws == h->tws && s.tct == h->tct && s.tcp == h->tcp &&
                     s.lx.size() == n && std::equal(s.lx.begin(), s.lx.end(), h->lx.begin()) &&
                     std::equal(s.ly.begin(), s.ly.end(), h->ly.begin()) &&
-                    std::memcmp(&s.choice, &h->choice, sizeof(wf_kernel_choice)) == 0 && s.guard == h->guard_rel;
+                    std::memcmp(&s.choice, &h->choice, sizeof(wf_kernel_choice)) == 0 && s.own_stage == h->own_stage && s.guard == h->guard_rel;
   if (same) {
     if (s.stream != h->stream) {
       WFX_EV(x, s.ev, wf_set_stream(s.ev, (void*)h->stream, 1));
@@ -45,6 +45,7 @@
   WFX_EV(x, ev, wf_set_stream(ev, (void*)h->stream, 1));
   WFX_EV(x, ev, wf_set_model(ev, &m));
   WFX_EV(x, ev, wf_set_kernel_choice(ev, &h->choice));
+  WFX_EV(x, ev, wf_set_own_stage(ev, h->own_stage));
   if (h->guard_user) WFX_EV(x, ev, wf_set_risk_guard(ev, h->guard_rel));
   WFX_EV(x, ev, wf_set_layout(ev, h->N, h->lx.data(), h->ly.data()));
   WFX_EV(x, ev, wf_set_batch(ev, E));
@@ -52,7 +53,7 @@
   s.E = E; s.mode = mode; s.stream = h->stream;
   s.model = h->model; s.tws = h->tws; s.tct = h->tct; s.tcp = h->tcp;
   s.lx.assign(h->lx.begin(), h->lx.begin() + n); s.ly.assign(h->ly.begin(), h->ly.begin() + n);
-  s.choice = h->choice; s.guard = h->guard_rel;
+  s.choice = h->choice; s.own_stage = h->own_stage; s.guard = h->guard_rel;
   return WF_OK;
 }
 
diff --git a/wfcrl-env_amd/csrc/wf_abi.hip b/wfcrl-env_amd/csrc/wf_abi.hip
--- a/wfcrl-env_amd/csrc/wf_abi.hip
+++ b/wfcrl-env_amd/csrc/wf_abi.hip
@@ -23,8 +23,8 @@
   h->d_env_moves = nullptr;
   hipFree(h->d_series_ws); hipFree(h->d_series_wd); hipFree(h->d_series_start); hipFree(h->d_ws_prev);
   hipFree(h->d_pair_tab); hipFree(h->d_pair_first); h->d_pair_tab = nullptr; h->d_pair_first = nullptr; h->pair_dirty = true;
-  hipFree(h->d_ll_tab); hipFree(h->d_ll_flag); hipFree(h->d_src_log);
-  h->d_ll_tab = h->d_src_log = nullptr; h->d_ll_flag = nullptr; h->ll_groups_cap = h->log_records_cap = 0;
+  hipFree(h->d_ll_tab); hipFree(h->d_ll_flag); hipFree(h->d_ll_own); hipFree(h->d_src_log);
+  h->d_ll_tab = h->d_src_log = nullptr; h->d_ll_flag = h->d_ll_own = nullptr; h->ll_groups_cap = h->log_records_cap = 0;
   hipFree(h->d_perm); hipFree(h->d_blk_group); hipFree(h->d_group_wd); hipFree(h->d_bins);
   h->d_perm = h->d_blk_group = h->d_bins = nullptr; h->d_group_wd = nullptr;
   h->perm_cap = h->blk_cap = h->pair_groups_cap = 0; h->n_groups = 0; h->grid_step = 0.0;
@@ -67,6 +67,8 @@
     if (off && off[0] == '0') c.one_block = 0;
     const char* fs = getenv("WF_LL_FAR_SKIP");
     if (fs && fs[0] == '0') c.far_skip = 0;
+    const char* ost = getenv("WF_LL_OWN_STAGE");
+    if (ost && (ost[0] == '0' || ost[0] == '2') && ost[1] == 0) h->own_stage = ost[0] - '0';
     const char* rr = getenv("WF_RISK_RESOLVE");
     if (rr && rr[0] >= '0' && rr[0] <= '2' && rr[1] == 0) h->resolve_mode = rr[0] - '0';
     const char* cal = getenv("WF_CALIBRATE");
diff --git a/wfcrl-env_amd/csrc/wf_dispatch.hip b/wfcrl-env_amd/csrc/wf_dispatch.hip
--- a/wfcrl-env_amd/csrc/wf_dispatch.hip
+++ b/wfcrl-env_amd/csrc/wf_dispatch.hip
@@ -195,8 +195,8 @@
 
 void set_ll_shape(wf_handle* h, int G, int S) {
   if (G == h->ll_G && S == h->ll_S) return;
-  hipFree(h->d_ll_tab); hipFree(h->d_ll_flag); hipFree(h->d_src_log);
-  h->d_ll_tab = h->d_src_log = nullptr; h->d_ll_flag = nullptr; h->ll_groups_cap = h->log_records_cap = 0;
+  hipFree(h->d_ll_tab); hipFree(h->d_ll_flag); hipFree(h->d_ll_own); hipFree(h->d_src_log);
+  h->d_ll_tab = h->d_src_log = nullptr; h->d_ll_flag = h->d_ll_own = nullptr; h->ll_groups_cap = h->log_records_cap = 0;
   h->ll_G = G; h->ll_S = S; h->pair_dirty = true;
 }
 int pair_table(wf_handle* h, const float** out) {
@@ -237,13 +237,19 @@
     WF_HIP(h, wfk_launch_pair_table(&pc, (int)ng, h->d_gx, h->d_gy, h->d_pair_tab, h->d_pair_first, h->stream));
     if (h->ll_G) {
       if (!h->d_ll_tab || h->ll_groups_cap < ng) {
-        hipFree(h->d_ll_tab); hipFree(h->d_ll_flag);
-        h->d_ll_tab = nullptr; h->d_ll_flag = nullptr; h->ll_groups_cap = 0;
+        hipFree(h->d_ll_tab); hipFree(h->d_ll_flag); hipFree(h->d_ll_own);
+        h->d_ll_tab = nullptr; h->d_ll_flag = h->d_ll_own = nullptr; h->ll_groups_cap = 0;
         WF_HIP(h, hipMalloc(&h->d_ll_tab, sizeof(float) * ng * wfk_ll_table_floats(h->N, h->ll_G * h->ll_S)));
         WF_HIP(h, hipMalloc(&h->d_ll_flag, sizeof(int) * ng));
+        WF_HIP(h, hipMalloc(&h->d_ll_own, sizeof(int) * ng * (size_t)((h->N + h->ll_G * h->ll_S - 1) / (h->ll_G * h->ll_S))));
         h->ll_groups_cap = ng;
       }
-      WF_HIP(h, wfk_launch_pair_table_ll(&pc, h->ll_G * h->ll_S, (int)ng, h->d_gx, h->d_gy, h->d_ll_tab, h->d_ll_flag, h->stream));
+      const double D_ = m.rotor_diameter;
+      const double reach0 = 6.12 * D_ / std::sqrt(8.0) + 0.25 * D_ + 1.0 * D_ + std::fabs(m.ad);
+      const double reach_k = 6.12 * std::max(m.ka * 0.25 + m.kb, 0.0) + std::fabs(m.bd);
+      const int own_mode = h->own_stage == 0 ? 0 : (h->own_stage == 2 ? 2 : 1);
+      WF_HIP(h, wfk_launch_pair_table_ll(&pc, h->ll_G * h->ll_S, (int)ng, h->d_gx, h->d_gy, h->d_ll_tab, h->d_ll_flag, h->d_ll_own, own_mode,
+                                         reach0, reach_k, h->stream));
       h->ll_ties = 2;
       if (h->wind_sync) {
         std::vector<int> f(ng);
@@ -352,7 +358,7 @@
     if (M) { ga.env_base = 0; ga.env_end = M; }
     if (h->ll_ties != 1)
       WF_HIP(h, wfk_launch_step_ll(h->ll_G, h->ll_S, &h->consts, h->d_tab, h->d_gidx, h->d_ws, h->d_wd, wstride, yaw, power, wspd, wdir,
-                                   load, h->B, ea, h->d_ll_tab, h->d_ll_flag, h->d_src_log,
+                                   load, h->B, ea, h->d_ll_tab, h->d_ll_flag, h->own_stage != 0 ? h->d_ll_own : nullptr, h->d_src_log,
                                    log_records, &ga, h->stream));
     if (M) {
       if (h->ll_ties != 0) {
@@ -401,12 +407,12 @@
 }
 
 struct CalibKey {
-  int device, N, B, n_cu, far_skip;
+  int device, N, B, n_cu, far_skip, own_stage;
   int mixed, slot_G, slot_S;
   unsigned long long layout_hash, model_hash;
   bool operator<(const CalibKey& o) const {
-    return std::tie(device, N, B, n_cu, far_skip, mixed, slot_G, slot_S, layout_hash, model_hash) <
-           std::tie(o.device, o.N, o.B, o.n_cu, o.far_skip, o.mixed, o.slot_G, o.slot_S, o.layout_hash, o.model_hash);
+    return std::tie(device, N, B, n_cu, far_skip, own_stage, mixed, slot_G, slot_S, layout_hash, model_hash) <
+           std::tie(o.device, o.N, o.B, o.n_cu, o.far_skip, o.own_stage, o.mixed, o.slot_G, o.slot_S, o.layout_hash, o.model_hash);
   }
 };
 struct CalibVal {
@@ -424,7 +430,7 @@
 }
 static CalibKey calib_key(const wf_handle* h) {
   CalibKey k{};
-  k.device = h->device; k.N = h->N; k.B = h->B; k.n_cu = h->n_cu; k.far_skip = h->choice.far_skip;
+  k.device = h->device; k.N = h->N; k.B = h->B; k.n_cu = h->n_cu; k.far_skip = h->choice.far_skip; k.own_stage = h->own_stage;
   k.mixed = h->choice.mixed != 0; k.slot_G = h->choice.slot_G; k.slot_S = h->choice.slot_S;
   k.layout_hash = fnv(h->ly.data(), sizeof(double) * h->ly.size(), fnv(h->lx.data(), sizeof(double) * h->lx.size()));
   const wf_model_params& m = h->model;
@@ -764,6 +770,41 @@
   return WF_OK;
 }
 
+int wf_set_own_stage(wf_handle* h, int mode) {
+  if (!h) return WF_E_INVALID;
+  if (mode < -1 || mode > 2) return fail(h, WF_E_INVALID, "wf_set_own_stage: -1 / 1 (where the pre-test allows), 0 (never) or 2 (every block)");
+  WF_ON_DEVICE(h);
+  WF_HIP(h, hipStreamSynchronize(h->stream));
+  if (mode != h->own_stage) {
+    h->own_stage = mode;
+    if (h->N > 0) apply_kernel_pick(h, h->N, h->B, nullptr);
+    h->wind_count = 0; h->shared_dir = false; h->n_groups = 0; h->grid_step = 0.0; h->series_T = 0; h->pair_dirty = true;
+  }
+  return WF_OK;
+}
+
+int wf_get_own_stage(wf_handle* h, int* mode, int* spec_blocks, int* blocks) {
+  if (!h) return WF_E_INVALID;
+  if (mode) *mode = h->own_stage;
+  if (spec_blocks) *spec_blocks = 0;
+  if (blocks) *blocks = 0;
+  if (!spec_blocks && !blocks) return WF_OK;
+  if (!h->ll_G || !h->d_ll_own || h->pair_dirty || h->wind_count == 0) return WF_OK;
+  WF_ON_DEVICE(h);
+  const int GS = h->ll_G * h->ll_S, nblk = (h->N + GS - 1) / GS;
+  const size_t ng = h->n_groups > 0 ? (size_t)h->n_groups : 1;
+  if (ng > h->ll_groups_cap) return WF_OK;
+  std::vector<int> f(ng * nblk);
+  WF_HIP(h, hipMemcpyAsync(f.data(), h->d_ll_own, sizeof(int) * f.size(), hipMemcpyDeviceToHost, h->stream));
+  WF_HIP(h, hipStreamSynchronize(h->stream));
+  const bool used = h->own_stage != 0 && h->consts.far_on && !h->consts.veer_on && GS <= 64 / GS;
+  int n = 0;
+  for (int v : f) n += v != 0;
+  if (spec_blocks) *spec_blocks = used ? n : 0;
+  if (blocks) *blocks = (int)f.size();
+  return WF_OK;
+}
+
 int wf_calibrate(wf_handle* h) {
   if (!h) return WF_E_INVALID;
   if (h->wind_count == 0) return fail(h, WF_E_INVALID, "wf_set_wind must be called before wf_calibrate");
diff --git a/wfcrl-env_amd/csrc/wf_handle.h b/wfcrl-env_amd/csrc/wf_handle.h
--- a/wfcrl-env_amd/csrc/wf_handle.h
+++ b/wfcrl-env_amd/csrc/wf_handle.h
@@ -44,11 +44,12 @@
 extern "C" size_t wfk_ll_table_floats(int N, int G);
 extern "C" int wfk_ll_farms_per_block(int G);
 extern "C" hipError_t wfk_launch_pair_table_ll(const WfPairConsts* pc, int G, int n_groups, const double* gx, const double* gy,
-                                               float* tab, int* cross_tie, hipStream_t s);
+                                               float* tab, int* cross_tie, int* own_ok, int own_mode, double reach0,
+                                               double reach_k, hipStream_t s);
 extern "C" hipError_t wfk_launch_step_ll(int G, int S, const WfConsts* c, const WfTables* tab, const int* gidx, const double* ws,
                                          const double* wd, int wind_stride, const float* yaw, float* power, float* o_ws,
                                          float* o_wd, float* load, int B, const WfEnvArgs* env, const float* ll_tab,
-                                         const int* cross_tie, float* src_log, size_t log_records,
+                                         const int* cross_tie, const int* own_ok, float* src_log, size_t log_records,
                                          const WfGroupArgs* grp, hipStream_t s);
 extern "C" hipError_t wfk_ll_func_attributes(int G, int S, int shared_speed, int table, int veer, int occ2, hipFuncAttributes* a);
 extern "C" hipError_t wfk_launch_fill(int n, double* a, hipStream_t s);
@@ -128,6 +129,7 @@
   int ll_G = 0, ll_S = 1;
   float* d_ll_tab = nullptr;
   int* d_ll_flag = nullptr;
+  int* d_ll_own = nullptr;
   float* d_src_log = nullptr;
   size_t ll_groups_cap = 0, log_records_cap = 0;
   int* d_farm_tie = nullptr;
@@ -142,6 +144,7 @@
   bool wind_sync = true;
   int ll_ties = 2;
   wf_kernel_choice choice{0, 0, -1, 0, 0, -1, -1, -1, -1, -1};
+  int own_stage = -1;
   int n_cu = 256;
   bool calib_done = false;
   int calib_code = -1;
diff --git a/wfcrl-env_amd/csrc/wf_kernels_ll.hip b/wfcrl-env_amd/csrc/wf_kernels_ll.hip
--- a/wfcrl-env_amd/csrc/wf_kernels_ll.hip
+++ b/wfcrl-env_amd/csrc/wf_kernels_ll.hip
@@ -1,10 +1,15 @@
 #include <hip/hip_runtime.h>
 
 #include <cstring>
+#include <mutex>
 #include <type_traits>
 #include <utility>
 
 #include "wf_kernel_common.h"
+
+#ifndef WF_LL_PART
+#define WF_LL_PART 0
+#endif
 
 namespace {
 
@@ -43,6 +48,31 @@
   v = fmaxf(v, dpp(v, std::integral_constant<int, 0x142>{}, std::integral_constant<int, 0xa>{}));
   v = fmaxf(v, dpp(v, std::integral_constant<int, 0x143>{}, std::integral_constant<int, 0xc>{}));
   return __int_as_float(__builtin_amdgcn_readlane(__float_as_int(v), 63));
+}
+
+template <int G>
+__device__ __forceinline__ float sub_max(float v) {
+  auto dpp = [](float x, auto ctrl) {
+    return __int_as_float(__builtin_amdgcn_update_dpp(__float_as_int(x), __float_as_int(x), decltype(ctrl)::value, 0xf, 0xf, false));
+  };
+  static_assert(G >= 2 && G <= 8, "sub_max: lanes per farm");
+  if constexpr (G < 4) v = fmaxf(v, dpp(v, std::integral_constant<int, 0x4E>{}));
+  if constexpr (G < 8) v = fmaxf(v, dpp(v, std::integral_constant<int, 0x124>{}));
+  v = fmaxf(v, dpp(v, std::integral_constant<int, 0x128>{}));
+  v = fmaxf(v, __shfl_xor(v, 16));
+  v = fmaxf(v, __shfl_xor(v, 32));
+  return v;
+}
+
+template <int G, int OS>
+__device__ __forceinline__ float group_bcast(float v, int gbase) {
+  if constexpr (G == 2) {
+    return __int_as_float(__builtin_amdgcn_update_dpp(__float_as_int(v), __float_as_int(v), OS | (OS << 2) | ((2 + OS) << 4) | ((2 + OS) << 6), 0xf, 0xf, false));
+  } else if constexpr (G == 4) {
+    return __int_as_float(__builtin_amdgcn_update_dpp(__float_as_int(v), __float_as_int(v), OS * 0x55, 0xf, 0xf, false));
+  } else {
+    return __shfl(v, gbase + OS);
+  }
 }
 
 struct SrcLog {
@@ -55,18 +85,26 @@
 struct ColdRec { float4 a, b, c; };
 static_assert(WF_LOG_HOT_FLOATS == 2 && WF_LOG_COLD_FLOATS == 12, "source log record");
 struct WfLogSide { float TI0, TI1, TI2, dTI; };
-
-}
-
+struct SrcB { float ubar, ct, a, Gwr, Gy, Gwt; unsigned risk; };
+struct SrcD { SrcLog Sc; WfLogSide X; bool split; float x0num_d, pfac, b2om_d; };
+
+}
+
+#if WF_LL_PART != 1
 __global__ void wf_pair_table_ll_kernel(const WfPairConsts pc, int G, const double* __restrict__ gx,
                                         const double* __restrict__ gy, float* __restrict__ tab, size_t group_floats,
-                                        int* __restrict__ cross_tie) {
+                                        int* __restrict__ cross_tie, int* __restrict__ own_ok, int own_mode, double reach0,
+                                        double reach_k) {
   const int i = blockIdx.x, t = threadIdx.x, grp = blockIdx.y;
   const int nblk = (pc.N + G - 1) / G;
   if (t >= nblk * G) return;
   gx += (size_t)grp * pc.N;
   gy += (size_t)grp * pc.N;
   const int J = t / G;
+  if (own_mode == 1 && i >= J * G && i < t && t < pc.N) {
+    const double dx = gx[t] - gx[i], dy = gy[t] - gy[i];
+    if (dx <= 0.0 || fabs(dy) < reach0 + reach_k * dx) own_ok[(size_t)grp * nblk + J] = 0;
+  }
   if (i >= (J + 1) * G) {
     if (t < pc.N && gx[t] - gx[i] >= 0.0) atomicOr(&cross_tie[grp], 1);
     return;
@@ -78,18 +116,24 @@
 extern "C" size_t wfk_ll_table_floats(int N, int G) { return wf_ll_block_offset((N + G - 1) / G, N, G); }
 
 extern "C" hipError_t wfk_launch_pair_table_ll(const WfPairConsts* pc, int G, int n_groups, const double* gx, const double* gy,
-                                               float* tab, int* cross_tie, hipStream_t s) {
+                                               float* tab, int* cross_tie, int* own_ok, int own_mode, double reach0,
+                                               double reach_k, hipStream_t s) {
   const int nblk = (pc->N + G - 1) / G;
   const int threads = ((nblk * G + 63) / 64) * 64;
   hipError_t e = hipMemsetAsync(cross_tie, 0, sizeof(int) * (size_t)n_groups, s);
   if (e != hipSuccess) return e;
+  e = hipMemsetD32Async((hipDeviceptr_t)own_ok, own_mode ? 1 : 0, (size_t)n_groups * nblk, s);
+  if (e != hipSuccess) return e;
   hipLaunchKernelGGL(wf_pair_table_ll_kernel, dim3(pc->N, n_groups), dim3(threads), 0, s, *pc, G, gx, gy, tab,
-                     wfk_ll_table_floats(pc->N, G), cross_tie);
+                     wfk_ll_table_floats(pc->N, G), cross_tie, own_ok, own_mode, reach0, reach_k);
   return hipGetLastError();
 }
+#else
+extern "C" size_t wfk_ll_table_floats(int N, int G);
+#endif
 
 #ifdef WF_LL_STAMP
-__device__ unsigned long long wf_ll_stamp[16];
+static __device__ unsigned long long wf_ll_stamp[16];
 #define WF_T(v) const unsigned long long v = __builtin_readcyclecounter()
 #define WF_ACC(k, a, b) st_acc[k] += (b) - (a)
 #else
@@ -103,10 +147,11 @@
     float* __restrict__ o_ws, float* __restrict__ o_wd, float* __restrict__ o_load, int B, const WfEnvArgs ea,
     const float* __restrict__ ll_tab, size_t group_floats, const int* __restrict__ cross_tie, float* __restrict__ src_log,
     size_t log_cold_offset, size_t log_side_offset, int n_pad, const WfGroupArgs ga, const double* __restrict__ gx,
-    const double* __restrict__ gy) {
+    const double* __restrict__ gy, const int* __restrict__ own_ok) {
   constexpr int EPW = 64 / G;
   constexpr int GS = G * S;
   constexpr int CH = 64 / GS;
+  constexpr bool STAGE = TAB && !VEER && GS <= CH;
   constexpr int CHUNK_FLOATS = TAB ? 64 * WF_PAIR_STRIDE : 4;
   __shared__ TableLds T;
   __shared__ __attribute__((aligned(16))) float prow[2][CHUNK_FLOATS];
@@ -476,7 +521,7 @@
   float psum = 0.0f, lsum = 0.0f;
   const int n_real = ga.n_real ? ga.n_real[env] : N;
 #ifdef WF_LL_STAMP
-  unsigned long long st_acc[12] = {0, 0, 0, 0, 0, 0, 0, 0, 0, 0, 0, 0};
+  unsigned long long st_acc[14] = {0, 0, 0, 0, 0, 0, 0, 0, 0, 0, 0, 0, 0, 0};
   WF_T(st_begin);
 #endif
   int q = 0;
@@ -486,7 +531,10 @@
   float4* const bndL = reinterpret_cast<float4*>(yaw_lds) + (size_t)wave * n_pad;
   constexpr int HOT_INSTR = (CH / 2) * EPW * 16 >= 1024 ? (CH / 2) * EPW * 16 / 1024 : 1;
   constexpr int HOT_F4 = HOT_INSTR * 64;
-  float4* const hotL = reinterpret_cast<float4*>(yaw_lds) + (size_t)WPB * n_pad + (size_t)wave * (2 * HOT_F4);
+  constexpr int SAVE_F4 = 9 * S * 32;
+  const int wave_f4 = (STAGE && own_ok && SAVE_F4 > 2 * HOT_F4) ? SAVE_F4 : 2 * HOT_F4;
+  float4* const hotL = reinterpret_cast<float4*>(yaw_lds) + (size_t)WPB * n_pad + (size_t)wave * wave_f4;
+  float2* const saveL = reinterpret_cast<float2*>(hotL);
   auto stage_hot = [&](int qq, int i_first) {
     const char* g0 = reinterpret_cast<const char*>(reinterpret_cast<const float4*>(log_hot) + (size_t)(i_first >> 1) * EPW);
     char* l0 = reinterpret_cast<char*>(hotL + (qq & 1) * HOT_F4);
@@ -515,6 +563,115 @@
     return R;
   };
   float* const logx = src_log + log_side_offset + (size_t)slot * n_pad * WF_LOG_SIDE_FLOATS;
+  auto src_part_b = [&](float m3, float cg, float sg) {
+    SrcB b;
+    b.ubar = fcbrt_pos(m3 * (1.0f / 9.0f));
+    b.ct = table_ct(c, T, b.ubar, b.risk) * cg;
+    const float sq1 = fsqrt(1.0f - b.ct * cg);
+    b.a = 0.5f * b.ct * frcp(1.0f + sq1);
+    b.Gwr = c.gam_wr * (b.a - b.a * b.a) * b.ubar;
+    const float scg = sg * cg * c.sw_tv;
+    b.Gy = scg * b.ct * ws;
+    b.Gwt = b.Gwr * c.sw_tv;
+    return b;
+  };
+  auto src_part_d = [&](const SrcB& b, float Vmean, float vbar, float wbar, const float* TIs, float yaw_i, float cg, float sg,
+                        auto any_of) {
+    SrcD d;
+    SrcLog& Sc = d.Sc;
+    const float ubar = b.ubar, ct = b.ct, a = b.a, Gwr = b.Gwr;
+    Sc.Gy = b.Gy;
+    Sc.Gwt = b.Gwt;
+    const float gt = c.gam_top * ws * ct, gb = c.gam_bot * ws * ct;
+    float val = c.sw_steer * (Vmean - Gwr * c.ks_core) * frcp(gt * c.ks_top - gb * c.ks_bot);
+    val = fminf(fmaxf(val, -1.0f), 1.0f);
+    const float asv = any_of(fabsf(val) > 0.3f) ? asinf(val) : asin_small(val);
+    const float gd = -(yaw_i * kDeg2Rad + 0.5f * asv);
+    const float c2h = fsqrt(fmaxf(fmaf(-val, val, 1.0f), 0.0f));
+    const float chh = fsqrt(0.5f * (1.0f + c2h));
+    const float shh = 0.5f * val * frcp(chh);
+    const float cgd = fmaf(cg, chh, -sg * shh);
+    const float s_cc = fsqrt(1.0f - ct * cgd), s_c = fsqrt(1.0f - ct);
+    const float om_scc = ct * cgd * frcp(1.0f + s_cc);
+    const float om_sc = ct * frcp(1.0f + s_c);
+    Sc.sM = fsqrt(ct);
+    const float E0 = fmaf(om_sc, om_sc, fmaf(-c.e0c1, om_sc, c.e0c2));
+    Sc.sz0d = 0.5f * c.D * fsqrt((1.0f + s_cc) * frcp(2.0f * (1.0f + s_c)));
+    Sc.sy0d = Sc.sz0d * cgd;
+    if constexpr (VEER) Sc.sy0d *= c.cos_veer;
+    const float th0 = c.dm03 * gd * frcp(cgd) * om_scc;
+    {
+      const float t2 = th0 * th0;
+      const float poly = th0 * fmaf(t2, fmaf(t2, fmaf(t2, fmaf(t2, fmaf(t2, 0.0088632355f, 0.0218694885f), 0.0539682540f),
+                                                        0.1333333333f), 0.3333333333f), 1.0f);
+      Sc.tan_th0 = poly;
+      if (__any(fabsf(th0) > 0.35f)) {
+        const float rev = th0 * 0.15915494309189535f;
+        const float hw = __builtin_amdgcn_sinf(rev) * frcp(__builtin_amdgcn_cosf(rev));
+        Sc.tan_th0 = (fabsf(th0) > 0.35f) ? hw : poly;
+      }
+    }
+    d.pfac = th0 * E0 * (1.0f / 5.2f) * fsqrt(Sc.sy0d * Sc.sz0d * frcp(ct)) * kLn2;
+    d.x0num_d = c.D * cgd * (1.0f + s_cc) * (1.0f / 1.41421356237f);
+    const float I0 = TIs[0];
+    const float uI = ubar * I0;
+    const float mix2 = (vbar * vbar + wbar * wbar) * (1.0f / 3.0f);
+    const float inv_ubar = frcp(ubar);
+    const float Itot = fsqrt(fmaf(uI, uI, mix2)) * inv_ubar;
+    const float Imix = mix2 * inv_ubar * inv_ubar * frcp(Itot + I0);
+    WfLogSide& X = d.X;
+    X.dTI = c.gch_gain * Imix;
+    Sc.sy0v = c.sz0v * cg;
+    if constexpr (VEER) Sc.sy0v *= c.cos_veer;
+    Sc.snw = c.near_c * fsqrt(0.5f * ct);
+    Sc.kdef = ct * cg * c.kdef;
+    Sc.ch_pref = c.ch_c * fexp2(c.ch_ai * flog2(a));
+    const float x0num_v = c.D * cg * (1.0f + s_c) * (1.0f / 1.41421356237f);
+    const float b2om = c.beta2 * om_sc;
+    d.b2om_d = c.beta2_d * om_sc;
+    Sc.x0d = d.x0num_d * frcp(fmaf(c.alpha4_d, TIs[0], d.b2om_d));
+    Sc.kyd = fmaf(c.ka_d, TIs[0], c.kb_d);
+    Sc.pj = d.pfac * frcp(Sc.kyd);
+    Sc.x0v = x0num_v * frcp(fmaf(c.alpha4, TIs[0] + X.dTI, b2om));
+    Sc.kyv = fmaf(c.ka, TIs[0] + X.dTI, c.kb);
+    X.TI0 = TIs[0]; X.TI1 = TIs[1]; X.TI2 = TIs[2];
+    d.split = !((TIs[0] == TIs[1]) && (TIs[1] == TIs[2]));
+    Sc.ch_pref = d.split ? -Sc.ch_pref : Sc.ch_pref;
+    Sc.ix0v = frcp(Sc.x0v);
+    Sc.inv_s0d = frcp(Sc.sy0d * Sc.sz0d);
+    Sc.d0 = Sc.tan_th0 * Sc.x0d;
+    return d;
+  };
+  auto log_store = [&](int i, const SrcD& d) {
+    const SrcLog& Sc = d.Sc;
+    log_hot[hot_index(i)] = make_float2(Sc.Gwt != 0.0f ? Sc.Gy * frcp(Sc.Gwt) : 0.0f, Sc.Gwt);
+    float4* lp = log_cold + (size_t)i * (3 * EPW);
+    lp[0] = make_float4(Sc.sy0d, Sc.sz0d, Sc.sM, Sc.tan_th0);
+    lp[EPW] = make_float4(Sc.sy0v, Sc.x0d, Sc.kyd, Sc.pj);
+    lp[2 * EPW] = make_float4(Sc.x0v, Sc.kyv, Sc.ch_pref, Sc.ix0v);
+    if (d.split) *reinterpret_cast<float4*>(logx + (size_t)i * WF_LOG_SIDE_FLOATS) = make_float4(d.X.TI0, d.X.TI1, d.X.TI2, d.X.dTI);
+  };
+  auto src_far_bound = [&](const SrcD& d, const float* TIs, float& k6, float& b6, float& n6) {
+    const SrcLog& Sc = d.Sc;
+    const float s0 = VEER ? c.sz0v : Sc.sy0v;
+    float kyv_m = Sc.kyv, bb = fmaf(-Sc.kyv, Sc.x0v, s0);
+    float db = fabsf(Sc.tan_th0 * Sc.x0d) + 2.2f * fabsf(Sc.pj);
+    if (__any(d.split)) {
+      const float TImax = fmaxf(TIs[0], fmaxf(TIs[1], TIs[2])), TImin = fminf(TIs[0], fminf(TIs[1], TIs[2]));
+      const float x0d_m = d.x0num_d * frcp(fmaf(c.alpha4_d, TImin, d.b2om_d));
+      const float pj_m = d.pfac * frcp(fmaf(c.ka_d, TImin, c.kb_d));
+      kyv_m = fmaf(c.ka, TImax + d.X.dTI, c.kb);
+      bb = d.split ? s0 : bb;
+      db = fabsf(Sc.tan_th0 * x0d_m) + 2.2f * fabsf(pj_m);
+    }
+    const float dbo = db + c.off[2];
+    k6 = c.far_k * kyv_m;
+    b6 = fmaf(c.far_k, bb, dbo);
+    n6 = fmaf(c.far_k, fmaxf(Sc.snw, s0), dbo);
+  };
+  auto within_bound = [&](const float4 bnd, float dx, float dy) {
+    return fabsf(dy) < fmaxf(fmaf(bnd.x, dx, bnd.y), bnd.z) + fabsf(fmaf(c.bd, dx, c.ad));
+  };
   int oidx[S], oidx_nx[S], oidx_n2[S];
   float yaw_nx[S];
 #pragma unroll
@@ -594,18 +751,8 @@
       const float cg = __shfl(cg_t[ps], src), sg = __shfl(sg_t[ps], src);
       WF_T(so_1);
       WF_ACC(6, so_0, so_1);
-      SrcLog Sc;
-      const float ubar = fcbrt_pos(m3 * (1.0f / 9.0f));
-      unsigned trisk;
-      const float ct = table_ct(c, T, ubar, trisk) * cg;
-      if (trisk) atomicOr(&risk_lds[wave][eiw], trisk);
-      const float sq1 = fsqrt(1.0f - ct * cg);
-      const float a = 0.5f * ct * frcp(1.0f + sq1);
-      const float Gwr = c.gam_wr * (a - a * a) * ubar;
-      const float gt = c.gam_top * ws * ct, gb = c.gam_bot * ws * ct;
-      const float scg = sg * cg * c.sw_tv;
-      Sc.Gy = scg * ct * ws;
-      Sc.Gwt = Gwr * c.sw_tv;
+      const SrcB Bs = src_part_b(m3, cg, sg);
+      if (Bs.risk) atomicOr(&risk_lds[wave][eiw], Bs.risk);
       WF_T(so_2);
       WF_ACC(7, so_1, so_2);
       float4 ex[S];
@@ -621,13 +768,13 @@
           ex[p] = *reinterpret_cast<const float4*>(rec + WF_PAIR_DX);
           const bool act1 = (p > ps) ? tvalid[p] : (ex[p].x >= 0.0f);
           if (p >= ps || __any(act1)) {
-            if (act1) apply_tab(PP, reinterpret_cast<const float4*>(rec), Sc.Gy, Sc.Gwt);
+            if (act1) apply_tab(PP, reinterpret_cast<const float4*>(rec), Bs.Gy, Bs.Gwt);
           }
         } else {
           ex[p] = fly_record(PP, xi_d, yi_d);
           const bool act1 = (p > ps) ? tvalid[p] : (ex[p].x >= 0.0f);
           if (p >= ps || __any(act1)) {
-            if (act1) apply_fly(PP, ex[p].x, ex[p].y, Sc.Gy, Sc.Gwt);
+            if (act1) apply_fly(PP, ex[p].x, ex[p].y, Bs.Gy, Bs.Gwt);
           }
         }
       };
@@ -639,88 +786,17 @@
       for (int k2 = 0; k2 < 9; ++k2) { vbar += V[ps][k2]; wbar += W[ps][k2]; }
       vbar = __shfl(vbar, src) * (1.0f / 9.0f);
       wbar = __shfl(wbar, src) * (1.0f / 9.0f);
-      float val = c.sw_steer * (Vmean - Gwr * c.ks_core) * frcp(gt * c.ks_top - gb * c.ks_bot);
-      val = fminf(fmaxf(val, -1.0f), 1.0f);
-      const float asv = __any(fabsf(val) > 0.3f) ? asinf(val) : asin_small(val);
-      const float gd = -(yaw_i * kDeg2Rad + 0.5f * asv);
-      const float c2h = fsqrt(fmaxf(fmaf(-val, val, 1.0f), 0.0f));
-      const float chh = fsqrt(0.5f * (1.0f + c2h));
-      const float shh = 0.5f * val * frcp(chh);
-      const float cgd = fmaf(cg, chh, -sg * shh);
-      const float s_cc = fsqrt(1.0f - ct * cgd), s_c = fsqrt(1.0f - ct);
-      const float om_scc = ct * cgd * frcp(1.0f + s_cc);
-      const float om_sc = ct * frcp(1.0f + s_c);
-      Sc.sM = fsqrt(ct);
-      const float E0 = fmaf(om_sc, om_sc, fmaf(-c.e0c1, om_sc, c.e0c2));
-      Sc.sz0d = 0.5f * c.D * fsqrt((1.0f + s_cc) * frcp(2.0f * (1.0f + s_c)));
-      Sc.sy0d = Sc.sz0d * cgd;
-      if constexpr (VEER) Sc.sy0d *= c.cos_veer;
-      const float th0 = c.dm03 * gd * frcp(cgd) * om_scc;
-      {
-        const float t2 = th0 * th0;
-        const float poly = th0 * fmaf(t2, fmaf(t2, fmaf(t2, fmaf(t2, fmaf(t2, 0.0088632355f, 0.0218694885f), 0.0539682540f),
-                                                          0.1333333333f), 0.3333333333f), 1.0f);
-        Sc.tan_th0 = poly;
-        if (__any(fabsf(th0) > 0.35f)) {
-          const float rev = th0 * 0.15915494309189535f;
-          const float hw = __builtin_amdgcn_sinf(rev) * frcp(__builtin_amdgcn_cosf(rev));
-          Sc.tan_th0 = (fabsf(th0) > 0.35f) ? hw : poly;
-        }
-      }
-      const float pfac = th0 * E0 * (1.0f / 5.2f) * fsqrt(Sc.sy0d * Sc.sz0d * frcp(ct)) * kLn2;
-      const float x0num_d = c.D * cgd * (1.0f + s_cc) * (1.0f / 1.41421356237f);
-      const float I0 = TIs[0];
-      const float uI = ubar * I0;
-      const float mix2 = (vbar * vbar + wbar * wbar) * (1.0f / 3.0f);
-      const float inv_ubar = frcp(ubar);
-      const float Itot = fsqrt(fmaf(uI, uI, mix2)) * inv_ubar;
-      const float Imix = mix2 * inv_ubar * inv_ubar * frcp(Itot + I0);
-      WfLogSide X;
-      X.dTI = c.gch_gain * Imix;
+      const SrcD Ds = src_part_d(Bs, Vmean, vbar, wbar, TIs, yaw_i, cg, sg, [](bool f) { return __any(f) != 0; });
+      const SrcLog& Sc = Ds.Sc;
+      const WfLogSide& X = Ds.X;
       if (lane == src) {
 #pragma unroll
         for (int j = 0; j < 3; ++j) TI[ps][j] = fmaxf(TI[ps][j] + X.dTI, amb0);
       }
-      Sc.sy0v = c.sz0v * cg;
-      if constexpr (VEER) Sc.sy0v *= c.cos_veer;
-      Sc.snw = c.near_c * fsqrt(0.5f * ct);
-      Sc.kdef = ct * cg * c.kdef;
-      Sc.ch_pref = c.ch_c * fexp2(c.ch_ai * flog2(a));
-      const float x0num_v = c.D * cg * (1.0f + s_c) * (1.0f / 1.41421356237f);
-      const float b2om = c.beta2 * om_sc, b2om_d = c.beta2_d * om_sc;
-      Sc.x0d = x0num_d * frcp(fmaf(c.alpha4_d, TIs[0], b2om_d));
-      Sc.kyd = fmaf(c.ka_d, TIs[0], c.kb_d);
-      Sc.pj = pfac * frcp(Sc.kyd);
-      Sc.x0v = x0num_v * frcp(fmaf(c.alpha4, TIs[0] + X.dTI, b2om));
-      Sc.kyv = fmaf(c.ka, TIs[0] + X.dTI, c.kb);
-      X.TI0 = TIs[0]; X.TI1 = TIs[1]; X.TI2 = TIs[2];
-      const bool split = !((TIs[0] == TIs[1]) && (TIs[1] == TIs[2]));
-      Sc.ch_pref = split ? -Sc.ch_pref : Sc.ch_pref;
-      Sc.ix0v = frcp(Sc.x0v);
-      Sc.inv_s0d = frcp(Sc.sy0d * Sc.sz0d);
-      Sc.d0 = Sc.tan_th0 * Sc.x0d;
       if (J + 1 < nblk) {
-        if (sub == 0) {
-          log_hot[hot_index(i)] = make_float2(Sc.Gwt != 0.0f ? Sc.Gy * frcp(Sc.Gwt) : 0.0f, Sc.Gwt);
-          float4* lp = log_cold + (size_t)i * (3 * EPW);
-          lp[0] = make_float4(Sc.sy0d, Sc.sz0d, Sc.sM, Sc.tan_th0);
-          lp[EPW] = make_float4(Sc.sy0v, Sc.x0d, Sc.kyd, Sc.pj);
-          lp[2 * EPW] = make_float4(Sc.x0v, Sc.kyv, Sc.ch_pref, Sc.ix0v);
-          if (split) *reinterpret_cast<float4*>(logx + (size_t)i * WF_LOG_SIDE_FLOATS) = make_float4(X.TI0, X.TI1, X.TI2, X.dTI);
-        }
-        const float s0 = VEER ? c.sz0v : Sc.sy0v;
-        float kyv_m = Sc.kyv, bb = fmaf(-Sc.kyv, Sc.x0v, s0);
-        float db = fabsf(Sc.tan_th0 * Sc.x0d) + 2.2f * fabsf(Sc.pj);
-        if (__any(split)) {
-          const float TImax = fmaxf(TIs[0], fmaxf(TIs[1], TIs[2])), TImin = fminf(TIs[0], fminf(TIs[1], TIs[2]));
-          const float x0d_m = x0num_d * frcp(fmaf(c.alpha4_d, TImin, b2om_d));
-          const float pj_m = pfac * frcp(fmaf(c.ka_d, TImin, c.kb_d));
-          kyv_m = fmaf(c.ka, TImax + X.dTI, c.kb);
-          bb = split ? s0 : bb;
-          db = fabsf(Sc.tan_th0 * x0d_m) + 2.2f * fabsf(pj_m);
-        }
-        const float dbo = db + c.off[2];
-        float k6 = c.far_k * kyv_m, b6 = fmaf(c.far_k, bb, dbo), n6 = fmaf(c.far_k, fmaxf(Sc.snw, s0), dbo);
+        if (sub == 0) log_store(i, Ds);
+        float k6, b6, n6;
+        src_far_bound(Ds, TIs, k6, b6, n6);
         k6 = wave_max<G>(k6);
         b6 = wave_max<G>(b6);
         n6 = wave_max<G>(n6);
@@ -740,6 +816,114 @@
       __builtin_amdgcn_s_setprio(0);
     };
 
+    auto own_stage = [&](const float* buf, int k0, int nm) -> bool {
+      if constexpr (STAGE) {
+        __builtin_amdgcn_s_setprio(3);
+        int ln = lane;
+        asm volatile("" : "+v"(ln));
+        const int sub = ln & (G - 1), gbase = ln & ~(G - 1), eiw = ln / G;
+        float2* const sv = saveL + ln;
+#pragma unroll
+        for (int p = 0; p < S; ++p)
+#pragma unroll
+          for (int k2 = 0; k2 < 9; ++k2) sv[(p * 9 + k2) * 64] = make_float2(V[p][k2], W[p][k2]);
+        SrcB Bm[S];
+        float Vmean[S], vbar[S], wbar[S];
+#pragma unroll
+        for (int p = 0; p < S; ++p) {
+          Bm[p] = src_part_b(cube_sum(esq[p]), cg_t[p], sg_t[p]);
+          Vmean[p] = 0.0f; vbar[p] = 0.0f; wbar[p] = 0.0f;
+        }
+        static_for<GS>([&](auto MM) {
+          constexpr int m = decltype(MM)::value;
+          constexpr int ps = m / G, os = m % G;
+          if (m < nm) {
+            float vs = 0.0f;
+#pragma unroll
+            for (int k2 = 0; k2 < 9; ++k2) vs += V[ps][k2];
+            Vmean[ps] = (sub == os) ? vs * (1.0f / 9.0f) : Vmean[ps];
+            const float Gy = group_bcast<G, os>(Bm[ps].Gy, gbase), Gwt = group_bcast<G, os>(Bm[ps].Gwt, gbase);
+            const float* recs = buf + ((k0 + m) * GS) * WF_PAIR_STRIDE;
+            static_for<S>([&](auto PP) {
+              constexpr int p = decltype(PP)::value;
+              const float* rec = recs + (p * G + sub) * WF_PAIR_STRIDE;
+              const bool act1 = (p > ps) ? tvalid[p] : (rec[WF_PAIR_DX] >= 0.0f);
+              if (p >= ps || __any(act1)) {
+                if (act1) apply_tab(PP, reinterpret_cast<const float4*>(rec), Gy, Gwt);
+              }
+            });
+            float vb = 0.0f, wb = 0.0f;
+#pragma unroll
+            for (int k2 = 0; k2 < 9; ++k2) { vb += V[ps][k2]; wb += W[ps][k2]; }
+            vbar[ps] = (sub == os) ? vb * (1.0f / 9.0f) : vbar[ps];
+            wbar[ps] = (sub == os) ? wb * (1.0f / 9.0f) : wbar[ps];
+          }
+        });
+        unsigned long long sub_lanes = 0ull;
+#pragma unroll
+        for (int e = 0; e < EPW; ++e) sub_lanes |= 1ull << (e * G);
+        sub_lanes <<= sub;
+        float dTI[S];
+#pragma unroll
+        for (int p = 0; p < S; ++p) {
+          const float TIs[3] = {TI[p][0], TI[p][1], TI[p][2]};
+          const SrcD Dm = src_part_d(Bm[p], Vmean[p], vbar[p], wbar[p], TIs, yaw_t[p], cg_t[p], sg_t[p],
+                                     [&](bool f) { return (__ballot(f) & sub_lanes) != 0ull; });
+          dTI[p] = Dm.X.dTI;
+          int it = tt[p];
+          asm volatile("" : "+v"(it));
+          if (J + 1 < nblk && tvalid[p]) log_store(it, Dm);
+          float k6, b6, n6;
+          src_far_bound(Dm, TIs, k6, b6, n6);
+          k6 = sub_max<G>(k6);
+          b6 = sub_max<G>(b6);
+          n6 = sub_max<G>(n6);
+          if (!c.far_on) { k6 = 0.0f; b6 = 0.0f; n6 = 3.0e38f; }
+          if (ln < G && tvalid[p]) bndL[tt[p]] = make_float4(k6, b6, n6, 0.0f);
+        }
+        __builtin_amdgcn_fence(__ATOMIC_RELEASE, "wavefront");
+        __builtin_amdgcn_wave_barrier();
+        __builtin_amdgcn_fence(__ATOMIC_ACQUIRE, "wavefront");
+        bool reach = false;
+        {
+          const int ma = ln / GS, mb = ln % GS;
+          if (ma < mb && mb < nm) {
+            const float2 e = *reinterpret_cast<const float2*>(buf + ((k0 + ma) * GS + mb) * WF_PAIR_STRIDE + WF_PAIR_DX);
+            reach = within_bound(bndL[first_own + ma], e.x, e.y);
+          }
+        }
+        const bool stands = __ballot(reach) == 0ull;
+#ifdef WF_LL_STAMP
+        st_acc[12] += 1ull;
+        st_acc[13] += stands ? 0ull : 1ull;
+#endif
+        if (stands) {
+#pragma unroll
+          for (int p = 0; p < S; ++p) {
+            if (tvalid[p] && Bm[p].risk) atomicOr(&risk_lds[wave][eiw], Bm[p].risk);
+#pragma unroll
+            for (int j = 0; j < 3; ++j) TI[p][j] = fmaxf(TI[p][j] + dTI[p], amb0);
+          }
+        } else {
+#pragma unroll
+          for (int p = 0; p < S; ++p)
+#pragma unroll
+            for (int k2 = 0; k2 < 9; ++k2) {
+              const float2 vw = sv[(p * 9 + k2) * 64];
+              V[p][k2] = vw.x; W[p][k2] = vw.y;
+            }
+        }
+        __builtin_amdgcn_s_setprio(0);
+        return stands;
+      } else {
+        return false;
+      }
+    };
+    bool spec_J = false;
+    if constexpr (STAGE) {
+      if (own_ok) spec_J = own_ok[(size_t)grp * nblk + J] != 0;
+    }
+
     for (int cq = 0; cq < n_chunks; ++cq, ++q) {
       if constexpr (TAB) {
         if (cq == 0 && first_own > 0) wf_dma_wait();
@@ -751,9 +935,6 @@
       const int k_log = min(max(first_own - i0, 0), CH);
       const int k_end = min(n_src - i0, CH);
       WF_T(st_a);
-      auto within_bound = [&](const float4 bnd, float dx, float dy) {
-        return fabsf(dy) < fmaxf(fmaf(bnd.x, dx, bnd.y), bnd.z) + fabsf(fmaf(c.bd, dx, c.ad));
-      };
       if constexpr (TAB) {
         if (k_log > 0) {
           unsigned long long near_bits, pair_bits;
@@ -857,8 +1038,12 @@
       }
       WF_T(st_b);
       WF_ACC(0, st_a, st_b);
+      bool staged = false;
+      if constexpr (STAGE) {
+        if (spec_J && k_log < k_end) staged = own_stage(buf, k_log, k_end - k_log);
+      }
 #pragma unroll 1
-      for (int k = k_log; k < k_end; ++k) {
+      for (int k = staged ? k_end : k_log; k < k_end; ++k) {
         const int i = i0 + k;
         const float* recs = buf + (k * GS) * WF_PAIR_STRIDE;
         const int slot_of_source = (i - first_own) / G;
@@ -959,7 +1144,7 @@
     st_acc[4] = __builtin_readcyclecounter() - st_begin;
     for (int k = 0; k < 5; ++k) atomicAdd(&wf_ll_stamp[k], st_acc[k]);
     atomicAdd(&wf_ll_stamp[5], 1ull);
-    for (int k = 6; k < 12; ++k) atomicAdd(&wf_ll_stamp[k], st_acc[k]);
+    for (int k = 6; k < 14; ++k) atomicAdd(&wf_ll_stamp[k], st_acc[k]);
   }
 #endif
 
@@ -992,7 +1177,7 @@
 static hipError_t launch_ll(const WfConsts* c, const WfTables* tab, const int* gidx, const double* ws, const double* wd,
                             int wind_stride, const float* yaw, float* power, float* o_ws, float* o_wd, float* load, int B,
                             const WfEnvArgs* env, const float* ll_tab, const int* cross_tie, float* src_log, size_t log_records,
-                            const WfGroupArgs* grp, const double* gx, const double* gy, hipStream_t s) {
+                            const WfGroupArgs* grp, const double* gx, const double* gy, const int* own_ok, hipStream_t s) {
   constexpr int fpb = kLLWaves * (64 / G);
   WfGroupArgs ga = *grp;
   const int n_farms = ga.env_end ? ga.env_end - ga.env_base : B;
@@ -1003,10 +1188,10 @@
   size_t group_floats = wfk_ll_table_floats(cc.N, G * S);
   int n_pad = ((cc.N + G * S - 1) / (G * S)) * (G * S);
   constexpr int hot_bytes = 32768 / (G * G * S) >= 1024 ? 32768 / (G * G * S) : 1024;
-  const size_t dyn_lds = sizeof(float4) * (size_t)kLLWaves * n_pad + (TAB ? (size_t)kLLWaves * 2 * hot_bytes : 0);
+  size_t dyn_lds = sizeof(float4) * (size_t)kLLWaves * n_pad + (TAB ? (size_t)kLLWaves * 2 * hot_bytes : 0);
   size_t log_cold_offset = log_records * WF_LOG_HOT_FLOATS, log_side_offset = log_records * WF_LOG_FLOATS;
   void* args[] = {&cc, &tab, &gidx, &ws, &wd, &wind_stride, &yaw, &power, &o_ws, &o_wd, &load, &B, &ea, &ll_tab,
-                  &group_floats, &cross_tie, &src_log, &log_cold_offset, &log_side_offset, &n_pad, &ga, &gx, &gy};
+                  &group_floats, &cross_tie, &src_log, &log_cold_offset, &log_side_offset, &n_pad, &ga, &gx, &gy, &own_ok};
   const void* fn = (const void*)&wf_step_ll_kernel<G, S, false, TAB, MC1, kLLWaves, VEER>;
   if constexpr (TAB) {
     if (wind_stride == 0) fn = (const void*)&wf_step_ll_kernel<G, S, true, TAB, MC1, kLLWaves, VEER>;
@@ -1022,10 +1207,33 @@
       fn = wind_stride == 0 ? (const void*)&wf_step_ll_kernel<G, S, true, TAB, MC1, kLLWaves, VEER, true>
                             : (const void*)&wf_step_ll_kernel<G, S, false, TAB, MC1, kLLWaves, VEER, true>;
   }
+  if (!(TAB && !VEER && G * S <= 64 / (G * S)) || !cc.far_on) own_ok = nullptr;
+  if (own_ok) {
+    const size_t save_wave = sizeof(float) * 18 * S * 64;
+    const size_t save_bytes = save_wave > 2 * (size_t)hot_bytes ? (save_wave - 2 * (size_t)hot_bytes) * kLLWaves : 0;
+    struct Occ { const void* fn; size_t lds; int keeps; };
+    static Occ seen[16] = {};
+    static int n_seen = 0;
+    static std::mutex seen_mutex;
+    std::lock_guard<std::mutex> lock(seen_mutex);
+    int keeps = -1;
+    for (int k = 0; k < n_seen; ++k)
+      if (seen[k].fn == fn && seen[k].lds == dyn_lds) keeps = seen[k].keeps;
+    if (keeps < 0) {
+      int without = 0, with = 0;
+      keeps = (hipOccupancyMaxActiveBlocksPerMultiprocessor(&without, fn, 64 * kLLWaves, dyn_lds) == hipSuccess &&
+               hipOccupancyMaxActiveBlocksPerMultiprocessor(&with, fn, 64 * kLLWaves, dyn_lds + save_bytes) == hipSuccess && with >= without && with > 0) ? 1 : 0;
+      if (n_seen < 16) seen[n_seen++] = Occ{fn, dyn_lds, keeps};
+    }
+    if (keeps) dyn_lds += save_bytes; else own_ok = nullptr;
+  }
   return hipLaunchKernel(fn, dim3(grid), dim3(64 * kLLWaves), args, dyn_lds, s);
 }
 
+#if WF_LL_PART != 1
 extern "C" int wfk_ll_farms_per_block(int G) { return kLLWaves * (64 / G); }
+#endif
+#if WF_LL_PART != 2
 #ifdef WF_LL_STAMP
 extern "C" int wfk_ll_stamps(unsigned long long* out, int reset) {
   hipError_t e = hipMemcpyFromSymbol(out, HIP_SYMBOL(wf_ll_stamp), sizeof(wf_ll_stamp));
@@ -1037,15 +1245,38 @@
 }
 #endif
 
+#endif
+
 #define WF_LL_DISPATCH(G_, S_, CALL) \
   if (G == G_ && S == S_) return CALL(G_, S_)
+#define WF_LL_STEP_ARGS                                                                                                          \
+  int G, int S, const WfConsts *c, const WfTables *tab, const int *gidx, const double *ws, const double *wd, int wind_stride,   \
+      const float *yaw, float *power, float *o_ws, float *o_wd, float *load, int B, const WfEnvArgs *env, const float *ll_tab,    \
+      const int *cross_tie, const int *own_ok, float *src_log, size_t log_records, const WfGroupArgs *grp, hipStream_t s
+#define WF_LL_LAUNCH(G_, S_) launch_ll<G_, S_, true, true>(c, tab, gidx, ws, wd, wind_stride, yaw, power, o_ws, o_wd, load, B, env, ll_tab, cross_tie, src_log, log_records, grp, nullptr, nullptr, own_ok, s)
+#if WF_LL_PART != 2
+extern "C" hipError_t wfk_launch_step_ll_s2(WF_LL_STEP_ARGS) {
+  WF_LL_DISPATCH(4, 2, WF_LL_LAUNCH);
+  WF_LL_DISPATCH(2, 2, WF_LL_LAUNCH);
+  return hipErrorInvalidValue;
+}
+extern "C" hipError_t wfk_ll_func_attributes_s2(int G, int S, int shared_speed, hipFuncAttributes* a) {
+#define WF_LL_ATTR_S2(G_, S_) hipFuncGetAttributes(a, shared_speed ? (const void*)&wf_step_ll_kernel<G_, S_, true, true, true, kLLWaves> : (const void*)&wf_step_ll_kernel<G_, S_, false, true, true, kLLWaves>)
+  WF_LL_DISPATCH(4, 2, WF_LL_ATTR_S2);
+  WF_LL_DISPATCH(2, 2, WF_LL_ATTR_S2);
+  return hipErrorInvalidValue;
+}
+#endif
+
+#if WF_LL_PART != 1
+extern "C" hipError_t wfk_launch_step_ll_s2(WF_LL_STEP_ARGS);
+extern "C" hipError_t wfk_ll_func_attributes_s2(int G, int S, int shared_speed, hipFuncAttributes* a);
 extern "C" hipError_t wfk_launch_step_ll(int G, int S, const WfConsts* c, const WfTables* tab, const int* gidx, const double* ws,
                                          const double* wd, int wind_stride, const float* yaw, float* power, float* o_ws,
                                          float* o_wd, float* load, int B, const WfEnvArgs* env, const float* ll_tab,
-                                         const int* cross_tie, float* src_log, size_t log_records,
+                                         const int* cross_tie, const int* own_ok, float* src_log, size_t log_records,
                                          const WfGroupArgs* grp, hipStream_t s) {
-#define WF_LL_LAUNCH(G_, S_) launch_ll<G_, S_, true, true>(c, tab, gidx, ws, wd, wind_stride, yaw, power, o_ws, o_wd, load, B, env, ll_tab, cross_tie, src_log, log_records, grp, nullptr, nullptr, s)
-#define WF_LL_LAUNCH_VEER(G_, S_) launch_ll<G_, S_, true, true, true>(c, tab, gidx, ws, wd, wind_stride, yaw, power, o_ws, o_wd, load, B, env, ll_tab, cross_tie, src_log, log_records, grp, nullptr, nullptr, s)
+#define WF_LL_LAUNCH_VEER(G_, S_) launch_ll<G_, S_, true, true, true>(c, tab, gidx, ws, wd, wind_stride, yaw, power, o_ws, o_wd, load, B, env, ll_tab, cross_tie, src_log, log_records, grp, nullptr, nullptr, nullptr, s)
   if (c->veer_on) {
     WF_LL_DISPATCH(4, 1, WF_LL_LAUNCH_VEER);
     WF_LL_DISPATCH(4, 2, WF_LL_LAUNCH_VEER);
@@ -1055,8 +1286,7 @@
   WF_LL_DISPATCH(4, 1, WF_LL_LAUNCH);
   WF_LL_DISPATCH(8, 1, WF_LL_LAUNCH);
   WF_LL_DISPATCH(16, 1, WF_LL_LAUNCH);
-  WF_LL_DISPATCH(4, 2, WF_LL_LAUNCH);
-  WF_LL_DISPATCH(2, 2, WF_LL_LAUNCH);
+  if (S == 2) return wfk_launch_step_ll_s2(G, S, c, tab, gidx, ws, wd, wind_stride, yaw, power, o_ws, o_wd, load, B, env, ll_tab, cross_tie, own_ok, src_log, log_records, grp, s);
   return hipErrorInvalidValue;
 }
 
@@ -1072,13 +1302,13 @@
 #define WF_LL_LAUNCH_FLY(G_, S_)                                                                                              \
   (c->mirror_core_n <= 1                                                                                                      \
        ? launch_ll<G_, S_, false, true>(c, tab, gidx, ws, wd, 1, yaw, power, o_ws, o_wd, load, B, env, nullptr, farm_tie, src_log, \
-                                        log_records, grp, gx, gy, s)                                                       \
+                                        log_records, grp, gx, gy, nullptr, s)                                                       \
        : launch_ll<G_, S_, false, false>(c, tab, gidx, ws, wd, 1, yaw, power, o_ws, o_wd, load, B, env, nullptr, farm_tie,      \
-                                         src_log, log_records, grp, gx, gy, s))
+                                         src_log, log_records, grp, gx, gy, nullptr, s))
   if (c->veer_on) {
     if (G == 4 && S == 2)
       return launch_ll<4, 2, false, false, true>(c, tab, gidx, ws, wd, 1, yaw, power, o_ws, o_wd, load, B, env, nullptr, farm_tie, src_log,
-                                                 log_records, grp, gx, gy, s);
+                                                 log_records, grp, gx, gy, nullptr, s);
     return hipErrorInvalidValue;
   }
   WF_LL_DISPATCH(4, 2, WF_LL_LAUNCH_FLY);
@@ -1088,29 +1318,31 @@
   return hipErrorInvalidValue;
 }
 
+extern "C" hipError_t wfk_ll_func_attributes_fly(int G, int S, int veer, int occ2, hipFuncAttributes* a) {
+  if (veer) return (G == 4 && S == 2) ? hipFuncGetAttributes(a, (const void*)&wf_step_ll_kernel<4, 2, false, false, true, kLLWaves, true>) : hipErrorInvalidValue;
+#define WF_LL_ATTR_FLY(G_, S_) hipFuncGetAttributes(a, (const void*)&wf_step_ll_kernel<G_, S_, false, false, true, kLLWaves>)
+#define WF_LL_ATTR_FLY_OCC2(G_, S_) hipFuncGetAttributes(a, (const void*)&wf_step_ll_kernel<G_, S_, false, false, true, kLLWaves, false, true>)
+  if (occ2) {
+    WF_LL_DISPATCH(4, 1, WF_LL_ATTR_FLY_OCC2);
+    WF_LL_DISPATCH(8, 1, WF_LL_ATTR_FLY_OCC2);
+  }
+  WF_LL_DISPATCH(4, 2, WF_LL_ATTR_FLY);
+  WF_LL_DISPATCH(2, 2, WF_LL_ATTR_FLY);
+  WF_LL_DISPATCH(4, 1, WF_LL_ATTR_FLY);
+  WF_LL_DISPATCH(8, 1, WF_LL_ATTR_FLY);
+  return hipErrorInvalidValue;
+}
+
 extern "C" hipError_t wfk_ll_func_attributes(int G, int S, int shared_speed, int table, int veer, int occ2, hipFuncAttributes* a) {
+  if (!table) return wfk_ll_func_attributes_fly(G, S, veer, occ2, a);
 #define WF_LL_ATTR_VEER(G_, S_) hipFuncGetAttributes(a, shared_speed ? (const void*)&wf_step_ll_kernel<G_, S_, true, true, true, kLLWaves, true> : (const void*)&wf_step_ll_kernel<G_, S_, false, true, true, kLLWaves, true>)
   if (veer) {
-    if (!table) return (G == 4 && S == 2) ? hipFuncGetAttributes(a, (const void*)&wf_step_ll_kernel<4, 2, false, false, true, kLLWaves, true>) : hipErrorInvalidValue;
     WF_LL_DISPATCH(4, 1, WF_LL_ATTR_VEER);
     WF_LL_DISPATCH(4, 2, WF_LL_ATTR_VEER);
     WF_LL_DISPATCH(2, 2, WF_LL_ATTR_VEER);
     return hipErrorInvalidValue;
   }
 #define WF_LL_ATTR(G_, S_) hipFuncGetAttributes(a, shared_speed ? (const void*)&wf_step_ll_kernel<G_, S_, true, true, true, kLLWaves> : (const void*)&wf_step_ll_kernel<G_, S_, false, true, true, kLLWaves>)
-#define WF_LL_ATTR_FLY(G_, S_) hipFuncGetAttributes(a, (const void*)&wf_step_ll_kernel<G_, S_, false, false, true, kLLWaves>)
-#define WF_LL_ATTR_FLY_OCC2(G_, S_) hipFuncGetAttributes(a, (const void*)&wf_step_ll_kernel<G_, S_, false, false, true, kLLWaves, false, true>)
-  if (!table) {
-    if (occ2) {
-      WF_LL_DISPATCH(4, 1, WF_LL_ATTR_FLY_OCC2);
-      WF_LL_DISPATCH(8, 1, WF_LL_ATTR_FLY_OCC2);
-    }
-    WF_LL_DISPATCH(4, 2, WF_LL_ATTR_FLY);
-    WF_LL_DISPATCH(2, 2, WF_LL_ATTR_FLY);
-    WF_LL_DISPATCH(4, 1, WF_LL_ATTR_FLY);
-    WF_LL_DISPATCH(8, 1, WF_LL_ATTR_FLY);
-    return hipErrorInvalidValue;
-  }
 #define WF_LL_ATTR_OCC2(G_, S_) hipFuncGetAttributes(a, shared_speed ? (const void*)&wf_step_ll_kernel<G_, S_, true, true, true, kLLWaves, false, true> : (const void*)&wf_step_ll_kernel<G_, S_, false, true, true, kLLWaves, false, true>)
   if (occ2) {
     WF_LL_DISPATCH(4, 1, WF_LL_ATTR_OCC2);
@@ -1120,7 +1352,7 @@
   WF_LL_DISPATCH(4, 1, WF_LL_ATTR);
   WF_LL_DISPATCH(8, 1, WF_LL_ATTR);
   WF_LL_DISPATCH(16, 1, WF_LL_ATTR);
-  WF_LL_DISPATCH(4, 2, WF_LL_ATTR);
-  WF_LL_DISPATCH(2, 2, WF_LL_ATTR);
+  if (S == 2) return wfk_ll_func_attributes_s2(G, S, shared_speed, a);
   return hipErrorInvalidValue;
 }
+#endif
```

Result: faster. 85.20 million (median of 6 runs) (+3.1%).
